# crate-crypto/rust-eth-kzg

Measured on AMD Instinct MI355X. Metric: blobs/sec compute_cells_and_kzg_proofs (4096-pt blob), higher is better.
Workload: dtype u32

## Files before the change

### include/c_eth_kzg_test_hooks.h

```cpp
#ifndef C_ETH_KZG_TEST_HOOKS_H
#define C_ETH_KZG_TEST_HOOKS_H
#include "c_eth_kzg.h"
#ifdef __cplusplus
extern "C" {
#endif

int eth_kzg_amd_test_fr_ntt4096(const DASContext *ctx, const uint8_t *in, uint8_t *out, int inverse_dit);
int eth_kzg_amd_test_g1_fft128(const DASContext *ctx, const uint8_t *in, uint8_t *out, int n_lanes, int inverse);
int eth_kzg_amd_test_fixed_msm(const DASContext *ctx, const uint8_t *scalars, int n_msm, uint8_t *out);
int eth_kzg_amd_test_g1_decompress(const DASContext *ctx, const uint8_t *in, int n, int subgroup_check, int32_t *status,
                                   uint8_t *out);
int eth_kzg_amd_test_field_mul(const DASContext *ctx, const uint8_t *a, const uint8_t *b, uint8_t *out, int n,
                               int is_fp);

int eth_kzg_amd_test_prover_scalars(const DASContext *ctx, int n, const uint8_t *blobs, uint32_t *scalars, uint64_t max_words,
                                    uint64_t *n_words, uint8_t *cells, uint8_t *proofs, int32_t *status, int32_t *fused_launches);

int eth_kzg_amd_test_sha256_many(const DASContext *ctx, uint64_t n, const uint8_t *prefix, uint64_t prefix_len, const uint8_t *d_body,
                                 uint64_t body_stride, uint64_t body_len, const uint8_t *d_tail, uint64_t tail_stride, uint64_t tail_len,
                                 uint8_t *d_out);

int eth_kzg_amd_test_verify_msm(const DASContext *ctx, int form, const uint8_t *points, int n_pts, const uint8_t *sc0, int n0,
                                const uint8_t *sc1, int n1, uint8_t *out96, int32_t *sub_status);

int eth_kzg_amd_test_verify_cells_partial_device(const DASContext *ctx, uint64_t n, const uint8_t *d_commitments,
                                                 const uint64_t *d_cell_indices, const uint8_t *d_cells, const uint8_t *d_proofs, uint64_t lo,
                                                 uint64_t hi, uint8_t *out96);
int eth_kzg_amd_test_verify_blob_batch_inputs(const DASContext *ctx, uint64_t n, int on_device, const void *blobs, const void *commitments,
                                              const void *proofs, uint8_t *out96, int32_t *verified);

int eth_kzg_amd_test_verify_many_sums(const DASContext *ctx, uint64_t n_batches, const uint64_t *commitments_lengths,
                                      const uint8_t *const *const *commitments, const uint64_t *cell_indices_lengths,
                                      const uint64_t *const *cell_indices, const uint64_t *cells_lengths, const uint8_t *const *const *cells,
                                      const uint64_t *proofs_lengths, const uint8_t *const *const *proofs, int32_t *verified, int32_t *status,
                                      int32_t *form4, uint8_t *sums96, uint32_t *rho, uint8_t *fold96, int32_t *probe_ranges,
                                      uint8_t *probe_sums96, uint64_t max_probes, uint64_t *n_probes);

int eth_kzg_amd_test_rs_decode(const DASContext *ctx, int R, const uint64_t *n_cells, const uint64_t *const *cell_indices,
                               const uint8_t *const *const *cells, int flat_source, int32_t *status, int32_t *deg,
                               uint8_t *zp, uint8_t *zeval, uint8_t *zcinv, uint8_t *coeffs);

int eth_kzg_amd_test_op_info(int op, int32_t *in_words, int32_t *out_words, int32_t *device_only, const char **name);
int eth_kzg_amd_test_op(const DASContext *ctx, int op, int n, const int32_t *in, int32_t *out, int on_device);

int eth_kzg_amd_test_table_info(const DASContext *ctx, int kind, int which, int64_t *out8, int32_t *piece_first_block, int max_pieces);
int eth_kzg_amd_test_table_audit(const DASContext *ctx, int kind, int which, uint64_t *visited, uint64_t *n_findings, int32_t *findings,
                                 int max_findings, double *ms);
int eth_kzg_amd_test_table_read(const DASContext *ctx, int kind, int which, int group, int window, int base, int d0, int n, uint32_t *out);
int eth_kzg_amd_test_table_audit_buffer(const DASContext *ctx, int c, int n_groups, int nb, const uint32_t *table, const uint8_t *bases,
                                        int on_device, uint64_t *visited, uint64_t *n_findings, int32_t *findings, int max_findings);

#ifdef __cplusplus
}
#endif
#endif
```

### rust-eth-kzg_amd/__init__.py

```python
import ctypes as C

import numpy as np
import os

_HERE = os.path.dirname(os.path.abspath(__file__))
LIB_PATH = os.path.join(_HERE, "libc_eth_kzg.so")
HOOKS_LIB_PATH = os.path.join(_HERE, "libc_eth_kzg_hooks.so")

BYTES_PER_BLOB = 131072
BYTES_PER_CELL = 2048
BYTES_PER_COMMITMENT = 48
BYTES_PER_PROOF = 48
CELLS_PER_EXT_BLOB = 128
FIELD_ELEMENTS_PER_BLOB = 4096
FIELD_ELEMENTS_PER_CELL = 64


class KzgError(Exception):
    """An operation the reference would report as `Err(..)` (CResult.status == Err)."""


class CResult(C.Structure):
    _fields_ = [("status", C.c_int), ("error_msg", C.c_void_p)]


VERIFY_PARTIAL_BYTES = 96
SETUP_NO_SUBGROUP_CHECK = 1
SETUP_CHECK_POWERS = 2
SETUP_G1_POINTS = 4096
SETUP_G2_POINTS = 65

EXPORTED_SYMBOLS = [
    "eth_kzg_das_context_new", "eth_kzg_das_context_free", "eth_kzg_free_error_message",
    "eth_kzg_blob_to_kzg_commitment", "eth_kzg_compute_cells_and_kzg_proofs", "eth_kzg_compute_cells",
    "eth_kzg_verify_cell_kzg_proof_batch", "eth_kzg_recover_cells_and_proofs",
    "eth_kzg_constant_bytes_per_cell", "eth_kzg_constant_bytes_per_proof", "eth_kzg_constant_cells_per_ext_blob",
    "eth_kzg_compute_kzg_proof", "eth_kzg_compute_blob_kzg_proof", "eth_kzg_verify_kzg_proof",
    "eth_kzg_verify_blob_kzg_proof", "eth_kzg_verify_blob_kzg_proof_batch",
    "eth_kzg_amd_das_context_new_on_device",
    "eth_kzg_amd_das_context_try_new", "eth_kzg_amd_das_context_new_on_devices", "eth_kzg_amd_context_devices",
    "eth_kzg_amd_das_context_new_with_setup", "eth_kzg_amd_das_context_new_with_setup_file", "eth_kzg_amd_setup_digest",
    "eth_kzg_amd_abi_version", "eth_kzg_amd_window_count", "eth_kzg_amd_glv_table",
    "eth_kzg_amd_compute_cells_and_kzg_proofs_batch", "eth_kzg_amd_blob_to_kzg_commitment_batch",
    "eth_kzg_amd_recover_cells_and_proofs_batch", "eth_kzg_amd_recover_cells_and_proofs_device",
    "eth_kzg_amd_verify_cell_kzg_proof_batch_partial", "eth_kzg_amd_verify_cell_kzg_proof_batch_combine",
    "eth_kzg_amd_compute_cells_and_kzg_proofs_device", "eth_kzg_amd_blob_to_kzg_commitment_device",
    "eth_kzg_amd_verify_cell_kzg_proof_batch_device", "eth_kzg_amd_verify_cell_kzg_proof_batch_many",
    "eth_kzg_amd_compute_blob_kzg_proof_batch", "eth_kzg_amd_compute_kzg_proof_batch",
    "eth_kzg_amd_compute_blob_kzg_proof_device", "eth_kzg_amd_compute_kzg_proof_device",
    "eth_kzg_amd_verify_blob_kzg_proof_batch_device",
    "eth_kzg_amd_table_bytes", "eth_kzg_amd_window_bits", "eth_kzg_amd_tables_ready", "eth_kzg_amd_table_groups_ready", "eth_kzg_amd_table_build_info", "eth_kzg_amd_linmap_info",
    "eth_kzg_amd_set_profiling", "eth_kzg_amd_get_stage_times",
    "eth_kzg_amd_comm_probe", "eth_kzg_amd_comm_unique_id", "eth_kzg_amd_comm_init", "eth_kzg_amd_comm_info",
    "eth_kzg_amd_all_gather", "eth_kzg_amd_comm_destroy",
    "eth_kzg_amd_compute_cells_and_kzg_proofs_batch_multi", "eth_kzg_amd_device_count",
]
TEST_HOOK_SYMBOLS = [
    "eth_kzg_amd_test_fr_ntt4096", "eth_kzg_amd_test_g1_fft128", "eth_kzg_amd_test_fixed_msm",
    "eth_kzg_amd_test_g1_decompress", "eth_kzg_amd_test_field_mul", "eth_kzg_amd_test_op_info", "eth_kzg_amd_test_op",
    "eth_kzg_amd_test_table_info", "eth_kzg_amd_test_table_audit", "eth_kzg_amd_test_table_read", "eth_kzg_amd_test_table_audit_buffer",
    "eth_kzg_amd_test_sha256_many", "eth_kzg_amd_test_verify_msm",
    "eth_kzg_amd_test_verify_cells_partial_device", "eth_kzg_amd_test_verify_blob_batch_inputs", "eth_kzg_amd_test_rs_decode",
    "eth_kzg_amd_test_prover_scalars", "eth_kzg_amd_test_verify_many_sums",
]

_lib = None


def load_library():
    global _lib
    if _lib is not None:
        return _lib
    path = os.environ.get("ETH_KZG_AMD_LIB", LIB_PATH)
    if not os.path.exists(path):
        raise RuntimeError(
            f"{LIB_PATH} is missing: build the HIP extension first (python -c 'import __graft_entry__ as g; g.build()' "
            "or make -C rust-eth-kzg_amd/csrc). There is no CPU fallback.")
    lib = C.CDLL(path)
    P, U8P, U64 = C.c_void_p, C.c_char_p, C.c_uint64
    lib.eth_kzg_das_context_new.restype = P
    lib.eth_kzg_das_context_new.argtypes = [C.c_bool]
    lib.eth_kzg_amd_das_context_new_on_device.restype = P
    lib.eth_kzg_amd_das_context_new_on_device.argtypes = [C.c_bool, C.c_int]
    lib.eth_kzg_amd_das_context_try_new.restype = P
    lib.eth_kzg_amd_das_context_try_new.argtypes = [C.c_bool, C.c_int, C.c_double, C.POINTER(CResult)]
    lib.eth_kzg_das_context_free.argtypes = [P]
    lib.eth_kzg_free_error_message.argtypes = [P]
    for name, args in {
        "eth_kzg_blob_to_kzg_commitment": [P, U8P, P],
        "eth_kzg_compute_cells_and_kzg_proofs": [P, U8P, P, P],
        "eth_kzg_compute_cells": [P, U8P, P],
        "eth_kzg_verify_cell_kzg_proof_batch": [P, U64, P, U64, P, U64, P, U64, P, P],
        "eth_kzg_recover_cells_and_proofs": [P, U64, P, U64, P, P, P],
        "eth_kzg_compute_kzg_proof": [P, U8P, U8P, P, P],
        "eth_kzg_compute_blob_kzg_proof": [P, U8P, U8P, P],
        "eth_kzg_verify_kzg_proof": [P, U8P, U8P, U8P, U8P, P],
        "eth_kzg_verify_blob_kzg_proof": [P, U8P, U8P, U8P, P],
        "eth_kzg_verify_blob_kzg_proof_batch": [P, U64, P, U64, P, U64, P, P],
        "eth_kzg_amd_compute_cells_and_kzg_proofs_batch": [P, U64, P, P, P, P],
        "eth_kzg_amd_blob_to_kzg_commitment_batch": [P, U64, P, P, P],
        "eth_kzg_amd_recover_cells_and_proofs_batch": [P, U64, P, P, P, P, P, P, P],
        "eth_kzg_amd_verify_cell_kzg_proof_batch_partial": [P, U64, P, U64, P, U64, P, U64, P, U64, U64, P],
        "eth_kzg_amd_verify_cell_kzg_proof_batch_combine": [P, U64, U8P, P],
        "eth_kzg_amd_recover_cells_and_proofs_device": [P, U64, P, P, P, P, P, P],
        "eth_kzg_amd_compute_cells_and_kzg_proofs_device": [P, U64, P, P, P, P, P],
        "eth_kzg_amd_blob_to_kzg_commitment_device": [P, U64, P, P, P, P],
        "eth_kzg_amd_verify_cell_kzg_proof_batch_device": [P, U64, P, P, P, P, P, P],
        "eth_kzg_amd_verify_cell_kzg_proof_batch_many": [P, U64, P, P, P, P, P, P, P, P, P, P],
        "eth_kzg_amd_compute_blob_kzg_proof_batch": [P, U64, P, P, P, P],
        "eth_kzg_amd_compute_kzg_proof_batch": [P, U64, P, P, P, P, P],
        "eth_kzg_amd_compute_blob_kzg_proof_device": [P, U64, P, P, P, P, P],
        "eth_kzg_amd_compute_kzg_proof_device": [P, U64, P, P, P, P, P, P],
        "eth_kzg_amd_verify_blob_kzg_proof_batch_device": [P, U64, P, P, P, P, P],
        "eth_kzg_amd_comm_unique_id": [P],
        "eth_kzg_amd_comm_probe": [P, P, U64],
        "eth_kzg_amd_comm_info": [P, P, P],
        "eth_kzg_amd_comm_init": [P, U8P, C.c_int, C.c_int],
        "eth_kzg_amd_all_gather": [P, P, P, U64, P],
        "eth_kzg_amd_compute_cells_and_kzg_proofs_batch_multi": [P, U64, U64, P, P, P, P],
    }.items():
        fn = getattr(lib, name)
        fn.restype = CResult
        fn.argtypes = args
    for name in ("eth_kzg_constant_bytes_per_cell", "eth_kzg_constant_bytes_per_proof",
                 "eth_kzg_constant_cells_per_ext_blob"):
        getattr(lib, name).restype = U64
    lib.eth_kzg_amd_comm_destroy.argtypes = [P]
    lib.eth_kzg_amd_comm_destroy.restype = None
    lib.eth_kzg_amd_device_count.restype = C.c_int
    lib.eth_kzg_amd_table_bytes.restype = U64
    lib.eth_kzg_amd_table_bytes.argtypes = [P]
    lib.eth_kzg_amd_window_bits.argtypes = [P]
    lib.eth_kzg_amd_tables_ready.argtypes = [P, C.c_int]
    lib.eth_kzg_amd_tables_ready.restype = C.c_int
    lib.eth_kzg_amd_table_build_info.argtypes = [P, C.POINTER(C.c_double)]
    lib.eth_kzg_amd_table_build_info.restype = None
    lib.eth_kzg_amd_table_groups_ready.argtypes = [P]
    lib.eth_kzg_amd_table_groups_ready.restype = C.c_int
    lib.eth_kzg_amd_linmap_info.argtypes = [P, P]
    lib.eth_kzg_amd_linmap_info.restype = None
    lib.eth_kzg_amd_set_profiling.argtypes = [P, C.c_int]
    lib.eth_kzg_amd_set_profiling.restype = None
    lib.eth_kzg_amd_get_stage_times.argtypes = [P, P, P, C.c_int]
    lib.eth_kzg_amd_das_context_new_on_devices.restype = P
    lib.eth_kzg_amd_das_context_new_on_devices.argtypes = [C.c_bool, P, U64, C.c_double, C.POINTER(CResult)]
    lib.eth_kzg_amd_context_devices.restype = U64
    lib.eth_kzg_amd_context_devices.argtypes = [P, P, U64]
    lib.eth_kzg_amd_abi_version.restype = C.c_int
    if hasattr(lib, "eth_kzg_amd_das_context_new_with_setup"):
        lib.eth_kzg_amd_das_context_new_with_setup.restype = P
        lib.eth_kzg_amd_das_context_new_with_setup.argtypes = [P, U64, P, U64, C.c_uint32, C.c_bool, P, U64, C.c_double, C.POINTER(CResult)]
        lib.eth_kzg_amd_das_context_new_with_setup_file.restype = P
        lib.eth_kzg_amd_das_context_new_with_setup_file.argtypes = [P, U64, C.c_uint32, C.c_bool, P, U64, C.c_double, C.POINTER(CResult)]
        lib.eth_kzg_amd_setup_digest.restype = None
        lib.eth_kzg_amd_setup_digest.argtypes = [P, P]
    lib.eth_kzg_amd_window_count.argtypes = [P]
    lib.eth_kzg_amd_glv_table.argtypes = [P]
    for name, args in {
        "eth_kzg_amd_test_fr_ntt4096": [P, U8P, P, C.c_int],
        "eth_kzg_amd_test_g1_fft128": [P, U8P, P, C.c_int, C.c_int],
        "eth_kzg_amd_test_fixed_msm": [P, U8P, C.c_int, P],
        "eth_kzg_amd_test_g1_decompress": [P, U8P, C.c_int, C.c_int, P, P],
        "eth_kzg_amd_test_field_mul": [P, U8P, U8P, P, C.c_int, C.c_int],
        "eth_kzg_amd_test_op_info": [C.c_int, P, P, P, C.POINTER(C.c_char_p)],
        "eth_kzg_amd_test_op": [P, C.c_int, C.c_int, P, P, C.c_int],
        "eth_kzg_amd_test_table_info": [P, C.c_int, C.c_int, P, P, C.c_int],
        "eth_kzg_amd_test_table_audit": [P, C.c_int, C.c_int, P, P, P, C.c_int, P],
        "eth_kzg_amd_test_table_read": [P, C.c_int, C.c_int, C.c_int, C.c_int, C.c_int, C.c_int, C.c_int, P],
        "eth_kzg_amd_test_table_audit_buffer": [P, C.c_int, C.c_int, C.c_int, P, P, C.c_int, P, P, P, C.c_int],
        "eth_kzg_amd_test_sha256_many": [P, U64, P, U64, P, U64, U64, P, U64, U64, P],
        "eth_kzg_amd_test_verify_msm": [P, C.c_int, U8P, C.c_int, U8P, C.c_int, U8P, C.c_int, P, P],
        "eth_kzg_amd_test_verify_cells_partial_device": [P, U64, P, P, P, P, U64, U64, P],
        "eth_kzg_amd_test_verify_blob_batch_inputs": [P, U64, C.c_int, P, P, P, P, P],
        "eth_kzg_amd_test_rs_decode": [P, C.c_int, P, P, P, C.c_int, P, P, P, P, P, P],
        "eth_kzg_amd_test_prover_scalars": [P, C.c_int, P, P, U64, P, P, P, P, P],
        "eth_kzg_amd_test_verify_many_sums": [P, U64, P, P, P, P, P, P, P, P, P, P, P, P, P, P, P, P, U64, P],
    }.items():
        if hasattr(lib, name):
            getattr(lib, name).argtypes = args
    _lib = lib
    return lib


def present_masks(n, present):
    masks = np.zeros(2 * max(1, n), dtype=np.uint64)
    prev_row, prev_mask = None, 0
    for b in range(n):
        row = present[b]
        if row is prev_row and prev_row is not None:
            m = prev_mask
        else:
            m = 0
            for c in row:
                c = int(c)
                if not 0 <= c < CELLS_PER_EXT_BLOB:
                    raise KzgError("InvalidCellIndex")
                m |= 1 << c
            prev_row, prev_mask = row, m
        masks[2 * b] = m & 0xFFFFFFFFFFFFFFFF
        masks[2 * b + 1] = m >> 64
    return masks


def parse_trusted_setup_json(text):
    import json
    try:
        doc = json.loads(text)
    except ValueError as e:
        raise KzgError(f"InvalidSetup: not JSON ({e})")
    if not isinstance(doc, dict):
        raise KzgError("InvalidSetup: the trusted setup JSON is an object with g1_monomial and g2_monomial")
    out = []
    for key, size in (("g1_monomial", 48), ("g2_monomial", 96)):
        pts = doc.get(key)
        if not isinstance(pts, list):
            raise KzgError(f"InvalidSetup: {key} is missing")
        dec = []
        for i, h in enumerate(pts):
            if not isinstance(h, str) or not h.startswith("0x"):
                raise KzgError(f"InvalidSetup: {key}[{i}] is not a 0x-prefixed hex string")
            try:
                b = bytes.fromhex(h[2:])
            except ValueError:
                raise KzgError(f"InvalidSetup: {key}[{i}] is not hex")
            if len(b) != size:
                raise KzgError(f"InvalidSetup: {key}[{i}] has {len(b)} bytes, not {size}")
            dec.append(b)
        out.append(dec)
    return out[0], out[1]


def _ptr_array(bufs):
    arr = (C.c_void_p * max(1, len(bufs)))()
    keep = []
    for i, b in enumerate(bufs):
        if isinstance(b, (bytes, bytearray)):
            b = C.create_string_buffer(bytes(b), len(b))
        keep.append(b)
        arr[i] = C.addressof(b)
    return arr, keep


def _flat_ptrs(items, size):
    n = len(items)
    flat = np.frombuffer(b"".join(bytes(x) if not isinstance(x, bytes) else x for x in items), dtype=np.uint8) if n else np.zeros(1, np.uint8)
    ptrs = np.uint64(flat.ctypes.data) + np.arange(max(1, n), dtype=np.uint64) * np.uint64(size)
    return ptrs, flat


def _out_ptrs(n_outer, n_inner, size):
    flat = np.zeros(max(1, n_outer * n_inner * size), dtype=np.uint8)
    inner = np.uint64(flat.ctypes.data) + np.arange(max(1, n_outer * n_inner), dtype=np.uint64) * np.uint64(size)
    outer = np.uint64(inner.ctypes.data) + np.arange(max(1, n_outer), dtype=np.uint64) * np.uint64(n_inner * 8)
    return flat, inner, outer


def _split(flat, n_outer, n_inner, size):
    raw = flat.tobytes()
    return [[raw[(b * n_inner + k) * size:(b * n_inner + k + 1) * size] for k in range(n_inner)] for b in range(n_outer)]


def _vp(arr):
    return arr.ctypes.data_as(C.c_void_p)


class DASContext:

    device_index = 0

    def __init__(self, use_precomp=True, device=None, wait_tables=True, table_budget_gb=None, devices=None):
        self.device_index = int(device) if device is not None else int(os.environ.get("ETH_KZG_AMD_DEVICE", "0"))
        self._lib = load_library()
        if devices is not None:
            devs = np.array([int(d) for d in devices], dtype=np.int32)
            self.device_index = int(devs[0]) if len(devs) else 0
            res = CResult()
            self._ctx = C.c_void_p(self._lib.eth_kzg_amd_das_context_new_on_devices(
                bool(use_precomp), _vp(devs) if len(devs) else None, len(devs), float(table_budget_gb or 0.0), C.byref(res)))
            if not self._ctx.value:
                msg = C.cast(res.error_msg, C.c_char_p).value.decode() if res.error_msg else "unknown"
                self._lib.eth_kzg_free_error_message(res.error_msg)
                raise KzgError(msg)
        elif table_budget_gb is not None:
            res = CResult()
            self._ctx = C.c_void_p(self._lib.eth_kzg_amd_das_context_try_new(bool(use_precomp), self.device_index, float(table_budget_gb), C.byref(res)))
            if not self._ctx.value:
                msg = C.cast(res.error_msg, C.c_char_p).value.decode() if res.error_msg else "unknown"
                self._lib.eth_kzg_free_error_message(res.error_msg)
                raise KzgError(msg)
        elif device is None:
            self._ctx = C.c_void_p(self._lib.eth_kzg_das_context_new(bool(use_precomp)))
        else:
            self._ctx = C.c_void_p(self._lib.eth_kzg_amd_das_context_new_on_device(bool(use_precomp), int(device)))
        if not self._ctx.value:
            raise RuntimeError("eth_kzg_das_context_new returned NULL")
        if wait_tables:
            self.tables_ready(-1)

    @classmethod
    def from_trusted_setup(cls, g1_monomial, g2_monomial, *, subgroup_check=True, check_powers=False, use_precomp=True, devices=None,
                           table_budget_gb=None, wait_tables=True):
        def flat(pts, size):
            if isinstance(pts, (bytes, bytearray, memoryview)):
                raw = bytes(pts)
                if len(raw) % size:
                    raise KzgError(f"InvalidSetup: {len(raw)} bytes are not a whole number of {size}-byte points")
                return raw, len(raw) // size
            pts = [bytes(x) for x in pts]
            for i, x in enumerate(pts):
                if len(x) != size:
                    raise KzgError(f"InvalidSetup: point {i} has {len(x)} bytes, not {size}")
            return b"".join(pts), len(pts)
        g1, n1 = flat(g1_monomial, 48)
        g2, n2 = flat(g2_monomial, 96)
        self = cls.__new__(cls)
        self._lib = load_library()
        self._ctx = C.c_void_p(None)
        devs = np.array([int(d) for d in devices], dtype=np.int32) if devices is not None else None
        self.device_index = int(devs[0]) if devs is not None and len(devs) else int(os.environ.get("ETH_KZG_AMD_DEVICE", "0"))
        flags = (0 if subgroup_check else SETUP_NO_SUBGROUP_CHECK) | (SETUP_CHECK_POWERS if check_powers else 0)
        res = CResult()
        b1, b2 = C.create_string_buffer(g1, max(1, len(g1))), C.create_string_buffer(g2, max(1, len(g2)))
        self._ctx = C.c_void_p(self._lib.eth_kzg_amd_das_context_new_with_setup(
            C.addressof(b1), n1, C.addressof(b2), n2, flags, bool(use_precomp), _vp(devs) if devs is not None and len(devs) else None,
            len(devs) if devs is not None else 0, float(table_budget_gb or 0.0), C.byref(res)))
        if not self._ctx.value:
            msg = C.cast(res.error_msg, C.c_char_p).value.decode() if res.error_msg else "unknown"
            self._lib.eth_kzg_free_error_message(res.error_msg)
            raise KzgError(msg)
        if wait_tables:
            self.tables_ready(-1)
        return self

    @classmethod
    def from_trusted_setup_json(cls, text_or_path, *, check_powers=True, **kwargs):
        text = text_or_path
        if not str(text_or_path).lstrip().startswith("{"):
            with open(text_or_path) as f:
                text = f.read()
        g1, g2 = parse_trusted_setup_json(text)
        return cls.from_trusted_setup(g1, g2, check_powers=check_powers, **kwargs)

    @property
    def setup_digest(self):
        out = C.create_string_buffer(32)
        self._lib.eth_kzg_amd_setup_digest(self._ctx, out)
        return out.raw

    def devices(self):
        out = np.zeros(64, dtype=np.int32)
        n = int(self._lib.eth_kzg_amd_context_devices(self._ctx, _vp(out), 64))
        return [int(d) for d in out[:n]]

    def tables_ready(self, wait_ms=0):
        return int(self._lib.eth_kzg_amd_tables_ready(self._ctx, int(wait_ms)))

    def table_build_info(self):
        out = (C.c_double * 4)()
        self._lib.eth_kzg_amd_table_build_info(self._ctx, out)
        return {"hipmalloc_ms": round(out[0], 1), "longest_hipmalloc_ms": round(out[1], 1), "pieces": int(out[2]), "bytes": int(out[3])}

    def table_groups_ready(self):
        return int(self._lib.eth_kzg_amd_table_groups_ready(self._ctx))

    def close(self):
        if getattr(self, "_ctx", None) and self._ctx.value:
            self._lib.eth_kzg_das_context_free(self._ctx)
            self._ctx = C.c_void_p(None)

    def __del__(self):
        try:
            self.close()
        except Exception:
            pass

    @property
    def handle(self):
        return self._ctx

    def _check(self, res):
        if res.status != 0:
            msg = C.string_at(res.error_msg).decode() if res.error_msg else "error"
            self._lib.eth_kzg_free_error_message(res.error_msg)
            raise KzgError(msg)

    def blob_to_kzg_commitment(self, blob):
        if len(blob) != BYTES_PER_BLOB:
            raise KzgError("BlobHasInvalidLength")
        out = C.create_string_buffer(48)
        self._check(self._lib.eth_kzg_blob_to_kzg_commitment(self._ctx, bytes(blob), out))
        return out.raw

    def compute_cells_and_kzg_proofs(self, blob):
        if len(blob) != BYTES_PER_BLOB:
            raise KzgError("BlobHasInvalidLength")
        cells = [C.create_string_buffer(BYTES_PER_CELL) for _ in range(CELLS_PER_EXT_BLOB)]
        proofs = [C.create_string_buffer(48) for _ in range(CELLS_PER_EXT_BLOB)]
        ca, _k1 = _ptr_array(cells)
        pa, _k2 = _ptr_array(proofs)
        self._check(self._lib.eth_kzg_compute_cells_and_kzg_proofs(self._ctx, bytes(blob), ca, pa))
        return [c.raw for c in cells], [p.raw for p in proofs]

    def compute_cells(self, blob):
        if len(blob) != BYTES_PER_BLOB:
            raise KzgError("BlobHasInvalidLength")
        cells = [C.create_string_buffer(BYTES_PER_CELL) for _ in range(CELLS_PER_EXT_BLOB)]
        ca, _k = _ptr_array(cells)
        self._check(self._lib.eth_kzg_compute_cells(self._ctx, bytes(blob), ca))
        return [c.raw for c in cells]

    def verify_cell_kzg_proof_batch(self, commitments, cell_indices, cells, proofs):
        if any(len(c) != 48 for c in commitments) or any(len(p) != 48 for p in proofs) \
                or any(len(c) != BYTES_PER_CELL for c in cells):
            raise KzgError("InvalidLength")
        ca, _k1 = _flat_ptrs(commitments, 48)
        cla, _k2 = _flat_ptrs(cells, BYTES_PER_CELL)
        pa, _k3 = _flat_ptrs(proofs, 48)
        idx = np.array(cell_indices, dtype=np.uint64) if len(cell_indices) else np.zeros(1, np.uint64)
        ok = C.c_bool(False)
        self._check(self._lib.eth_kzg_verify_cell_kzg_proof_batch(
            self._ctx, len(commitments), _vp(ca), len(cell_indices), _vp(idx), len(cells), _vp(cla), len(proofs), _vp(pa),
            C.byref(ok)))
        return bool(ok.value)

    def prepare_verify_cell_kzg_proof_batch(self, commitments, cell_indices, cells, proofs):
        if any(len(c) != 48 for c in commitments) or any(len(p) != 48 for p in proofs) \
                or any(len(c) != BYTES_PER_CELL for c in cells):
            raise KzgError("InvalidLength")
        ca, k1 = _flat_ptrs(commitments, 48)
        cla, k2 = _flat_ptrs(cells, BYTES_PER_CELL)
        pa, k3 = _flat_ptrs(proofs, 48)
        idx = np.array(cell_indices, dtype=np.uint64) if len(cell_indices) else np.zeros(1, np.uint64)
        n = (len(commitments), len(cell_indices), len(cells), len(proofs))

        def run(_keep=(k1, k2, k3)):
            ok = C.c_bool(False)
            self._check(self._lib.eth_kzg_verify_cell_kzg_proof_batch(
                self._ctx, n[0], _vp(ca), n[1], _vp(idx), n[2], _vp(cla), n[3], _vp(pa), C.byref(ok)))
            return bool(ok.value)
        return run

    def prepare_verify_cell_kzg_proof_batch_many(self, problems):
        nb, lens, tabs, keep = self._marshal_many(problems)
        ver = (C.c_bool * max(1, nb))()
        st = (C.c_int32 * max(1, nb))()

        def run(_keep=keep):
            self._check(self._lib.eth_kzg_amd_verify_cell_kzg_proof_batch_many(
                self._ctx, nb, _vp(lens[0]), _vp(tabs[0]), _vp(lens[1]), _vp(tabs[1]), _vp(lens[2]), _vp(tabs[2]), _vp(lens[3]), _vp(tabs[3]),
                ver, st))
            return [bool(v) for v in ver][:nb], list(st)[:nb]
        return run

    @staticmethod
    def _marshal_many(problems):
        nb = len(problems)
        keep, lens = [], np.zeros((4, max(1, nb)), dtype=np.uint64)
        tabs = [np.zeros(max(1, nb), dtype=np.uint64) for _ in range(4)]
        for b, (commitments, cell_indices, cells, proofs) in enumerate(problems):
            if any(len(c) != 48 for c in commitments) or any(len(p) != 48 for p in proofs) \
                    or any(len(c) != BYTES_PER_CELL for c in cells):
                commitments, cell_indices, cells, proofs = [], [0], [], []
            ca, k1 = _flat_ptrs(commitments, 48)
            cla, k2 = _flat_ptrs(cells, BYTES_PER_CELL)
            pa, k3 = _flat_ptrs(proofs, 48)
            idx = np.array(cell_indices, dtype=np.uint64) if len(cell_indices) else np.zeros(1, np.uint64)
            keep += [ca, k1, cla, k2, pa, k3, idx]
            lens[:, b] = (len(commitments), len(cell_indices), len(cells), len(proofs))
            tabs[0][b], tabs[1][b], tabs[2][b], tabs[3][b] = ca.ctypes.data, idx.ctypes.data, cla.ctypes.data, pa.ctypes.data
        return nb, np.ascontiguousarray(lens), tabs, keep

    def verify_cell_kzg_proof_batch_many(self, problems):
        return self.prepare_verify_cell_kzg_proof_batch_many(problems)()

    def verify_cell_kzg_proof_batch_partial(self, commitments, cell_indices, cells, proofs, shard_begin, shard_end):
        if any(len(c) != 48 for c in commitments) or any(len(p) != 48 for p in proofs) \
                or any(len(c) != BYTES_PER_CELL for c in cells):
            raise KzgError("InvalidLength")
        ca, _k1 = _flat_ptrs(commitments, 48)
        cla, _k2 = _flat_ptrs(cells, BYTES_PER_CELL)
        pa, _k3 = _flat_ptrs(proofs, 48)
        idx = np.array(cell_indices, dtype=np.uint64) if len(cell_indices) else np.zeros(1, np.uint64)
        out = C.create_string_buffer(VERIFY_PARTIAL_BYTES)
        self._check(self._lib.eth_kzg_amd_verify_cell_kzg_proof_batch_partial(
            self._ctx, len(commitments), _vp(ca), len(cell_indices), _vp(idx), len(cells), _vp(cla), len(proofs), _vp(pa),
            int(shard_begin), int(shard_end), out))
        return out.raw

    def verify_cell_kzg_proof_batch_combine(self, partials):
        blob = b"".join(partials)
        if len(blob) % VERIFY_PARTIAL_BYTES:
            raise KzgError("InvalidLength")
        ok = C.c_bool(False)
        self._check(self._lib.eth_kzg_amd_verify_cell_kzg_proof_batch_combine(
            self._ctx, len(blob) // VERIFY_PARTIAL_BYTES, blob, C.byref(ok)))
        return bool(ok.value)

    def recover_cells_and_kzg_proofs(self, cell_indices, cells):
        if any(len(c) != BYTES_PER_CELL for c in cells):
            raise KzgError("InvalidLength")
        cla, _k = _ptr_array(cells)
        idx = (C.c_uint64 * max(1, len(cell_indices)))(*cell_indices)
        out_cells = [C.create_string_buffer(BYTES_PER_CELL) for _ in range(CELLS_PER_EXT_BLOB)]
        out_proofs = [C.create_string_buffer(48) for _ in range(CELLS_PER_EXT_BLOB)]
        oca, _k1 = _ptr_array(out_cells)
        opa, _k2 = _ptr_array(out_proofs)
        self._check(self._lib.eth_kzg_recover_cells_and_proofs(
            self._ctx, len(cells), cla, len(cell_indices), idx, oca, opa))
        return [c.raw for c in out_cells], [p.raw for p in out_proofs]

    def compute_kzg_proof(self, blob, z):
        if len(blob) != BYTES_PER_BLOB or len(z) != 32:
            raise KzgError("InvalidLength")
        proof, y = C.create_string_buffer(48), C.create_string_buffer(32)
        self._check(self._lib.eth_kzg_compute_kzg_proof(self._ctx, bytes(blob), bytes(z), proof, y))
        return proof.raw, y.raw

    def compute_blob_kzg_proof(self, blob, commitment):
        if len(blob) != BYTES_PER_BLOB or len(commitment) != 48:
            raise KzgError("InvalidLength")
        proof = C.create_string_buffer(48)
        self._check(self._lib.eth_kzg_compute_blob_kzg_proof(self._ctx, bytes(blob), bytes(commitment), proof))
        return proof.raw

    def verify_kzg_proof(self, commitment, z, y, proof):
        if len(commitment) != 48 or len(proof) != 48 or len(z) != 32 or len(y) != 32:
            raise KzgError("InvalidLength")
        ok = C.c_bool(False)
        self._check(self._lib.eth_kzg_verify_kzg_proof(self._ctx, bytes(commitment), bytes(z), bytes(y), bytes(proof), C.byref(ok)))
        return bool(ok.value)

    def verify_blob_kzg_proof(self, blob, commitment, proof):
        if len(blob) != BYTES_PER_BLOB or len(commitment) != 48 or len(proof) != 48:
            raise KzgError("InvalidLength")
        ok = C.c_bool(False)
        self._check(self._lib.eth_kzg_verify_blob_kzg_proof(self._ctx, bytes(blob), bytes(commitment), bytes(proof), C.byref(ok)))
        return bool(ok.value)

    def verify_blob_kzg_proof_batch(self, blobs, commitments, proofs):
        if any(len(b) != BYTES_PER_BLOB for b in blobs) or any(len(c) != 48 for c in commitments) \
                or any(len(p) != 48 for p in proofs):
            raise KzgError("InvalidLength")
        ba, _k1 = _ptr_array(blobs)
        ca, _k2 = _ptr_array(commitments)
        pa, _k3 = _ptr_array(proofs)
        ok = C.c_bool(False)
        self._check(self._lib.eth_kzg_verify_blob_kzg_proof_batch(self._ctx, len(blobs), ba, len(commitments), ca, len(proofs), pa,
                                                                  C.byref(ok)))
        return bool(ok.value)

    def compute_cells_and_kzg_proofs_batch(self, blobs):
        n = len(blobs)
        if any(len(b) != BYTES_PER_BLOB for b in blobs):
            raise KzgError("InvalidLength")
        ba, _kb = _flat_ptrs(blobs, BYTES_PER_BLOB)
        cells, _ci, cpp = _out_ptrs(n, 128, BYTES_PER_CELL)
        proofs, _pi, ppp = _out_ptrs(n, 128, 48)
        st = (C.c_int32 * max(1, n))()
        self._check(self._lib.eth_kzg_amd_compute_cells_and_kzg_proofs_batch(self._ctx, n, _vp(ba), _vp(cpp), _vp(ppp), st))
        return list(st)[:n], _split(cells, n, 128, BYTES_PER_CELL), _split(proofs, n, 128, 48)

    def host_batch_buffers(self, n):
        cells, ci, cpp = _out_ptrs(n, 128, BYTES_PER_CELL)
        proofs, pi, ppp = _out_ptrs(n, 128, 48)
        return {"cells": cells.reshape(n, 128, BYTES_PER_CELL), "proofs": proofs.reshape(n, 128, 48), "_ci": ci, "_pi": pi,
                "cpp": cpp, "ppp": ppp, "status": (C.c_int32 * max(1, n))()}

    def compute_cells_and_kzg_proofs_batch_np(self, blobs_np, bufs, want_proofs=True):
        n = blobs_np.shape[0]
        assert blobs_np.dtype == np.uint8 and blobs_np.flags["C_CONTIGUOUS"] and blobs_np.size == n * BYTES_PER_BLOB
        ba = np.uint64(blobs_np.ctypes.data) + np.arange(max(1, n), dtype=np.uint64) * np.uint64(BYTES_PER_BLOB)
        self._check(self._lib.eth_kzg_amd_compute_cells_and_kzg_proofs_batch(
            self._ctx, n, _vp(ba), _vp(bufs["cpp"]), _vp(bufs["ppp"]) if want_proofs else None, bufs["status"]))
        return list(bufs["status"])[:n]

    def blob_to_kzg_commitment_batch(self, blobs):
        n = len(blobs)
        if any(len(b) != BYTES_PER_BLOB for b in blobs):
            raise KzgError("InvalidLength")
        ba, _kb = _ptr_array(blobs)
        outs = [C.create_string_buffer(48) for _ in range(n)]
        oa, _ko = _ptr_array(outs)
        st = (C.c_int32 * max(1, n))()
        self._check(self._lib.eth_kzg_amd_blob_to_kzg_commitment_batch(self._ctx, n, ba, oa, st))
        return list(st)[:n], [o.raw for o in outs]

    def recover_cells_and_kzg_proofs_batch(self, batch):
        n = len(batch)
        keep = []
        lens = np.array([len(c) for _, c in batch] or [0], dtype=np.uint64)
        ilens = np.array([len(i) for i, _ in batch] or [0], dtype=np.uint64)
        cpp, ipp = np.zeros(max(1, n), np.uint64), np.zeros(max(1, n), np.uint64)
        for b, (idx, cells) in enumerate(batch):
            if any(len(c) != BYTES_PER_CELL for c in cells):
                raise KzgError("InvalidLength")
            ca, k1 = _flat_ptrs(cells, BYTES_PER_CELL)
            ia = np.array(idx, dtype=np.uint64) if len(idx) else np.zeros(1, np.uint64)
            keep += [ca, k1, ia]
            cpp[b], ipp[b] = ca.ctypes.data, ia.ctypes.data
        out_cells, _ci, ocp = _out_ptrs(n, 128, BYTES_PER_CELL)
        out_proofs, _pi, opp = _out_ptrs(n, 128, 48)
        st = (C.c_int32 * max(1, n))()
        self._check(self._lib.eth_kzg_amd_recover_cells_and_proofs_batch(
            self._ctx, n, _vp(lens), _vp(cpp), _vp(ilens), _vp(ipp), _vp(ocp), _vp(opp), st))
        return list(st)[:n], _split(out_cells, n, 128, BYTES_PER_CELL), _split(out_proofs, n, 128, 48)

    def compute_cells_and_kzg_proofs_device(self, n, d_blobs, d_cells, d_proofs, want_status=True, stream=None):
        st = (C.c_int32 * max(1, n))() if want_status else None
        self._check(self._lib.eth_kzg_amd_compute_cells_and_kzg_proofs_device(
            self._ctx, n, C.c_void_p(d_blobs), C.c_void_p(d_cells) if d_cells else None,
            C.c_void_p(d_proofs) if d_proofs else None, st, C.c_void_p(stream) if stream else None))
        return list(st)[:n] if want_status else None

    def recover_cells_and_kzg_proofs_device(self, n, d_cells, present, d_out_cells, d_out_proofs, stream=None):
        masks = present_masks(n, present)
        st = (C.c_int32 * max(1, n))()
        self._check(self._lib.eth_kzg_amd_recover_cells_and_proofs_device(
            self._ctx, n, C.c_void_p(d_cells), _vp(masks), C.c_void_p(d_out_cells) if d_out_cells else None,
            C.c_void_p(d_out_proofs) if d_out_proofs else None, st, C.c_void_p(stream) if stream else None))
        return list(st)[:n]

    @staticmethod
    def comm_unique_id():
        out = C.create_string_buffer(128)
        res = load_library().eth_kzg_amd_comm_unique_id(out)
        if res.status != 0:
            msg = C.cast(res.error_msg, C.c_char_p).value.decode() if res.error_msg else "error"
            load_library().eth_kzg_free_error_message(res.error_msg)
            raise KzgError(msg)
        return out.raw

    def comm_probe(self):
        buf = C.create_string_buffer(512)
        self._check(self._lib.eth_kzg_amd_comm_probe(self._ctx, buf, 512))
        return buf.value.decode()

    def comm_init(self, unique_id, rank, world):
        self._check(self._lib.eth_kzg_amd_comm_init(self._ctx, unique_id, int(rank), int(world)))

    def comm_info(self):
        r, w = C.c_int(-1), C.c_int(-1)
        self._check(self._lib.eth_kzg_amd_comm_info(self._ctx, C.byref(r), C.byref(w)))
        return r.value, w.value

    def all_gather(self, d_send, d_recv, bytes_per_rank, stream=None):
        self._check(self._lib.eth_kzg_amd_all_gather(self._ctx, C.c_void_p(d_send), C.c_void_p(d_recv), int(bytes_per_rank),
                                                     C.c_void_p(stream) if stream else None))

    def comm_destroy(self):
        self._lib.eth_kzg_amd_comm_destroy(self._ctx)

    @staticmethod
    def compute_cells_and_kzg_proofs_batch_multi(contexts, blobs_np, bufs):
        lib = load_library()
        n = blobs_np.shape[0]
        ba = np.uint64(blobs_np.ctypes.data) + np.arange(max(1, n), dtype=np.uint64) * np.uint64(BYTES_PER_BLOB)
        ctxs = (C.c_void_p * len(contexts))(*[c.handle for c in contexts])
        contexts[0]._check(lib.eth_kzg_amd_compute_cells_and_kzg_proofs_batch_multi(
            ctxs, len(contexts), n, _vp(ba), _vp(bufs["cpp"]), _vp(bufs["ppp"]), bufs["status"]))
        return list(bufs["status"])[:n]

    def verify_cell_kzg_proof_batch_device(self, n, d_commitments, d_cell_indices, d_cells, d_proofs, stream=None):
        ok = C.c_bool(False)
        self._check(self._lib.eth_kzg_amd_verify_cell_kzg_proof_batch_device(
            self._ctx, int(n), C.c_void_p(d_commitments), C.c_void_p(d_cell_indices), C.c_void_p(d_cells), C.c_void_p(d_proofs),
            C.byref(ok), C.c_void_p(stream) if stream else None))
        return bool(ok.value)

    def blob_to_kzg_commitment_device(self, n, d_blobs, d_out, want_status=True, stream=None):
        st = (C.c_int32 * max(1, n))() if want_status else None
        self._check(self._lib.eth_kzg_amd_blob_to_kzg_commitment_device(
            self._ctx, n, C.c_void_p(d_blobs), C.c_void_p(d_out), st, C.c_void_p(stream) if stream else None))
        return list(st)[:n] if want_status else None

    def compute_blob_kzg_proof_batch(self, blobs, commitments):
        n = len(blobs)
        if len(commitments) != n or any(len(b) != BYTES_PER_BLOB for b in blobs) or any(len(c) != 48 for c in commitments):
            raise KzgError("InvalidLength")
        ba, _kb = _flat_ptrs(blobs, BYTES_PER_BLOB)
        ca, _kc = _flat_ptrs(commitments, 48)
        out = np.zeros(max(1, n) * 48, dtype=np.uint8)
        oa = np.uint64(out.ctypes.data) + np.arange(max(1, n), dtype=np.uint64) * np.uint64(48)
        st = (C.c_int32 * max(1, n))()
        self._check(self._lib.eth_kzg_amd_compute_blob_kzg_proof_batch(self._ctx, n, _vp(ba), _vp(ca), _vp(oa), st))
        raw = out.tobytes()
        return list(st)[:n], [raw[48 * b:48 * b + 48] for b in range(n)]

    def compute_kzg_proof_batch(self, blobs, zs):
        n = len(blobs)
        if len(zs) != n or any(len(b) != BYTES_PER_BLOB for b in blobs) or any(len(z) != 32 for z in zs):
            raise KzgError("InvalidLength")
        ba, _kb = _flat_ptrs(blobs, BYTES_PER_BLOB)
        za, _kz = _flat_ptrs(zs, 32)
        proofs, ys = np.zeros(max(1, n) * 48, dtype=np.uint8), np.zeros(max(1, n) * 32, dtype=np.uint8)
        pa = np.uint64(proofs.ctypes.data) + np.arange(max(1, n), dtype=np.uint64) * np.uint64(48)
        ya = np.uint64(ys.ctypes.data) + np.arange(max(1, n), dtype=np.uint64) * np.uint64(32)
        st = (C.c_int32 * max(1, n))()
        self._check(self._lib.eth_kzg_amd_compute_kzg_proof_batch(self._ctx, n, _vp(ba), _vp(za), _vp(pa), _vp(ya), st))
        rp, ry = proofs.tobytes(), ys.tobytes()
        return list(st)[:n], [rp[48 * b:48 * b + 48] for b in range(n)], [ry[32 * b:32 * b + 32] for b in range(n)]

    def compute_blob_kzg_proof_device(self, n, d_blobs, d_commitments, d_out_proofs, want_status=True, stream=None):
        st = (C.c_int32 * max(1, n))() if want_status else None
        self._check(self._lib.eth_kzg_amd_compute_blob_kzg_proof_device(
            self._ctx, n, C.c_void_p(d_blobs), C.c_void_p(d_commitments), C.c_void_p(d_out_proofs), st, C.c_void_p(stream) if stream else None))
        return list(st)[:n] if want_status else None

    def compute_kzg_proof_device(self, n, d_blobs, d_zs, d_out_proofs, d_out_ys, want_status=True, stream=None):
        st = (C.c_int32 * max(1, n))() if want_status else None
        self._check(self._lib.eth_kzg_amd_compute_kzg_proof_device(
            self._ctx, n, C.c_void_p(d_blobs), C.c_void_p(d_zs), C.c_void_p(d_out_proofs), C.c_void_p(d_out_ys), st,
            C.c_void_p(stream) if stream else None))
        return list(st)[:n] if want_status else None

    def verify_blob_kzg_proof_batch_device(self, n, d_blobs, d_commitments, d_proofs, stream=None):
        ok = C.c_bool(False)
        self._check(self._lib.eth_kzg_amd_verify_blob_kzg_proof_batch_device(
            self._ctx, int(n), C.c_void_p(d_blobs), C.c_void_p(d_commitments), C.c_void_p(d_proofs), C.byref(ok),
            C.c_void_p(stream) if stream else None))
        return bool(ok.value)

    STAGES = ["blob_to_coeffs", "coeffs_to_cells", "fk20_scalars", "msm_fixed", "g1_ifft", "g1_fft", "compress", "g1_linmap"]

    def set_profiling(self, on):
        self._lib.eth_kzg_amd_set_profiling(self._ctx, int(bool(on)))

    def get_stage_times(self):
        n = len(self.STAGES)
        ms = (C.c_double * n)()
        ln = (C.c_uint64 * n)()
        self._lib.eth_kzg_amd_get_stage_times(self._ctx, ms, ln, n)
        return {s: (ms[i], int(ln[i])) for i, s in enumerate(self.STAGES)}

    def table_bytes(self):
        return int(self._lib.eth_kzg_amd_table_bytes(self._ctx))

    def window_bits(self):
        return int(self._lib.eth_kzg_amd_window_bits(self._ctx))

    def window_count(self):
        return int(self._lib.eth_kzg_amd_window_count(self._ctx))

    def linmap_info(self):
        out = (C.c_int32 * 4)()
        self._lib.eth_kzg_amd_linmap_info(self._ctx, out)
        return tuple(out)
```

### rust-eth-kzg_amd/csrc/c_api_hooks.cpp

```cpp
#include "../../include/c_eth_kzg_test_hooks.h"
#include "c_ctx.hpp"
#include "launch.hpp"

#include <algorithm>
#include <array>
#include <cstdio>
#include <cstdlib>
#include <cstring>
#include <vector>

namespace {
kzg::Engine* eng(const DASContext* ctx) {
    if (!ctx || !ctx->engine) {
        fprintf(stderr, "c_eth_kzg: context pointer is null\n");
        abort();
    }
    return ctx->engine;
}
}

extern "C" {

int eth_kzg_amd_test_fr_ntt4096(const DASContext* ctx, const uint8_t* in, uint8_t* out, int inverse_dit) {
    return eng(ctx)->test_fr_ntt4096(in, out, inverse_dit);
}
int eth_kzg_amd_test_g1_fft128(const DASContext* ctx, const uint8_t* in, uint8_t* out, int n_lanes, int inverse) {
    return eng(ctx)->test_g1_fft128(in, out, n_lanes, inverse);
}
int eth_kzg_amd_test_fixed_msm(const DASContext* ctx, const uint8_t* scalars, int n_msm, uint8_t* out) {
    return eng(ctx)->test_fixed_msm(scalars, n_msm, out);
}
int eth_kzg_amd_test_prover_scalars(const DASContext* ctx, int n, const uint8_t* blobs, uint32_t* scalars, uint64_t max_words, uint64_t* n_words,
                                    uint8_t* cells, uint8_t* proofs, int32_t* status, int32_t* fused_launches) {
    if (!blobs || !scalars || !n_words || !cells || !proofs || !status || !fused_launches) return kzg::ERR_INPUT;
    return eng(ctx)->test_prover_scalars(n, blobs, scalars, max_words, n_words, cells, proofs, status, fused_launches);
}
int eth_kzg_amd_test_g1_decompress(const DASContext* ctx, const uint8_t* in, int n, int subgroup_check, int32_t* status,
                                   uint8_t* out) {
    return eng(ctx)->test_g1_decompress(in, n, subgroup_check, status, out);
}
int eth_kzg_amd_test_field_mul(const DASContext* ctx, const uint8_t* a, const uint8_t* b, uint8_t* out, int n, int is_fp) {
    return eng(ctx)->test_field_mul(a, b, out, n, is_fp);
}
int eth_kzg_amd_test_sha256_many(const DASContext* ctx, uint64_t n, const uint8_t* prefix, uint64_t prefix_len, const uint8_t* d_body,
                                 uint64_t body_stride, uint64_t body_len, const uint8_t* d_tail, uint64_t tail_stride, uint64_t tail_len,
                                 uint8_t* d_out) {
    if (n > (1u << 24) || (prefix_len | body_len | tail_len) >> 31) return kzg::ERR_INPUT;
    return eng(ctx)->test_sha256_many((int)n, prefix, (uint32_t)prefix_len, d_body, body_stride, (uint32_t)body_len, d_tail, tail_stride,
                                      (uint32_t)tail_len, d_out);
}
int eth_kzg_amd_test_verify_msm(const DASContext* ctx, int form, const uint8_t* points, int n_pts, const uint8_t* sc0, int n0,
                                const uint8_t* sc1, int n1, uint8_t* out96, int32_t* sub_status) {
    if (!points || !sc0 || !sc1 || !out96) return kzg::ERR_INPUT;
    return eng(ctx)->test_verify_msm(form, points, n_pts, sc0, n0, sc1, n1, out96, sub_status);
}
int eth_kzg_amd_test_verify_cells_partial_device(const DASContext* ctx, uint64_t n, const uint8_t* d_commitments, const uint64_t* d_cell_indices,
                                                 const uint8_t* d_cells, const uint8_t* d_proofs, uint64_t lo, uint64_t hi, uint8_t* out96) {
    if (!d_commitments || !d_cell_indices || !d_cells || !d_proofs || !out96) return kzg::ERR_INPUT;
    return eng(ctx)->test_verify_cells_partial_device(n, d_commitments, d_cell_indices, d_cells, d_proofs, lo, hi, out96);
}
int eth_kzg_amd_test_verify_blob_batch_inputs(const DASContext* ctx, uint64_t n, int on_device, const void* blobs, const void* commitments,
                                              const void* proofs, uint8_t* out96, int32_t* verified) {
    if (!blobs || !commitments || !proofs || !out96 || !verified) return kzg::ERR_INPUT;
    int v = 0;
    const int rc = eng(ctx)->test_verify_blob_batch_inputs(n, on_device, blobs, commitments, proofs, out96, &v);
    *verified = v;
    return rc;
}
int eth_kzg_amd_test_verify_many_sums(const DASContext* ctx, uint64_t n_batches, const uint64_t* commitments_lengths,
                                      const uint8_t* const* const* commitments, const uint64_t* cell_indices_lengths,
                                      const uint64_t* const* cell_indices, const uint64_t* cells_lengths, const uint8_t* const* const* cells,
                                      const uint64_t* proofs_lengths, const uint8_t* const* const* proofs, int32_t* verified, int32_t* status,
                                      int32_t* form4, uint8_t* sums96, uint32_t* rho, uint8_t* fold96, int32_t* probe_ranges, uint8_t* probe_sums96,
                                      uint64_t max_probes, uint64_t* n_probes) {
    if (!commitments_lengths || !commitments || !cell_indices_lengths || !cell_indices || !cells_lengths || !cells || !proofs_lengths || !proofs ||
        !verified || !status || !form4 || !sums96 || !rho || !fold96 || !n_probes || (max_probes && (!probe_ranges || !probe_sums96)))
        return kzg::ERR_INPUT;
    return eng(ctx)->test_verify_many_sums(n_batches, commitments_lengths, commitments, cell_indices_lengths, cell_indices, cells_lengths, cells,
                                           proofs_lengths, proofs, verified, status, form4, sums96, rho, fold96, probe_ranges, probe_sums96, max_probes,
                                           n_probes);
}
int eth_kzg_amd_test_rs_decode(const DASContext* ctx, int R, const uint64_t* n_cells, const uint64_t* const* cell_indices,
                               const uint8_t* const* const* cells, int flat_source, int32_t* status, int32_t* deg, uint8_t* zp, uint8_t* zeval,
                               uint8_t* zcinv, uint8_t* coeffs) {
    if (R < 1 || R > 4096 || !n_cells || !cell_indices || !cells || (flat_source != 0 && flat_source != 1)) return kzg::ERR_INPUT;
    for (int r = 0; r < R; r++) {
        if (n_cells[r] < 64 || n_cells[r] > 128 || !cell_indices[r] || !cells[r]) return kzg::ERR_INPUT;
        for (uint64_t k = 0; k < n_cells[r]; k++) {
            if (cell_indices[r][k] >= 128 || (k && cell_indices[r][k - 1] >= cell_indices[r][k])) return kzg::ERR_INPUT;
            if (!cells[r][flat_source ? 0 : k]) return kzg::ERR_INPUT;
        }
    }
    return eng(ctx)->test_rs_decode(R, n_cells, cell_indices, cells, flat_source, status, deg, zp, zeval, zcinv, coeffs);
}
int eth_kzg_amd_test_op_info(int op, int32_t* in_words, int32_t* out_words, int32_t* device_only, const char** name) {
    int i, o, d;
    const char* nm;
    if (kzg::launch::test_op_info(op, &i, &o, &d, &nm) != 0) return -1;
    *in_words = i;
    *out_words = o;
    *device_only = d;
    *name = nm;
    return 0;
}
int eth_kzg_amd_test_op(const DASContext* ctx, int op, int n, const int32_t* in, int32_t* out, int on_device) {
    if (on_device) return eng(ctx)->test_op(op, n, in, out);
    int i, o, d;
    const char* nm;
    if (kzg::launch::test_op_info(op, &i, &o, &d, &nm) != 0 || d || n <= 0) return kzg::ERR_INPUT;
    return kzg::launch::test_op_host(op, n, in, out) == 0 ? 0 : kzg::ERR_INPUT;
}

static bool glv_shape_ok(int c, int n_groups, int nb) {
    return kzg::launch::glv_width_supported(c) && n_groups >= 1 && n_groups <= 128 && nb >= 1 && nb <= 64;
}
int eth_kzg_amd_test_table_info(const DASContext* ctx, int kind, int which, int64_t* out8, int32_t* piece_first_block, int max_pieces) {
    return eng(ctx)->test_table_info(kind, which, out8, piece_first_block, max_pieces);
}
int eth_kzg_amd_test_table_audit(const DASContext* ctx, int kind, int which, uint64_t* visited, uint64_t* n_findings, int32_t* findings,
                                 int max_findings, double* ms) {
    return eng(ctx)->test_table_audit(kind, which, visited, n_findings, findings, max_findings, ms);
}
int eth_kzg_amd_test_table_read(const DASContext* ctx, int kind, int which, int group, int window, int base, int d0, int n, uint32_t* out) {
    return eng(ctx)->test_table_read(kind, which, group, window, base, d0, n, out);
}
int eth_kzg_amd_test_table_audit_buffer(const DASContext* ctx, int c, int n_groups, int nb, const uint32_t* table, const uint8_t* bases,
                                        int on_device, uint64_t* visited, uint64_t* n_findings, int32_t* findings, int max_findings) {
    if (!glv_shape_ok(c, n_groups, nb) || max_findings < 0) return kzg::ERR_INPUT;
    if (on_device) return eng(ctx)->test_table_audit_buffer(c, n_groups, nb, table, bases, visited, n_findings, findings, max_findings);
    const int WL = kzg::launch::glv_lower_windows(c), W = kzg::launch::glv_windows(c);
    const size_t lower = kzg::launch::glv_entries_per_base(c, 0, WL) * (size_t)nb, upper = kzg::launch::glv_entries_per_base(c, WL, W) * (size_t)nb;
    std::vector<const void*> blocks((size_t)2 * n_groups);
    const char* t = (const char*)table;
    for (int g = 0; g < n_groups; g++) {
        blocks[2 * g] = t + (size_t)g * (lower + upper) * kzg::launch::SIZEOF_TABP;
        blocks[2 * g + 1] = t + ((size_t)g * (lower + upper) + lower) * kzg::launch::SIZEOF_TABP;
    }
    unsigned long long v = 0, nf = 0;
    kzg::launch::table_audit_host(blocks.data(), bases, c, n_groups, nb, &v, &nf, findings, max_findings);
    std::vector<std::array<int32_t, 5>> f(std::min<unsigned long long>(nf, (unsigned long long)max_findings));
    if (!f.empty()) {
        memcpy(f.data(), findings, f.size() * sizeof(f[0]));
        std::sort(f.begin(), f.end());
        memcpy(findings, f.data(), f.size() * sizeof(f[0]));
    }
    *visited = v;
    *n_findings = nf;
    return 0;
}

}
```

### rust-eth-kzg_amd/csrc/engine.hip

```cpp
#include "engine_internal.hpp"

namespace kzg {

static Fr fr_from_u64(uint64_t v) {
    Fr a = zero<FrParams>();
    a.v[0] = (uint32_t)v;
    a.v[1] = (uint32_t)(v >> 32);
    return to_mont(a);
}
static Fr fr_pow_limbs(const Fr& base, const uint32_t* e, int nl) {
    Fr acc = one<FrParams>();
    for (int i = 32 * nl - 1; i >= 0; i--) {
        acc = sqr(acc);
        if ((e[i >> 5] >> (i & 31)) & 1) acc = mul(acc, base);
    }
    return acc;
}
static Fr fr_root_of_unity(int log_n) {
    uint32_t e[8];
    for (int i = 0; i < 8; i++) e[i] = FrParams::MOD[i];
    e[0] -= 1;
    for (int s = 0; s < log_n; s++) {
        for (int i = 0; i < 8; i++) e[i] = (e[i] >> 1) | (i < 7 ? (e[i + 1] << 31) : 0);
    }
    return fr_pow_limbs(fr_from_u64(7), e, 8);
}
typedef unsigned __int128 u128;
static const u128 GLV_LAMBDA = ((u128)0xac45a4010001a402ULL << 64) | 0x00000000ffffffffULL;
static void glv_split(const Fr& canon, u128& k1, u128& k2) {
    u128 rem = 0, q = 0;
    for (int i = 255; i >= 0; i--) {
        bool top = (rem >> 127) & 1;
        rem = (rem << 1) | ((canon.v[i >> 5] >> (i & 31)) & 1);
        q <<= 1;
        if (top || rem >= GLV_LAMBDA) { rem -= GLV_LAMBDA; q |= 1; }
    }
    k1 = rem;
    k2 = q;
}
static void recode_glv_wnaf(const Fr& k_mont, const Fr& lambda_mont, uint32_t* out) {
    constexpr int TWW = launch::TWIDDLE_WORDS, W = launch::TWIDDLE_WNAF_W;
    u128 r, q;
    glv_split(from_mont(k_mont), r, q);
    struct Half { u128 mag; bool neg; };
    auto signed_sub = [](u128 a, u128 b) { return a >= b ? Half{a - b, false} : Half{b - a, true}; };
    const Half cand[4][2] = {
        {Half{r, false}, Half{q, false}},
        {signed_sub(r, GLV_LAMBDA), Half{q + 1, false}},
        {signed_sub(r, 1), signed_sub(q, GLV_LAMBDA + 1)},
        {signed_sub(r, GLV_LAMBDA + 1), signed_sub(q, GLV_LAMBDA)},
    };
    auto fr_of = [](const Half& h) {
        Fr a = zero<FrParams>();
        for (int i = 0; i < 4; i++) a.v[i] = (uint32_t)(h.mag >> (32 * i));
        a = to_mont(a);
        return h.neg ? neg(a) : a;
    };
    auto naf = [&](const Half& h, int8_t* dg, int& len, int& weight) {
        u128 v = h.mag;
        len = weight = 0;
        for (int t = 0; v != 0; t++, v >>= 1) {
            if (t >= 4 * TWW) throw std::runtime_error("constant recoding too long");
            if (!(v & 1)) continue;
            int d = (int)(v & ((1u << W) - 1));
            if (d >= (1 << (W - 1))) d -= 1 << W;
            if (d < 0) v += (u128)(-d); else v -= (u128)d;
            dg[t] = (int8_t)(h.neg ? -d : d);
            len = t + 1;
            weight++;
        }
    };
    double best_cost = 0;
    int best = -1;
    std::vector<uint32_t> best_words;
    for (int c = 0; c < 4; c++) {
        if (!eq(add(fr_of(cand[c][0]), mul(fr_of(cand[c][1]), lambda_mont)), k_mont)) throw std::runtime_error("GLV split failed");
        std::vector<uint32_t> words(2 * TWW, 0u);
        int len[2], wt[2];
        for (int h = 0; h < 2; h++) naf(cand[c][h], reinterpret_cast<int8_t*>(&words[(size_t)h * TWW]), len[h], wt[h]);
        const double cost = linmap::COST_DBL * std::max(len[0], len[1]) + 5.0e3 * (wt[0] + wt[1]);
        if (best < 0 || cost < best_cost) { best = c; best_cost = cost; best_words = words; }
    }
    for (int i = 0; i < 2 * TWW; i++) out[i] = best_words[i];
    for (int h = 0; h < 2; h++) {
        const int8_t* dg = reinterpret_cast<const int8_t*>(out + (size_t)h * TWW);
        Fr back = zero<FrParams>(), pw = one<FrParams>();
        for (int t = 0; t < 4 * TWW; t++, pw = add(pw, pw)) {
            const int d = dg[t];
            if (!d) continue;
            Fr term = pw;
            for (int m = 1; m < (d < 0 ? -d : d); m++) term = add(term, pw);
            back = d < 0 ? sub(back, term) : add(back, term);
        }
        if (!eq(back, fr_of(cand[best][h]))) throw std::runtime_error("constant recoding failed");
    }
}
double trace_clock_ms() {
    static const auto t0 = std::chrono::steady_clock::now();
    return std::chrono::duration<double, std::milli>(std::chrono::steady_clock::now() - t0).count();
}
static thread_local std::string t_last_error;
const std::string& Engine::last_error() const { return t_last_error; }
void Engine::set_error(const std::exception& e) { t_last_error = e.what(); }

BufferPool::~BufferPool() {
    for (auto& f : free_) {
        if (host_) (void)hipHostFree(f.second);
        else (void)hipFree(f.second);
    }
}
void* BufferPool::get(size_t bytes, size_t* cls) {
    size_t c = 256;
    while (c < bytes) c <<= 1;
    *cls = c;
    for (size_t i = 0; i < free_.size(); i++)
        if (free_[i].first == c) {
            void* p = free_[i].second;
            free_[i] = free_.back();
            free_.pop_back();
            pooled_ -= c;
            return p;
        }
    void* p = nullptr;
    hipError_t e = host_ ? hipHostMalloc(&p, c, hipHostMallocDefault) : hipMalloc(&p, c);
    if (e != hipSuccess) {
        (void)hipGetLastError();
        for (auto& f : free_) { if (host_) (void)hipHostFree(f.second); else (void)hipFree(f.second); }
        free_.clear();
        pooled_ = 0;
        e = host_ ? hipHostMalloc(&p, c, hipHostMallocDefault) : hipMalloc(&p, c);
        if (e != hipSuccess) throw std::runtime_error(host_ ? "hipHostMalloc failed" : "hipMalloc failed");
    }
    return p;
}
void BufferPool::put(void* p, size_t cls) {
    constexpr size_t KEEP = 6ull << 30;
    if (pooled_ + cls > KEEP) {
        if (host_) (void)hipHostFree(p); else (void)hipFree(p);
        return;
    }
    free_.emplace_back(cls, p);
    pooled_ += cls;
}
PoolBuf::PoolBuf(Engine& e, size_t bytes, bool pinned_host) : e_(e), host_(pinned_host) {
    p = (host_ ? e_.pin_pool_ : e_.dev_pool_).get(bytes ? bytes : 1, &cls_);
}
PoolBuf::~PoolBuf() {
    (void)hipStreamSynchronize(e_.stream_);
    (host_ ? e_.pin_pool_ : e_.dev_pool_).put(p, cls_);
}

std::atomic<bool> g_exiting{false};
std::mutex g_engines_mu;
std::vector<Engine*> g_engines;
void Engine::stop_builder() {
    cancel_build_.store(true);
    if (builder_.joinable()) builder_.join();
}
void stop_all_builders_at_exit() {
    g_exiting.store(true);
    std::vector<Engine*> live;
    {
        std::lock_guard<std::mutex> lk(g_engines_mu);
        live = g_engines;
    }
    for (Engine* e : live) e->stop_builder();
}

Engine::SerialLease Engine::lease_serial() {
    return lanes_.lease(this, max_lanes_, auxiliary_, [this] {
        try {
            return std::unique_ptr<Engine>(new Engine(use_precomp_, dev_, this));
        } catch (...) {
            (void)hipGetLastError();
            throw;
        }
    });
}

Engine::Engine(bool use_precomp, int device, const Engine* primary, double table_budget_gb, std::shared_ptr<const TrustedSetup> setup)
    : dev_(device), use_precomp_(use_precomp), primary_(primary), auxiliary_(primary != nullptr) {
    setup_ = primary ? primary->setup_ : setup ? std::move(setup) : TrustedSetup::mainnet();
    knobs_ = primary ? primary->knobs_ : Knobs::from_env();
    if (knobs_.serial_lanes) max_lanes_ = knobs_.serial_lanes;
    if (knobs_.device_batch_max) device_batch_max_ = ((knobs_.device_batch_max + 63) / 64) * 64;
    if (use_precomp) {
        if (launch::glv_width_supported(knobs_.glv_window)) want_glv_c_ = knobs_.glv_window;
        if (table_budget_gb != 0) table_budget_gb_ = table_budget_gb;
        else if (knobs_.table_budget_gb != 0) table_budget_gb_ = knobs_.table_budget_gb;
    }
    vm_search_ = knobs_.vm_search;
    msm_split_ = knobs_.msm_split;
    fused_scalars_ = knobs_.fused_scalars;
    if (knobs_.pip_shift_min >= 1) pip_shift_min_ = knobs_.pip_shift_min;
#ifdef KZG_CIRC_MAX
    circ_max_ = KZG_CIRC_MAX;
#else
    circ_max_ = 2;
#endif
    try {
        construct();
    } catch (...) {
        teardown();
        throw;
    }
}

void Engine::construct() {
    TraceLap lap{knobs_.trace, "context"};
    HIPCK(hipSetDevice(dev_));
    {
        int cus = 0;
        HIPCK(hipDeviceGetAttribute(&cus, hipDeviceAttributeMultiprocessorCount, dev_));
        wave_slots_ = cus * 4 * 2;
        if (knobs_.msm_chunks >= 0) msm_chunks_ = knobs_.msm_chunks;
    }
    HIPCK(hipStreamCreateWithFlags(&stream_, hipStreamNonBlocking));
    if (!primary_) {
        int prio_low = 0, prio_high = 0;
        HIPCK(hipDeviceGetStreamPriorityRange(&prio_low, &prio_high));
        HIPCK(hipStreamCreateWithPriority(&build_stream_, hipStreamNonBlocking, prio_low));
    }
    if (v_two_streams_) HIPCK(hipStreamCreateWithFlags(&v_side_, hipStreamNonBlocking));
    HIPCK(hipEventCreateWithFlags(&v_decoded_, hipEventDisableTiming));
    HIPCK(hipEventCreateWithFlags(&v_checked_, hipEventDisableTiming));
    for (Work& w : work_) {
        HIPCK(hipEventCreateWithFlags(&w.done, hipEventDisableTiming));
        HIPCK(hipEventCreateWithFlags(&w.ev_in, hipEventDisableTiming));
        HIPCK(hipEventCreateWithFlags(&w.ev_cells, hipEventDisableTiming));
        HIPCK(hipEventCreateWithFlags(&w.ev_cells_host, hipEventDisableTiming));
        HIPCK(hipEventCreateWithFlags(&w.ev_done, hipEventDisableTiming));
        HIPCK(hipEventCreateWithFlags(&w.ev_coeffs, hipEventDisableTiming));
        HIPCK(hipEventCreateWithFlags(&w.ev_side, hipEventDisableTiming));
        if (&w == &work_[0]) continue;
        if (primary_) continue;
        int prio_low = 0, prio_high = 0;
        HIPCK(hipDeviceGetStreamPriorityRange(&prio_low, &prio_high));
        HIPCK(hipStreamCreateWithFlags(&w.stream, hipStreamNonBlocking));
        HIPCK(hipStreamCreateWithPriority(&w.copy, hipStreamNonBlocking, prio_high));
    }
    launch::init_attributes();
    if (!primary_) settle_streams();
    lap("HIP runtime + stream");
    init_constants();
    lap("twiddles, recodings");
    init_srs();
    lap("SRS decompress");
    init_fk20();
    lap("FK20 bases + start tables");
    init_verifier();
    HIPCK(hipStreamSynchronize(stream_));
    lap("verifier (G2 lines, cosets)");
    if (setup_->check_powers && !primary_) {
        check_setup_powers();
        lap("setup: powers of one tau");
    }
    if (knobs_.fault == "constructor" && !primary_) throw std::runtime_error("injected fault (ETH_KZG_AMD_FAULT=constructor)");
    start_builder();
}

bool Engine::streams_overlap(hipStream_t a, hipStream_t b) {
    int khz = 0;
    if (hipDeviceGetAttribute(&khz, hipDeviceAttributeWallClockRate, dev_) != hipSuccess || khz <= 0) khz = 100000;
    const double spin_us = 300.0;
    const uint64_t ticks = (uint64_t)(spin_us * 1e-3 * khz);
    for (int t = 0; t < 3; t++) {
        HIPCK(hipStreamSynchronize(a));
        HIPCK(hipStreamSynchronize(b));
        const auto t0 = std::chrono::steady_clock::now();
        launch::spin(ticks, a);
        launch::spin(ticks, b);
        HIPCK(hipStreamSynchronize(a));
        HIPCK(hipStreamSynchronize(b));
        const double us = std::chrono::duration<double, std::micro>(std::chrono::steady_clock::now() - t0).count();
        if (us < 1.6 * spin_us) return true;
    }
    return false;
}
void Engine::settle_streams() {
    const bool trace = knobs_.trace;
    launch::spin(1, stream_);
    std::vector<hipStream_t> chosen{stream_}, rejected;
    bool gave_up = false;
    for (int i = 1; i < NW; i++) {
        Work& w = work_[i];
        if (!w.stream || gave_up) continue;
        for (int attempt = 0;; attempt++) {
            launch::spin(1, w.stream);
            bool ok = true;
            for (hipStream_t c : chosen) ok = ok && streams_overlap(c, w.stream);
            if (ok || attempt == 5) {
                if (trace) fprintf(stderr, "[eth_kzg_amd] work set %d: stream %s after %d replacement(s)\n", i, ok ? "runs beside the others" : "still shares a queue", attempt);
                if (!ok) gave_up = true;
                break;
            }
            rejected.push_back(w.stream);
            HIPCK(hipStreamCreateWithFlags(&w.stream, hipStreamNonBlocking));
        }
        chosen.push_back(w.stream);
    }
    for (hipStream_t r : rejected) hipStreamDestroy(r);
}

Engine::~Engine() { teardown(); }

void Engine::teardown() noexcept {
    (void)hipSetDevice(dev_);
    lanes_.clear();
    stop_builder();
    {
        std::lock_guard<std::mutex> lk(g_engines_mu);
        g_engines.erase(std::remove(g_engines.begin(), g_engines.end(), this), g_engines.end());
    }
    if (build_stream_) hipStreamDestroy(build_stream_);
    host_pool_.reset();
    vm_pool_.reset();
    stage_pool_.reset();
    void* ptrs[] = {d_w8192_, d_w29_, d_tapk_, d_naf_, d_srs_, d_fk_bases_, d_in_, d_cells_, d_proofs_, d_coset_, d_coset_inv_, d_circ_terms_, d_4844_};
    for (void* p : ptrs)
        if (p) hipFree(p);
    for (SlpProgram& P : slp_prog_) {
        if (P.d_words) hipFree(P.d_words);
        if (P.d_naf && P.owns_naf) hipFree(P.d_naf);
    }
    for (Work& w : work_) {
        void* dev[] = {w.coeffs, w.canon, w.scalars, w.X, w.status, w.circ_table, w.slp_arena, w.d_in, w.d_cells, w.d_proofs};
        for (void* p : dev)
            if (p) hipFree(p);
        void* pin[] = {w.h_in, w.h_cells, w.h_proofs, w.h_status};
        for (void* p : pin)
            if (p) hipHostFree(p);
        hipEvent_t evs[] = {w.done, w.ev_in, w.ev_cells, w.ev_cells_host, w.ev_done, w.ev_coeffs, w.ev_side};
        for (hipEvent_t e : evs)
            if (e) hipEventDestroy(e);
        for (hipEvent_t e : w.sub_events) hipEventDestroy(e);
        if (w.stream) hipStreamDestroy(w.stream);
        if (w.copy) hipStreamDestroy(w.copy);
    }
    if (v_dev_) hipFree(v_dev_);
    if (v_pin_) hipHostFree(v_pin_);
    for (VmSlot& v : vm_slot_) {
        if (v.dev) hipFree(v.dev);
        if (v.pin) hipHostFree(v.pin);
        if (v.vs.dev) hipFree(v.vs.dev);
        if (v.vs.pin) hipHostFree(v.vs.pin);
    }
    if (vd_pin_) hipHostFree(vd_pin_);
    for (hipEvent_t e : vd_events_)
        if (e) hipEventDestroy(e);
    if (v_side_) hipStreamDestroy(v_side_);
    if (v_decoded_) hipEventDestroy(v_decoded_);
    if (v_checked_) hipEventDestroy(v_checked_);
    if (stream_) hipStreamDestroy(stream_);
}

void Engine::init_constants() {
    std::vector<Fr> w(N_EXT);
    Fr g = fr_root_of_unity(13);
    w[0] = one<FrParams>();
    for (int i = 1; i < N_EXT; i++) w[i] = mul(w[i - 1], g);
    if (!eq(mul(w[N_EXT - 1], g), one<FrParams>())) throw std::runtime_error("omega_8192 has wrong order");
    HIPCK(hipMalloc(&d_w8192_, N_EXT * sizeof(Fr)));
    HIPCK(hipMemcpy(d_w8192_, w.data(), N_EXT * sizeof(Fr), hipMemcpyHostToDevice));
    {
        std::vector<uint32_t> w29((size_t)N_EXT * 9);
        launch::ntt_twiddles29(w.data(), w29.data());
        HIPCK(hipMalloc(&d_w29_, w29.size() * 4));
        HIPCK(hipMemcpy(d_w29_, w29.data(), w29.size() * 4, hipMemcpyHostToDevice));
    }
    {
        Fr lam = zero<FrParams>();
        for (int i = 0; i < 4; i++) lam.v[i] = (uint32_t)(GLV_LAMBDA >> (32 * i));
        Fr lm = to_mont(lam);
        if (!is_zero(add(add(sqr(lm), lm), one<FrParams>()))) throw std::runtime_error("GLV lambda is not a cube root of unity");
        constexpr int TWW = launch::TWIDDLE_WORDS;
        std::vector<uint32_t> tw((size_t)128 * 2 * TWW, 0u);
        for (int k = 0; k < 128; k++) recode_glv_wnaf(w[64 * k], lm, &tw[(size_t)k * 2 * TWW]);
        HIPCK(hipMalloc(&d_naf_, tw.size() * 4));
        HIPCK(hipMemcpy(d_naf_, tw.data(), tw.size() * 4, hipMemcpyHostToDevice));
        std::vector<uint32_t> plus, minus;
        int max_t = 0;
        for (int d = 0; d < 128; d++) {
            Fr c = zero<FrParams>();
            for (int t = 0; t < 64; t++) c = add(c, w[(64 * d * t) & (N_EXT - 1)]);
            if (d != 0 && (d & 1) == 0) {
                if (!is_zero(c)) throw std::runtime_error("circulant symbol: even entry is not zero");
                continue;
            }
            u128 kk[2];
            glv_split(from_mont(c), kk[0], kk[1]);
            Fr back = zero<FrParams>();
            for (int half = 0; half < 2; half++) {
                u128 k = kk[half];
                Fr pw = half ? lm : one<FrParams>();
                for (int t = 0; k != 0; t++, k >>= 1, pw = add(pw, pw)) {
                    if (!(k & 1)) continue;
                    const int dg = 2 - (int)(k & 3);
                    if (dg < 0) k += 1;
                    const uint32_t word = (uint32_t)d | ((uint32_t)t << 7) | ((uint32_t)half << 15) | ((dg < 0 ? 1u : 0u) << 16) | (1u << 17);
                    (dg < 0 ? minus : plus).push_back(word);
                    back = dg < 0 ? sub(back, pw) : add(back, pw);
                    if (t > max_t) max_t = t;
                }
            }
            if (!eq(back, c)) throw std::runtime_error("circulant term list does not reproduce its symbol");
        }
        if ((int)plus.size() < launch::CIRC_LANES || max_t >= 255) throw std::runtime_error("circulant term list is malformed");
        std::vector<uint32_t> all(plus);
        all.insert(all.end(), minus.begin(), minus.end());
        circ_T_ = max_t + 1;
        circ_per_lane_ = ((int)all.size() + launch::CIRC_LANES - 1) / launch::CIRC_LANES;
        all.resize((size_t)circ_per_lane_ * launch::CIRC_LANES, 0u);
        HIPCK(hipMalloc(&d_circ_terms_, all.size() * 4));
        HIPCK(hipMemcpy(d_circ_terms_, all.data(), all.size() * 4, hipMemcpyHostToDevice));
    }
    init_linmap(reinterpret_cast<const Fr8*>(w.data()));
    for (int sgi = 0; sgi < 3; sgi++) {
        Fr v = zero<FrParams>();
        v.v[sgi + 1] = 1;
        v = to_mont(v);
        memcpy(&seg_shift_[sgi], &v, 32);
    }
    Fr i4096 = inv(fr_from_u64(N_BLOB)), i128 = inv(fr_from_u64(128));
    memcpy(&n_inv4096_, &i4096, 32);
    memcpy(&inv128_, &i128, 32);
    HIPCK(hipMalloc(&d_tapk_, (size_t)2 * N_EXT * launch::SIZEOF_FR29));
    launch::fk20_tap_consts(d_w29_, half_, d_tapk_, stream_);
    launch::fk20_tap_consts(d_w29_, inv128_, (char*)d_tapk_ + (size_t)N_EXT * launch::SIZEOF_FR29, stream_);
    HIPCK(hipGetLastError());
}

static linmap::Strategy slp_strategy(int id) {
    linmap::Strategy s;
    s.allow_toom8 = true;
    {
        Fr lam = zero<FrParams>();
        for (int i = 0; i < 4; i++) lam.v[i] = (uint32_t)(GLV_LAMBDA >> (32 * i));
        s.lambda = to_mont(lam);
    }
    auto fixed = [&](int k4, int k8, int k16, int k32) {
        s.tuned = false;
        s.balanced_lincomb = true;
        s.phi = false;
        s.hankel_split = {{2, 2}, {4, k4}, {8, k8}, {16, k16}, {32, k32}};
    };
    switch (id) {
        case 2: fixed(2, 2, 2, 2); break;
        case 3: fixed(4, 2, 4, 2); break;
        case 4: fixed(2, 2, 2, 4); break;
        case 5: fixed(4, 2, 4, 8); break;
        default: break;
    }
    return s;
}
void Engine::build_slp_program(int id) {
    const Fr* w128p = reinterpret_cast<const Fr*>(w128_.data());
    const std::vector<Fr> w128(w128p, w128p + 128);
    const bool verbose = knobs_.trace;
    linmap::Plan plan = linmap::build_fk20_proofs_plan(w128, slp_strategy(id), verbose);
    {
        std::vector<linmap::Ref> perm(128);
        for (int p = 0; p < 128; p++) {
            int k = 0;
            for (int b = 0; b < 7; b++) k |= ((p >> b) & 1) << (6 - b);
            perm[p] = plan.outputs[k];
        }
        plan.outputs = perm;
    }
    const linmap::Schedule sched = linmap::make_schedule(plan, id == SLP_TUNED_FUSED);
    uint64_t st = 0x853c49e6748fea9bull + (uint64_t)id;
    for (int it = 0; it < 2; it++) {
        std::vector<Fr> in(128);
        for (auto& v : in) {
            for (int i = 0; i < 8; i++) { st ^= st << 13; st ^= st >> 7; st ^= st << 17; v.v[i] = (uint32_t)(st >> 16); }
            v.v[7] &= 0x3fffffffu;
        }
        const auto want = linmap::fk20_proofs_map_by_definition(w128, in);
        const auto got1 = linmap::run_over_fr(plan, in);
        const auto got2 = linmap::run_schedule_over_fr(sched, plan.consts, 128, 128, in);
        for (int p = 0; p < 128; p++) {
            int k = 0;
            for (int b = 0; b < 7; b++) k |= ((p >> b) & 1) << (6 - b);
            if (!eq(want[k], got1[p]) || !eq(want[k], got2[p])) throw std::runtime_error("FK20 proofs map: compiled program differs from its definition");
        }
    }
    SlpProgram& P = slp_prog_[id];
    if (id == SLP_TUNED && slp_prog_[SLP_TUNED_FUSED].ready) {
        P.d_naf = slp_prog_[SLP_TUNED_FUSED].d_naf;
    } else {
        Fr lam = zero<FrParams>();
        for (int i = 0; i < 4; i++) lam.v[i] = (uint32_t)(GLV_LAMBDA >> (32 * i));
        const Fr lm = to_mont(lam);
        constexpr int TWW = launch::TWIDDLE_WORDS;
        std::vector<uint32_t> naf(plan.consts.size() * 2 * TWW);
        for (size_t c = 0; c < plan.consts.size(); c++) recode_glv_wnaf(plan.consts[c], lm, &naf[c * 2 * TWW]);
        HIPCK(hipMalloc(&P.d_naf, naf.size() * 4));
        P.owns_naf = true;
        HIPCK(hipMemcpy(P.d_naf, naf.data(), naf.size() * 4, hipMemcpyHostToDevice));
    }
    HIPCK(hipMalloc(&P.d_words, sched.words.size() * 4));
    HIPCK(hipMemcpy(P.d_words, sched.words.data(), sched.words.size() * 4, hipMemcpyHostToDevice));
    P.launches.clear();
    for (auto& L : sched.launches) P.launches.push_back(SlpLaunch{(int)L.kind, L.first, L.count});
    P.n_slots = sched.n_slots;
    P.info[0] = (int)plan.count(linmap::OP_MULC);
    P.info[1] = (int)(plan.count(linmap::OP_ADD) + plan.count(linmap::OP_SUB));
    P.info[2] = (int)plan.doublings();
    P.info[3] = (int)sched.launches.size();
    if (verbose) fprintf(stderr, "[linmap] program %d: %d multiplications, %d additions, %d doublings, %d launches, %d slots\n", id, P.info[0], P.info[1], P.info[2], P.info[3], P.n_slots);
    P.ready = true;
}
const Engine::SlpProgram& Engine::slp_program(int id) {
    std::lock_guard<std::mutex> lk(slp_build_mu_);
    if (!slp_prog_[id].ready) build_slp_program(id);
    return slp_prog_[id];
}
int Engine::pick_slp_program(int lanes) const {
    if (slp_force_ >= 0) return slp_force_;
    const int groups = lanes / 64, simds = wave_slots_ / 2;
    if (712 * groups <= simds) return SLP_KARATSUBA;
    if (456 * groups <= simds) return SLP_DEPTH_456;
    if (606 * groups <= wave_slots_) return SLP_DEPTH_606;
    if (456 * groups <= wave_slots_) return SLP_DEPTH_456;
    if (372 * groups <= wave_slots_) return SLP_DEPTH_372;
    if (456 * groups <= wave_slots_ * 3 / 2) return SLP_DEPTH_456;
    if (groups <= 12) return SLP_DEPTH_372;
    return lanes >= slp_fuse_min_ ? SLP_TUNED_FUSED : SLP_TUNED;
}
void Engine::init_linmap(const Fr8* w8192_mont) {
    static_assert(sizeof(Fr8) == sizeof(Fr), "layout");
    if (knobs_.slp_program >= 0 && knobs_.slp_program < SLP_COUNT) slp_force_ = knobs_.slp_program;
    w128_.resize(128);
    for (int e = 0; e < 128; e++) w128_[e] = w8192_mont[64 * e];
    build_slp_program(SLP_TUNED_FUSED);
    build_slp_program(SLP_TUNED);
    const SlpProgram& fused = slp_prog_[SLP_TUNED_FUSED];
    {
        if (fused.info[0] != slp_prog_[SLP_TUNED].info[0]) throw std::runtime_error("FK20 proofs map: the two schedules differ");
    }
    for (int i = 0; i < 3; i++) slp_info_[i] = fused.info[i];
    slp_info_[3] = fused.info[3];
    const Fr h = inv(fr_from_u64(2));
    memcpy(&half_, &h, 32);
}

void Engine::init_srs() {
    const TrustedSetup& ts = *setup_;
    if (ts.g1.size() != (size_t)N_BLOB * 48) throw std::runtime_error("trusted setup: wrong number of G1 points");
    const bool checked = ts.subgroup_check && !ts.embedded && !primary_;
    uint8_t* d_bytes = nullptr;
    int* d_st = nullptr;
    std::vector<int> st(N_BLOB);
    struct Scratch {
        uint8_t*& b;
        int*& s;
        ~Scratch() { if (b) (void)hipFree(b); if (s) (void)hipFree(s); }
    } scratch{d_bytes, d_st};
    HIPCK(hipMalloc(&d_bytes, (size_t)N_BLOB * 48));
    HIPCK(hipMalloc(&d_st, N_BLOB * sizeof(int)));
    HIPCK(hipMalloc(&d_srs_, N_BLOB * sizeof(G1Affine)));
    HIPCK(hipMemcpy(d_bytes, ts.g1.data(), (size_t)N_BLOB * 48, hipMemcpyHostToDevice));
    {
        Fp12w nobeta{};
        launch::g1_decompress(d_bytes, d_srs_, d_st, N_BLOB, 0, nobeta, stream_);
    }
    HIPCK(hipMemcpyAsync(st.data(), d_st, N_BLOB * sizeof(int), hipMemcpyDeviceToHost, stream_));
    HIPCK(hipStreamSynchronize(stream_));
    for (int i = 0; i < N_BLOB; i++) {
        if (st[i]) throw std::runtime_error("g1_monomial[" + std::to_string(i) + "] is not the encoding of a curve point");
        if ((ts.g1[(size_t)i * 48] >> 6) & 1) throw std::runtime_error("g1_monomial[" + std::to_string(i) + "] is the point at infinity");
    }
    {
        G1Affine P;
        HIPCK(hipMemcpy(&P, (const G1Affine*)d_srs_ + 1, sizeof(G1Affine), hipMemcpyDeviceToHost));
        uint32_t lam[4];
        for (int i = 0; i < 4; i++) lam[i] = (uint32_t)(GLV_LAMBDA >> (32 * i));
        G1Affine Q = to_affine(scalar_mul<4>(to_jac(P), lam));
        Fp bx = mul(Q.x, inv(P.x));
        Fp b3 = mul(sqr(bx), bx);
        if (!eq(b3, one<FpParams>()) || eq(bx, one<FpParams>()) || !eq(Q.y, P.y)) {
            if (!ts.embedded) throw std::runtime_error("g1_monomial[1] is not in the prime-order subgroup (the endomorphism check failed on it)");
            throw std::runtime_error("GLV endomorphism check failed");
        }
        memcpy(&beta_, &bx, 48);
    }
    if (checked) {
        launch::g1_decompress(d_bytes, d_srs_, d_st, N_BLOB, 1, beta_, stream_);
        HIPCK(hipMemcpyAsync(st.data(), d_st, N_BLOB * sizeof(int), hipMemcpyDeviceToHost, stream_));
        HIPCK(hipStreamSynchronize(stream_));
        for (int i = 0; i < N_BLOB; i++) {
            if (st[i] == 2) throw std::runtime_error("g1_monomial[" + std::to_string(i) + "] is not in the prime-order subgroup");
            if (st[i]) throw std::runtime_error("g1_monomial[" + std::to_string(i) + "] is not the encoding of a curve point");
        }
    }
}

}
```

### rust-eth-kzg_amd/csrc/engine.hpp

```cpp
#pragma once
#include "knobs.hpp"
#include "host_sync.hpp"
#include "trusted_setup.hpp"
#include <hip/hip_runtime.h>
#include <cstddef>
#include <cstdint>
#include <atomic>
#include <condition_variable>
#include <deque>
#include <functional>
#include <mutex>
#include <thread>
#include <string>
#include <utility>
#include <vector>
#include <memory>

namespace kzg {

namespace pairing { struct G2Prepared; }
struct Comm;
struct G1Affine;
struct Fr8 { uint32_t v[8]; };
struct Fp12w { uint32_t v[12]; };

constexpr uint64_t MAX_CELLS_PER_VERIFICATION = (1u << 24) - 1;
constexpr int VM_SPLIT_MIN_PROBLEMS = 192, VM_SPLIT_MIN_CELLS = 24576, VM_CHUNK_CELLS = 131072;
struct VerifyManyTap {
    int passes = 0;
    int small = 0, folded = 0, searched = 0;
    int fold_verdict = -1;
    std::vector<uint8_t> sums;
    std::vector<uint32_t> rho;
    std::vector<uint8_t> fold;
    std::vector<int> probes;
    std::vector<uint8_t> probe_sums;
};

enum Status : int {
    OK = 0,
    ERR_SCALAR = 1,
    ERR_G1 = 2,
    ERR_INPUT = 3,
    ERR_RECOVERY = 4,
    ERR_DEVICE = 5,
};

class BufferPool {
public:
    explicit BufferPool(bool pinned_host) : host_(pinned_host) {}
    ~BufferPool();
    void* get(size_t bytes, size_t* cls);
    void put(void* p, size_t cls);
private:
    bool host_;
    std::vector<std::pair<size_t, void*>> free_;
    size_t pooled_ = 0;
};
class Engine;
struct PoolBuf {
    void* p = nullptr;
    PoolBuf(Engine& e, size_t bytes, bool pinned_host = false);
    ~PoolBuf();
    PoolBuf(const PoolBuf&) = delete;
    PoolBuf& operator=(const PoolBuf&) = delete;
private:
    Engine& e_;
    size_t cls_ = 0;
    bool host_;
};

struct Work {
    std::mutex mu;
    int cap = 0;
    void *coeffs = nullptr, *canon = nullptr, *scalars = nullptr, *X = nullptr;
    int* status = nullptr;
    void *circ_table = nullptr, *slp_arena = nullptr;
    size_t slp_arena_bytes = 0;
    hipEvent_t done = nullptr;
    int stage_cap = 0;
    uint8_t *d_in = nullptr, *d_cells = nullptr, *d_proofs = nullptr;
    uint8_t *h_in = nullptr, *h_cells = nullptr, *h_proofs = nullptr;
    int* h_status = nullptr;
    hipStream_t stream = nullptr, copy = nullptr;
    hipEvent_t ev_in = nullptr, ev_cells = nullptr, ev_cells_host = nullptr, ev_done = nullptr;
    hipEvent_t ev_coeffs = nullptr, ev_side = nullptr;
    std::vector<hipEvent_t> sub_events;
};
class Engine {
public:
    friend struct PoolBuf;
    struct SharedTable;
    Engine(bool use_precomp, int device, const Engine* primary = nullptr, double table_budget_gb = 0,
           std::shared_ptr<const TrustedSetup> setup = nullptr);
    static constexpr double DEFAULT_TABLE_BUDGET_GB = 108.0;
    ~Engine();
    Engine(const Engine&) = delete;

    using SerialLease = LanePool<Engine>::Lease;
    friend class LanePool<Engine>;

    SerialLease lease_serial();

    int device() const { return dev_; }
    const TrustedSetup& setup() const { return *setup_; }
    Comm* comm() const { return comm_; }
    void set_comm(Comm* c) { comm_ = c; }
    hipStream_t stream() const { return stream_; }
    const std::string& last_error() const;

    int compute_cells_and_kzg_proofs_device(int n, const uint8_t* d_blobs, uint8_t* d_cells, uint8_t* d_proofs,
                                            int* h_status, hipStream_t stream, bool sync);
    int blob_to_kzg_commitment_device(int n, const uint8_t* d_blobs, uint8_t* d_commitments, int* h_status,
                                      hipStream_t stream, bool sync);

    int compute_cells_and_kzg_proofs_host(int n, const uint8_t* const* blobs, uint8_t* const* const* cells,
                                          uint8_t* const* const* proofs, int* h_status);
    int blob_to_kzg_commitment_host(int n, const uint8_t* const* blobs, uint8_t* const* out, int* h_status);

    int verify_cell_kzg_proof_batch_host(uint64_t n_commitments, const uint8_t* const* commitments, uint64_t n_indices,
                                         const uint64_t* cell_indices, uint64_t n_cells, const uint8_t* const* cells,
                                         uint64_t n_proofs, const uint8_t* const* proofs, int* verified);
    int verify_cell_kzg_proof_batch_device(uint64_t n, const uint8_t* d_commitments, const uint64_t* d_cell_indices,
                                           const uint8_t* d_cells, const uint8_t* d_proofs, int* verified, hipStream_t stream);
    int verify_cell_kzg_proof_batch_many_host(uint64_t n_batches, const uint64_t* n_commitments, const uint8_t* const* const* commitments,
                                              const uint64_t* n_indices, const uint64_t* const* cell_indices, const uint64_t* n_cells,
                                              const uint8_t* const* const* cells, const uint64_t* n_proofs,
                                              const uint8_t* const* const* proofs, int* verified, int* status, VerifyManyTap* tap = nullptr);
    int verify_cell_kzg_proof_batch_combined(uint64_t n_commitments, const uint8_t* const* commitments, uint64_t n_indices,
                                             const uint64_t* cell_indices, uint64_t n_cells, const uint8_t* const* cells,
                                             uint64_t n_proofs, const uint8_t* const* proofs, int* verified);
    int verify_cell_kzg_proof_batch_partial_host(uint64_t n_commitments, const uint8_t* const* commitments, uint64_t n_indices,
                                                 const uint64_t* cell_indices, uint64_t n_cells, const uint8_t* const* cells,
                                                 uint64_t n_proofs, const uint8_t* const* proofs, uint64_t lo, uint64_t hi,
                                                 uint8_t* out96);
    int verify_cell_kzg_proof_batch_combine_host(uint64_t n_partials, const uint8_t* partials96, int* verified);
    int recover_cells_and_kzg_proofs_host(uint64_t n_cells, const uint8_t* const* cells, uint64_t n_indices,
                                          const uint64_t* cell_indices, uint8_t* const* out_cells,
                                          uint8_t* const* out_proofs);

    int compute_kzg_proof_host(const uint8_t* blob, const uint8_t* z, uint8_t* out_proof, uint8_t* out_y);
    int compute_blob_kzg_proof_host(const uint8_t* blob, const uint8_t* commitment, uint8_t* out_proof);
    int verify_kzg_proof_host(const uint8_t* commitment, const uint8_t* z, const uint8_t* y, const uint8_t* proof, int* verified);
    int verify_blob_kzg_proof_host(const uint8_t* blob, const uint8_t* commitment, const uint8_t* proof, int* verified);
    int verify_blob_kzg_proof_batch_host(uint64_t n_blobs, const uint8_t* const* blobs, uint64_t n_commitments,
                                         const uint8_t* const* commitments, uint64_t n_proofs, const uint8_t* const* proofs,
                                         int* verified, G1Affine* sums2 = nullptr);
    int compute_blob_kzg_proof_device(int n, const uint8_t* d_blobs, const uint8_t* d_commitments, uint8_t* d_out_proofs, int* h_status,
                                      hipStream_t stream, bool sync);
    int compute_kzg_proof_device(int n, const uint8_t* d_blobs, const uint8_t* d_z, uint8_t* d_out_proofs, uint8_t* d_out_y, int* h_status,
                                 hipStream_t stream, bool sync);
    int compute_blob_kzg_proof_batch_host(int n, const uint8_t* const* blobs, const uint8_t* const* commitments, uint8_t* const* out_proofs,
                                          int* h_status);
    int compute_kzg_proof_batch_host(int n, const uint8_t* const* blobs, const uint8_t* const* zs, uint8_t* const* out_proofs,
                                     uint8_t* const* out_ys, int* h_status);
    int verify_blob_kzg_proof_batch_device(uint64_t n, const uint8_t* d_blobs, const uint8_t* d_commitments, const uint8_t* d_proofs,
                                           int* verified, hipStream_t stream, G1Affine* sums2 = nullptr);

    int recover_cells_and_kzg_proofs_device(int R, const uint8_t* d_cells, const uint64_t* present_masks, uint8_t* d_out_cells,
                                            uint8_t* d_out_proofs, int* status, hipStream_t stream);
    int recover_cells_and_kzg_proofs_batch_host(int R, const uint64_t* n_cells, const uint8_t* const* const* cells,
                                                const uint64_t* n_indices, const uint64_t* const* cell_indices,
                                                uint8_t* const* const* out_cells, uint8_t* const* const* out_proofs,
                                                int* status);

    int test_fr_ntt4096(const uint8_t* in_be, uint8_t* out_be, int inverse_dit);
    int test_g1_fft128(const uint8_t* in_compressed, uint8_t* out_compressed, int n_lanes, int inverse);
    int test_fixed_msm(const uint8_t* scalars_be, int n_msm, uint8_t* out_compressed);
    int test_prover_scalars(int n, const uint8_t* blobs, uint32_t* scalars, uint64_t max_words, uint64_t* n_words, uint8_t* cells, uint8_t* proofs,
                            int32_t* status, int32_t* fused_launches);
    int test_g1_decompress(const uint8_t* in, int n, int subgroup_check, int* h_status, uint8_t* out_recompressed);
    int test_field_mul(const uint8_t* a, const uint8_t* b, uint8_t* out, int n, int is_fp);
    int test_op(int op, int n, const int32_t* in, int32_t* out);
    int test_sha256_many(int n, const uint8_t* prefix, uint32_t prefix_len, const uint8_t* d_body, size_t body_stride, uint32_t body_len,
                         const uint8_t* d_tail, size_t tail_stride, uint32_t tail_len, uint8_t* d_out);
    int test_verify_msm(int form, const uint8_t* points, int n_pts, const uint8_t* sc0_be, int n0, const uint8_t* sc1_be, int n1,
                        uint8_t* out96, int32_t* h_status);
    int test_verify_cells_partial_device(uint64_t n, const uint8_t* d_commitments, const uint64_t* d_cell_indices, const uint8_t* d_cells,
                                         const uint8_t* d_proofs, uint64_t lo, uint64_t hi, uint8_t* out96);
    int test_verify_blob_batch_inputs(uint64_t n, int on_device, const void* blobs, const void* commitments, const void* proofs, uint8_t* out96,
                                      int* verified);
    int test_verify_many_sums(uint64_t n_batches, const uint64_t* n_commitments, const uint8_t* const* const* commitments, const uint64_t* n_indices,
                              const uint64_t* const* cell_indices, const uint64_t* n_cells, const uint8_t* const* const* cells, const uint64_t* n_proofs,
                              const uint8_t* const* const* proofs, int32_t* verified, int32_t* status, int32_t* form4, uint8_t* sums96, uint32_t* rho,
                              uint8_t* fold96, int32_t* probe_ranges, uint8_t* probe_sums96, uint64_t max_probes, uint64_t* n_probes);
    int test_rs_decode(int R, const uint64_t* n_cells, const uint64_t* const* cell_indices, const uint8_t* const* const* cells, int flat_source,
                       int32_t* status, int32_t* deg, uint8_t* zp, uint8_t* zeval, uint8_t* zcinv, uint8_t* coeffs);
    std::shared_ptr<SharedTable> test_table(int kind, int which) const;
    int test_table_info(int kind, int which, int64_t* out8, int32_t* piece_first_block, int max_pieces);
    int test_table_audit(int kind, int which, uint64_t* visited, uint64_t* n_findings, int32_t* findings, int max_findings, double* ms);
    int test_table_read(int kind, int which, int group, int window, int base, int d0, int n, uint32_t* out);
    int test_table_audit_buffer(int c, int n_groups, int nb, const uint32_t* table, const uint8_t* bases, uint64_t* visited, uint64_t* n_findings,
                                int32_t* findings, int max_findings);

    enum Stage { ST_BLOB_TO_COEFFS = 0, ST_COEFFS_TO_CELLS, ST_FK20_SCALARS, ST_MSM_FIXED, ST_G1_IFFT, ST_G1_FFT,
                 ST_COMPRESS, ST_G1_LINMAP, ST_COUNT };
    void set_profiling(bool on);
    void get_stage_times(double* ms, uint64_t* launches);

    struct TableView {
        std::shared_ptr<SharedTable> main, next;
        int c = 0;
        size_t bytes = 0;
    };
    enum TableSel { TAB_FK = 0, TAB_SRS = 1 };
    TableView table_view(TableSel which) const;
    int tables_ready(int wait_ms);
    int table_groups_ready(TableSel which) const;
    void table_build_info(double* out4) const;
    void stop_builder();
    size_t table_bytes() const { return table_view(TAB_FK).bytes + table_view(TAB_SRS).bytes; }
    int window_bits() const { return table_view(TAB_FK).c; }
    int window_count() const { const int c = window_bits(); return c > 0 ? (128 + c - 1) / c : 0; }
    const int* linmap_info() const { return slp_info_; }

private:
    void construct();
    void teardown() noexcept;
    void start_builder();
    void init_constants();
    void init_linmap(const Fr8* w8192_mont);
    void init_srs();
    void check_setup_powers();
    void settle_streams();
    bool streams_overlap(hipStream_t a, hipStream_t b);
    void init_fk20();
    void init_verifier();
    int open_blobs_at(int n, const uint8_t* const* blobs, const Fr8* z_mont, bool want_proofs, uint8_t* h_proofs, Fr8* h_y_canon,
                      int* h_status);
    void open_blobs_core(int n, const uint8_t* d_blobs, const void* d_z_mont, void* d_y, uint8_t* d_proofs, hipStream_t st);
    struct Scratch4844 {
        uint8_t *dig = nullptr, *proofs = nullptr;
        void *z = nullptr, *y = nullptr, *aff = nullptr;
        int *blob_bad = nullptr, *z_bad = nullptr, *g1_bad = nullptr, *status = nullptr;
    };
    Scratch4844 scratch_4844(int n);
    void fs_challenges_device(int n, const uint8_t* d_blobs, const uint8_t* d_commitments, const Scratch4844& s, hipStream_t st);
    int finish_verify_blob_batch(int n, const Fr8* z_mont, const Fr8* y_canon, const uint8_t* const* commitments, const uint8_t* const* proofs,
                                 const void* d_points, G1Affine* sums2 = nullptr);
    int proofs_batch_host(int n, const uint8_t* const* blobs, const uint8_t* const* commitments, const uint8_t* const* zs,
                          uint8_t* const* out_proofs, uint8_t* const* out_ys, int* h_status);
    void open_staged_blobs(int nb, const uint8_t* h_blobs_pinned, const Fr8* z_mont, const uint8_t* h_commitments, uint8_t* h_proofs, Fr8* h_y,
                           int* h_blob_status, int* h_g1_status);
    HostPool* ensure_host_pool();
    void* d_4844_ = nullptr;
    int cap_4844_ = 0;
    int pairing_check_4844(const void* d_points, const std::vector<Fr8>& sc0, const std::vector<Fr8>& sc1, G1Affine* sums2 = nullptr);
    struct VerifyScratch {
        hipStream_t stream = nullptr;
        void* dev = nullptr;
        size_t dev_cap = 0;
        uint8_t* pin = nullptr;
        size_t pin_cap = 0;
    };
    struct VerifyDeviceSource {
        const uint8_t *d_cells, *d_proofs;
        hipEvent_t* chunk_events;
        int chunk_cells, n_chunks;
    };
    int verify_cells_partial(uint64_t n_commitments, const uint8_t* const* commitments, uint64_t n_indices,
                             const uint64_t* cell_indices, uint64_t n_cells, const uint8_t* const* cells, uint64_t n_proofs,
                             const uint8_t* const* proofs, uint64_t lo, uint64_t hi, G1Affine* out2, bool* empty,
                             const VerifyDeviceSource* dsrc = nullptr, VerifyScratch* vs = nullptr);
    int verify_cells_partial_device(uint64_t n, const uint8_t* d_commitments, const uint64_t* d_cell_indices, const uint8_t* d_cells,
                                    const uint8_t* d_proofs, uint64_t lo, uint64_t hi, G1Affine* out2, bool* empty, hipStream_t user_stream);
    bool verify_cells_pairing(const G1Affine* pts2) const;
    bool verify_cells_pairing_split(const G1Affine* pts2);
    struct RsDecodeTap { int* deg = nullptr; Fr8 *zp = nullptr, *zeval = nullptr, *zcinv = nullptr; };
    int rs_decode(int R, const uint8_t* d_cells, bool flat_source, const std::vector<int>& slot, const std::vector<int>& stof,
                  const std::vector<uint32_t>& present, int* st_out, const RsDecodeTap* tap = nullptr);
    int recover_batch_to_coeffs(int R, const uint64_t* n_cells, const uint8_t* const* const* cells,
                                const uint64_t* const* cell_indices, int* st_out);
    void ensure_workspace(int n);
    void ensure_workspace(Work& w, int n, bool release = false);
    void ensure_staging(Work& w, int n);
    void run_proofs_from_coeffs(int n, uint8_t* d_proofs, hipStream_t st) { run_proofs_from_coeffs(work_[0], n, d_proofs, st); }
    enum ProofsPhase { PROOFS_ALL = 0, PROOFS_HEAD = 1, PROOFS_TAIL = 2 };
    void run_proofs_from_coeffs(Work& w, int n, uint8_t* d_proofs, hipStream_t st, const TableView* tv_pre = nullptr, ProofsPhase phase = PROOFS_ALL,
                                int msm_cut = 0);
    void enqueue_compute(Work& w, int n, const uint8_t* d_blobs, uint8_t* d_cells, uint8_t* d_proofs, hipStream_t st,
                         hipEvent_t after_cells);
    int fk20_segs(int n) const;
    Work& lease_work(int first, int last);
    void release_work(Work& w);
    std::mutex lease_mu_;
    std::condition_variable lease_cv_;
    void set_error(const std::exception& e);
    void launch_msm(const void* scalars, TableSel table, void* out, int n_groups, int n_slices, int out_stride,
                    int brp_bits, hipStream_t st, int out_fmt );
    void launch_msm(const void* scalars, const TableView& tv, bool scalars_split, void* out, int n_groups, int n_slices, int out_stride,
                    int brp_bits, hipStream_t st, int out_fmt );
    void launch_msm_range(const void* scalars, const SharedTable& t, int g0, int gcnt, void* out, int n_groups, int n_slices, int out_stride,
                          int brp_bits, hipStream_t st, int out_fmt);
    long msm_waves(long msms, int c) const;
    void build_final_tables();
    void publish(TableSel which, const std::shared_ptr<SharedTable>& main, const std::shared_ptr<SharedTable>& next);
    void g1_fft128_full(void* X, int stride, int inverse, hipStream_t st);

    struct StageMark { int stage; int launches; hipEvent_t a, b; };
    int mark_begin(int stage, hipStream_t st);
    void mark_end(int mark, int launches, hipStream_t st);
    bool profiling_ = false;
    std::vector<StageMark> marks_;
    unsigned marks_gen_ = 0;
    std::mutex marks_mu_;

    int dev_ = 0;
    std::shared_ptr<const TrustedSetup> setup_;
    Comm* comm_ = nullptr;
    bool use_precomp_ = true;
    Knobs knobs_;
    int want_glv_c_ = 0;
    double table_budget_gb_ = DEFAULT_TABLE_BUDGET_GB;
    mutable std::mutex tab_mu_;
    std::condition_variable tab_cv_;
    std::weak_ptr<SharedTable> start_tab_[2];
    Published<SharedTable> pub_[2];
    int tables_state_ = 0;
    std::string tables_error_;
    std::thread builder_;
    std::atomic<bool> cancel_build_{false};
    bool progressive_build_ = false;
    hipStream_t build_stream_ = nullptr;
    int wave_slots_ = 2048;
    int device_batch_max_ = 4096;
    int msm_chunks_ = -1;
    int fused_scalars_ = -1;
    std::atomic<uint64_t> fused_launches_{0};
    bool msm_split_ = true;
    hipStream_t stream_ = nullptr;
    std::recursive_mutex mu_;
    static constexpr int NW = 4;
    Work work_[NW];
    std::unique_ptr<HostPool> host_pool_;
    std::once_flag host_pool_once_;

    void* d_w8192_ = nullptr;
    void* d_w29_ = nullptr;
    void* d_naf_ = nullptr;
    Fp12w beta_;
    void* d_srs_ = nullptr;
    void* d_fk_bases_ = nullptr;
    BufferPool dev_pool_{false}, pin_pool_{true};
    void* d_tapk_ = nullptr;
    Fr8 n_inv4096_, inv128_;

    void* d_coset_ = nullptr;
    void* d_coset_inv_ = nullptr;
    Fr8 inv64_, n_inv8192_;
    std::shared_ptr<pairing::G2Prepared> g2_tau_, g2_neg_gen_;
    std::shared_ptr<pairing::G2Prepared> g2_tau1_;

    void* v_dev_ = nullptr;
    size_t v_dev_cap_ = 0;
    uint8_t* v_pin_ = nullptr;
    size_t v_pin_cap_ = 0;
    hipStream_t v_side_ = nullptr;
    bool v_two_streams_ = false;
    hipEvent_t v_decoded_ = nullptr, v_checked_ = nullptr;

    const Engine* primary_ = nullptr;
    bool auxiliary_ = false;
    std::mutex lane_busy_;
    LanePool<Engine> lanes_;
    int max_lanes_ = 4;

    struct VerifyRequest;
    Combiner<VerifyRequest> combiner_{VM_SLOTS};
    std::atomic<int> verify_inflight_{0};
    int verify_lanes_ = 1;
    int comb_max_cells_ = 1024;

    static constexpr int VM_SLOTS = 3;
    struct VmSlot {
        VerifyScratch vs;
        void* dev = nullptr;
        size_t dev_cap = 0;
        uint8_t* pin = nullptr;
        size_t pin_cap = 0;
    };
    VmSlot vm_slot_[VM_SLOTS];
    SlotSet<VM_SLOTS> vm_slots_;
    std::unique_ptr<HostPool> stage_pool_;
    std::once_flag stage_pool_once_;
    std::unique_ptr<HostPool> vm_pool_;
    std::once_flag vm_pool_once_;
    bool vm_search_ = true;
    int vm_small_max_ = -1;
    uint8_t* vd_pin_ = nullptr;
    size_t vd_pin_cap_ = 0;
    static constexpr int VD_CHUNKS = 8;
    hipEvent_t vd_events_[VD_CHUNKS] = {};

    void *d_circ_terms_ = nullptr;
    int pip_shift_min_ = 1;
    int circ_T_ = 0, circ_per_lane_ = 0, circ_max_ = 2;
    Fr8 seg_shift_[3];
    struct SlpLaunch { int kind, first, count; };
    enum SlpProgramId { SLP_TUNED_FUSED = 0, SLP_TUNED = 1, SLP_KARATSUBA = 2, SLP_DEPTH_456 = 3, SLP_DEPTH_606 = 4, SLP_DEPTH_372 = 5, SLP_COUNT = 6 };
    struct SlpProgram {
        std::vector<SlpLaunch> launches;
        void *d_words = nullptr, *d_naf = nullptr;
        bool owns_naf = false, ready = false;
        int n_slots = 0;
        int info[4] = {0, 0, 0, 0};
    };
    SlpProgram slp_prog_[SLP_COUNT];
    std::mutex slp_build_mu_;
    std::vector<Fr8> w128_;
    const SlpProgram& slp_program(int id);
    void build_slp_program(int id);
    int pick_slp_program(int lanes) const;
    int slp_force_ = -1;
    int slp_fuse_min_ = 1024;
    int slp_info_[4] = {0, 0, 0, 0};
    Fr8 half_;

    int& cap_ = work_[0].cap;
    void *&d_coeffs_ = work_[0].coeffs, *&d_canon_ = work_[0].canon, *&d_scalars_ = work_[0].scalars, *&d_X_ = work_[0].X;
    int*& d_status_ = work_[0].status;
    uint8_t *d_in_ = nullptr, *d_cells_ = nullptr, *d_proofs_ = nullptr;
    int stage_cap_ = 0;
};

}
```

### rust-eth-kzg_amd/csrc/engine_prover.hip

```cpp
#include "engine_internal.hpp"

namespace kzg {

void Engine::set_profiling(bool on) { std::lock_guard<std::mutex> lk(marks_mu_); profiling_ = on; }
int Engine::mark_begin(int stage, hipStream_t st) {
    if (!profiling_) return -1;
    std::lock_guard<std::mutex> lk(marks_mu_);
    StageMark m{stage, 0, nullptr, nullptr};
    HIPCK(hipEventCreate(&m.a));
    HIPCK(hipEventCreate(&m.b));
    HIPCK(hipEventRecord(m.a, st));
    marks_.push_back(m);
    return (int)((marks_gen_ & 0x7ff) << 20) | ((int)marks_.size() - 1);
}
void Engine::mark_end(int mark, int launches, hipStream_t st) {
    if (mark < 0) return;
    std::lock_guard<std::mutex> lk(marks_mu_);
    const int idx = mark & 0xfffff;
    if (((mark >> 20) & 0x7ff) != (int)(marks_gen_ & 0x7ff) || idx >= (int)marks_.size()) return;
    marks_[idx].launches = launches;
    HIPCK(hipEventRecord(marks_[idx].b, st));
}
void Engine::get_stage_times(double* ms, uint64_t* launches) {
    std::lock_guard<std::mutex> lk(marks_mu_);
    for (int i = 0; i < ST_COUNT; i++) { ms[i] = 0; launches[i] = 0; }
    hipSetDevice(dev_);
    hipDeviceSynchronize();
    for (auto& m : marks_) {
        float t = 0;
        if (hipEventElapsedTime(&t, m.a, m.b) == hipSuccess) { ms[m.stage] += t; launches[m.stage] += m.launches; }
        hipEventDestroy(m.a);
        hipEventDestroy(m.b);
    }
    marks_.clear();
    marks_gen_++;
}

void Engine::ensure_workspace(int n) {
    ensure_workspace(work_[0], n);
    HIPCK(hipStreamWaitEvent(stream_, work_[0].done, 0));
}
void Engine::ensure_workspace(Work& w, int n, bool release) {
    if (n <= w.cap && !release) return;
    int cap = ((n + 63) / 64) * 64;
    void** ptrs[] = {&w.coeffs, &w.canon, &w.scalars, &w.X, (void**)&w.status};
    for (void** p : ptrs)
        if (*p) { HIPCK(hipFree(*p)); *p = nullptr; }
    w.cap = 0;
    if (release) {
        if (w.slp_arena) { HIPCK(hipFree(w.slp_arena)); w.slp_arena = nullptr; w.slp_arena_bytes = 0; }
        return;
    }
    HIPCK(hipMalloc(&w.coeffs, (size_t)cap * N_BLOB * sizeof(Fr)));
    if (&w == &work_[0]) HIPCK(hipMalloc(&w.canon, (size_t)cap * N_BLOB * sizeof(Fr)));
    HIPCK(hipMalloc(&w.scalars, (size_t)cap * 128 * 64 * sizeof(Fr)));
    HIPCK(hipMalloc(&w.X, (size_t)cap * 128 * launch::SIZEOF_JACS));
    HIPCK(hipMalloc(&w.status, (size_t)cap * sizeof(int)));
    w.cap = cap;
}
void Engine::ensure_staging(Work& w, int n) {
    if (n <= w.stage_cap) return;
    void* dev[] = {w.d_in, w.d_cells, w.d_proofs};
    for (void* p : dev)
        if (p) HIPCK(hipFree(p));
    void* pin[] = {w.h_in, w.h_cells, w.h_proofs, w.h_status};
    for (void* p : pin)
        if (p) HIPCK(hipHostFree(p));
    w.d_in = w.d_cells = w.d_proofs = w.h_in = w.h_cells = w.h_proofs = nullptr;
    w.h_status = nullptr;
    w.stage_cap = 0;
    HIPCK(hipMalloc(&w.d_in, (size_t)n * BYTES_PER_BLOB));
    HIPCK(hipMalloc(&w.d_cells, (size_t)n * N_CELLS * BYTES_PER_CELL));
    HIPCK(hipMalloc(&w.d_proofs, (size_t)n * N_CELLS * 48));
    HIPCK(hipHostMalloc(&w.h_in, (size_t)n * BYTES_PER_BLOB, hipHostMallocDefault));
    HIPCK(hipHostMalloc(&w.h_cells, (size_t)n * N_CELLS * BYTES_PER_CELL, hipHostMallocDefault));
    HIPCK(hipHostMalloc(&w.h_proofs, (size_t)n * N_CELLS * 48, hipHostMallocDefault));
    HIPCK(hipHostMalloc(&w.h_status, (size_t)n * sizeof(int), hipHostMallocDefault));
    w.stage_cap = n;
}
Work& Engine::lease_work(int first, int last) {
    std::unique_lock<std::mutex> lk(lease_mu_);
    for (;;) {
        for (int i = first; i <= last; i++)
            if (work_[i].mu.try_lock()) return work_[i];
        lease_cv_.wait_for(lk, std::chrono::milliseconds(2));
    }
}
void Engine::release_work(Work& w) {
    w.mu.unlock();
    lease_cv_.notify_one();
}

void Engine::launch_msm(const void* scalars, TableSel which, void* out, int n_groups, int n_slices, int out_stride,
                        int brp_bits, hipStream_t st, int out_fmt) {
    launch_msm(scalars, table_view(which), false, out, n_groups, n_slices, out_stride, brp_bits, st, out_fmt);
}
void Engine::launch_msm(const void* scalars, const TableView& tv, bool scalars_split, void* out, int n_groups, int n_slices,
                        int out_stride, int brp_bits, hipStream_t st, int out_fmt) {
    const SharedTable* main = tv.main.get();
    const SharedTable* next = tv.next.get();
    int ready = 0;
    if (next) ready = std::min(n_groups, next->ready_groups.load(std::memory_order_acquire));
    if (!scalars_split) launch::glv_split(const_cast<void*>(scalars), (size_t)n_groups * n_slices * 64, st);
    if (ready > 0) launch_msm_range(scalars, *next, 0, ready, out, n_groups, n_slices, out_stride, brp_bits, st, out_fmt);
    if (ready < n_groups) launch_msm_range(scalars, *main, ready, n_groups - ready, out, n_groups, n_slices, out_stride, brp_bits, st, out_fmt);
}
long Engine::msm_waves(long msms, int c) const {
    const long W = launch::glv_windows(c);
    if (msm_chunks_ > 0 || (msm_chunks_ < 0 && (msms * 4 + 63) / 64 >= (long)wave_slots_)) return msms * 4;
    if (msm_chunks_ < 0 && msm_split_ && (msms * 4 * W + 63) / 64 <= (long)wave_slots_ / 2) return (msms * 4 * W + 63) / 64;
    return (msms * 2 * W + 63) / 64;
}
void Engine::launch_msm_range(const void* scalars, const SharedTable& t, int g0, int gcnt, void* out, int n_groups, int n_slices,
                              int out_stride, int brp_bits, hipStream_t st, int out_fmt) {
    const launch::TabBlocks tb{(const void* const*)t.d_blocks, g0, gcnt};
    const int c = t.c;
    const long msms = (long)gcnt * n_slices;
    int mode = 1;
    if (n_slices <= FLAT_MSM_MAX_SLICES && circ_max_ > 0) mode = 0;
    else if (msm_chunks_ >= 0) mode = msm_chunks_ == 0 ? 1 : 2;
    else if (msm_split_ && (msms * 4 * launch::glv_windows(c) + 63) / 64 <= (long)wave_slots_ / 2) mode = 3;
    else if ((msms * 4 + 63) / 64 >= (long)wave_slots_) {
        mode = 2;
    }
    if (mode == 1 && msm_chunks_ < 0 && msm_split_) {
        const long per_slice = (long)gcnt * 2 * launch::glv_windows(c), slots = (long)wave_slots_ * 64, lanes = per_slice * n_slices;
        const int n_a = (int)(slots / per_slice);
        if (lanes > slots && lanes * 4 <= slots * 5 && n_a >= 1 && n_a < n_slices) {
            const size_t pt = out_fmt == launch::FMT_JACS ? launch::SIZEOF_JACS : launch::SIZEOF_JACQ;
            launch::msm_glv(c, 1, scalars, tb, out, n_groups, n_a, 64, out_stride, brp_bits, beta_, st, out_fmt);
            const int n_b = n_slices - n_a;
            launch::msm_glv(c, (n_b <= FLAT_MSM_MAX_SLICES && circ_max_ > 0) ? 0 : 3, (const char*)scalars + (size_t)n_a * n_groups * 64 * sizeof(Fr), tb,
                            (char*)out + (size_t)n_a * pt, n_groups, n_b, 64, out_stride, brp_bits, beta_, st, out_fmt);
            return;
        }
    }
    launch::msm_glv(c, mode, scalars, tb, out, n_groups, n_slices, 64, out_stride, brp_bits, beta_, st, out_fmt);
}

void Engine::g1_fft128_full(void* X, int stride, int inverse, hipStream_t st) {
    if (!inverse) {
        for (int half = 64; half >= 1; half >>= 1)
            launch::g1_fft_layer(X, stride, half, 128 / (2 * half), 0, 1, d_naf_, beta_, st);
    } else {
        for (int half = 1; half <= 64; half <<= 1)
            launch::g1_fft_layer(X, stride, half, 128 / (2 * half), 1, 0, d_naf_, beta_, st);
    }
}

int Engine::fk20_segs(int n) const { return (n > circ_max_ || circ_T_ > 129) ? 1 : n <= 2 ? 4 : n <= 4 ? 2 : 1; }
void Engine::run_proofs_from_coeffs(Work& w, int n, uint8_t* d_proofs, hipStream_t st, const TableView* tv_pre, ProofsPhase phase, int msm_cut) {
    const int bp = ((n + 63) / 64) * 64;
    const int segs = fk20_segs(n);
    const Fr8 two_segments[3] = {seg_shift_[1], seg_shift_[1], seg_shift_[1]};
    const bool linmap_mode = n > circ_max_;
    void* X = w.X;
    const SlpProgram* prog = nullptr;
    int mulc_coop_lanes = 0;
    if (linmap_mode) {
        int which = pick_slp_program(bp);
        if (slp_force_ < 0 && bp == 64 && n > 32 && launch::coop_points_max() > 0) which = SLP_DEPTH_456;
        mulc_coop_lanes = n <= 32 ? n : (bp == 64 && which == SLP_DEPTH_456) ? n : 0;
        prog = &slp_program(which);
        const size_t need = (size_t)prog->n_slots * bp * launch::SIZEOF_JACS;
        if (need > w.slp_arena_bytes) {
            if (w.slp_arena) { HIPCK(hipStreamSynchronize(st)); HIPCK(hipFree(w.slp_arena)); w.slp_arena = nullptr; w.slp_arena_bytes = 0; }
            HIPCK(hipMalloc(&w.slp_arena, need));
            w.slp_arena_bytes = need;
        }
        X = w.slp_arena;
    }
    constexpr int fmt = launch::FMT_JACS;
    constexpr size_t pt = launch::SIZEOF_JACS;
    const TableView tv = tv_pre ? *tv_pre : table_view(TAB_FK);
    if (!tv_pre) {
        const int mk1 = mark_begin(ST_FK20_SCALARS, st);
        launch::fk20_scalars(n, w.coeffs, w.scalars, d_w29_, linmap_mode ? half_ : inv128_, segs, segs == 2 ? two_segments : seg_shift_, st);
        mark_end(mk1, 1, st);
    }
    if (phase != PROOFS_ALL) {
        if (!tv_pre || !linmap_mode || segs != 1 || msm_cut <= 0 || msm_cut >= n || msm_cut % 64) throw std::logic_error("run_proofs_from_coeffs: bad MSM cut");
        if (phase == PROOFS_HEAD) {
            launch::g1_set_inf(X, (size_t)128 * bp, st, fmt);
            launch_msm(w.scalars, tv, true, X, 128, msm_cut, bp, 0, st, fmt);
            return;
        }
        launch_msm((char*)w.scalars + (size_t)msm_cut * 128 * 64 * sizeof(Fr), tv, true, (char*)X + (size_t)msm_cut * pt, 128, n - msm_cut, bp, 0, st, fmt);
    }
    if (phase == PROOFS_ALL) launch::g1_set_inf(X, (size_t)128 * bp, st, fmt);
    const int mk2 = mark_begin(ST_MSM_FIXED, st);
    if (phase == PROOFS_ALL) launch_msm(w.scalars, tv, true, X, 128, segs * n, bp, 0, st, fmt);
    mark_end(mk2, 1, st);
    if (linmap_mode) {
        const int mk3 = mark_begin(ST_G1_LINMAP, st);
        int n_launches = 0;
        for (auto& L : prog->launches)
            launch::g1_slp_launch(L.kind, w.slp_arena, bp, (const uint32_t*)prog->d_words + (size_t)L.first * 4, L.count, prog->d_naf, beta_, st, 0,
                                  mulc_coop_lanes, n);
        n_launches = (int)prog->launches.size();
        mark_end(mk3, n_launches, st);
        const int mk4 = mark_begin(ST_COMPRESS, st);
        launch::g1_compress((const char*)w.slp_arena + (size_t)128 * bp * pt, d_proofs, 128, bp, n, st, fmt);
        mark_end(mk4, 1, st);
        return;
    }
    if (n <= circ_max_) {
        if (!w.circ_table) HIPCK(hipMalloc(&w.circ_table, launch::g1_circ_table_bytes(circ_max_, circ_T_)));
        const int mk5 = mark_begin(ST_G1_IFFT, st);
        launch::g1_circ128(w.X, bp, n, segs, w.circ_table, circ_T_, d_circ_terms_, circ_per_lane_, beta_, st);
        mark_end(mk5, 2, st);
    } else throw std::logic_error("run_proofs_from_coeffs: a batch above the circulant form needs the compiled linear map");
    const int mk10 = mark_begin(ST_COMPRESS, st);
    launch::g1_compress(w.X, d_proofs, 128, bp, n, st, fmt);
    mark_end(mk10, 1, st);
}

void Engine::enqueue_compute(Work& w, int n, const uint8_t* d_blobs, uint8_t* d_cells, uint8_t* d_proofs, hipStream_t st,
                             hipEvent_t after_cells) {
    ensure_workspace(w, n);
    HIPCK(hipStreamWaitEvent(st, w.done, 0));
    HIPCK(hipMemsetAsync(w.status, 0, n * sizeof(int), st));
    const int mk11 = mark_begin(ST_BLOB_TO_COEFFS, st);
    launch::blob_to_coeffs(n, d_blobs, w.coeffs, nullptr, w.status, d_w29_, n_inv4096_, st);
    mark_end(mk11, 1, st);
    bool side = d_cells && d_proofs && n <= SIDE_CELLS_MAX && w.copy && !profiling_;
    if (side && n > FLAT_MSM_MAX_SLICES) {
        const long simds = wave_slots_ / 2, waves = msm_waves(128L * n, table_view(TAB_FK).c);
        if (waves > simds * 4 / 5 && waves <= simds) side = false;
    }
    const int segs = fk20_segs(n);
    const bool fused = d_cells && d_proofs && fused_scalars_ != 0 && (fused_scalars_ == 1 || (!side && segs == 1));
    if (fused) {
        const bool linmap_mode = n > circ_max_;
        const Fr8 two_segments[3] = {seg_shift_[1], seg_shift_[1], seg_shift_[1]};
        const TableView tv = table_view(TAB_FK);
        const int mk = mark_begin(ST_COEFFS_TO_CELLS, st);
        launch::coeffs_to_cells_scalars(n, w.coeffs, d_cells, w.scalars, d_blobs, w.status, d_w29_,
                                        (const char*)d_tapk_ + (linmap_mode ? 0 : (size_t)N_EXT * launch::SIZEOF_FR29), segs,
                                        segs == 2 ? two_segments : seg_shift_, st);
        mark_end(mk, 1, st);
        fused_launches_.fetch_add(1, std::memory_order_relaxed);
        if (after_cells) HIPCK(hipEventRecord(after_cells, st));
        run_proofs_from_coeffs(w, n, d_proofs, st, &tv);
        return;
    }
    if (side) {
        HIPCK(hipEventRecord(w.ev_coeffs, st));
        HIPCK(hipStreamWaitEvent(w.copy, w.ev_coeffs, 0));
        launch::coeffs_to_cells(n, w.coeffs, d_cells, d_w29_, w.copy);
        if (after_cells) HIPCK(hipEventRecord(after_cells, w.copy));
        HIPCK(hipEventRecord(w.ev_side, w.copy));
        run_proofs_from_coeffs(w, n, d_proofs, st);
        HIPCK(hipStreamWaitEvent(st, w.ev_side, 0));
        return;
    }
    if (d_cells) {
        const int mk12 = mark_begin(ST_COEFFS_TO_CELLS, st);
        launch::coeffs_to_cells(n, w.coeffs, d_cells, d_w29_, st);
        mark_end(mk12, 1, st);
    }
    if (after_cells) HIPCK(hipEventRecord(after_cells, st));
    if (d_proofs) run_proofs_from_coeffs(w, n, d_proofs, st);
}

int Engine::compute_cells_and_kzg_proofs_device(int n, const uint8_t* d_blobs, uint8_t* d_cells, uint8_t* d_proofs,
                                                int* h_status, hipStream_t st, bool sync) {
    if (n <= 0) return OK;
    Work* held = nullptr;
    try {
        HIPCK(hipSetDevice(dev_));
        Work& w = lease_work(1, NW - 1);
        held = &w;
        if (!st) {
            st = w.stream;
            HIPCK(hipEventRecord(w.ev_in, nullptr));
            HIPCK(hipStreamWaitEvent(st, w.ev_in, 0));
        }
        int sub = std::min(n, device_batch_max_);
        for (int b0 = 0; b0 < n;) {
            const int nb = std::min(sub, n - b0);
            try {
                enqueue_compute(w, nb, d_blobs + (size_t)b0 * BYTES_PER_BLOB, d_cells ? d_cells + (size_t)b0 * N_CELLS * BYTES_PER_CELL : nullptr,
                                d_proofs ? d_proofs + (size_t)b0 * N_CELLS * 48 : nullptr, st, nullptr);
            } catch (const HipError& e) {
                if (!e.out_of_memory() || sub <= 64) throw;
                (void)hipGetLastError();
                HIPCK(hipStreamSynchronize(st));
                ensure_workspace(w, 0, true);
                sub = std::max(64, ((sub / 2 + 63) / 64) * 64);
                continue;
            }
            if (h_status) HIPCK(hipMemcpyAsync(h_status + b0, w.status, nb * sizeof(int), hipMemcpyDeviceToHost, st));
            b0 += nb;
        }
        HIPCK(hipEventRecord(w.done, st));
        HIPCK(hipGetLastError());
        release_work(w);
        held = nullptr;
        if (sync || h_status) HIPCK(hipStreamSynchronize(st));
    } catch (const std::exception& e) {
        if (held) release_work(*held);
        set_error(e);
        return ERR_DEVICE;
    }
    return OK;
}

int Engine::blob_to_kzg_commitment_device(int n, const uint8_t* d_blobs, uint8_t* d_commitments, int* h_status,
                                          hipStream_t st, bool sync) {
    if (n <= 0) return OK;
    std::lock_guard<std::recursive_mutex> lk(mu_);
    if (n > device_batch_max_) {
        for (int b0 = 0; b0 < n; b0 += device_batch_max_) {
            const int nb = std::min(device_batch_max_, n - b0);
            const int rc = blob_to_kzg_commitment_device(nb, d_blobs + (size_t)b0 * BYTES_PER_BLOB, d_commitments + (size_t)b0 * 48,
                                                         h_status ? h_status + b0 : nullptr, st, sync);
            if (rc) return rc;
        }
        return OK;
    }
    try {
        HIPCK(hipSetDevice(dev_));
        if (!st) {
            st = stream_;
            HIPCK(hipEventRecord(work_[0].ev_in, nullptr));
            HIPCK(hipStreamWaitEvent(st, work_[0].ev_in, 0));
        }
        ensure_workspace(n);
        HIPCK(hipStreamWaitEvent(st, work_[0].done, 0));
        const int bp = ((n + 63) / 64) * 64;
        HIPCK(hipMemsetAsync(d_status_, 0, n * sizeof(int), st));
        launch::blob_to_coeffs(n, d_blobs, d_coeffs_, d_canon_, d_status_, d_w29_, n_inv4096_, st);
        launch::g1_set_inf(d_X_, (size_t)64 * bp, st, launch::FMT_JACS);
        launch_msm(d_canon_, TAB_SRS, d_X_, 64, n, bp, 0, st, launch::FMT_JACS);
        launch::g1_sum_positions(d_X_, 64, bp, n, st);
        launch::g1_compress(d_X_, d_commitments, 1, bp, n, st, launch::FMT_JACS);
        if (h_status) HIPCK(hipMemcpyAsync(h_status, d_status_, n * sizeof(int), hipMemcpyDeviceToHost, st));
        HIPCK(hipEventRecord(work_[0].done, st));
        HIPCK(hipGetLastError());
        if (sync || h_status) HIPCK(hipStreamSynchronize(st));
    } catch (const std::exception& e) {
        set_error(e);
        return ERR_DEVICE;
    }
    return OK;
}

HostPool* Engine::ensure_host_pool() {
    std::call_once(host_pool_once_, [this] {
        int t = 8;
        const unsigned hw = std::thread::hardware_concurrency();
        if (hw && (int)hw < 2 * t) t = (int)hw / 2 > 1 ? (int)hw / 2 : 1;
        if (knobs_.host_threads) t = knobs_.host_threads;
        host_pool_.reset(new HostPool(t, [d = dev_] { (void)hipSetDevice(d); }));
    });
    return host_pool_.get();
}

int Engine::compute_cells_and_kzg_proofs_host(int n, const uint8_t* const* blobs, uint8_t* const* const* cells,
                                              uint8_t* const* const* proofs, int* h_status) {
    if (n <= 0) return OK;
    constexpr int SUPER = 4096, SUB = 256, PART = 32;
    const bool threaded = n >= 32;
    const bool trace = knobs_.trace;
    const auto t_begin = std::chrono::steady_clock::now();
    auto now_ms = [&]() { return std::chrono::duration<double, std::milli>(std::chrono::steady_clock::now() - t_begin).count(); };
    const double slow_ms = knobs_.trace ? 50.0 : 0.0;
    double step_at[8] = {0};
    int n_steps = 0;
    auto step = [&]() { if (slow_ms > 0 && n_steps < 8) step_at[n_steps++] = now_ms(); };
    struct SlowReport {
        const double& limit; double* at; int& n; std::function<double()> now;
        ~SlowReport() {
            if (limit <= 0 || now() < limit) return;
            fprintf(stderr, "[host-batch] @%.0f ms: slow call, %.1f ms; steps (lease, enqueue sub-batches, enqueue proofs, events recorded, cells back, all back):", trace_clock_ms(), now());
            for (int i = 0; i < n; i++) fprintf(stderr, " %.1f", at[i]);
            fprintf(stderr, "\n");
        }
    } slow_report{slow_ms, step_at, n_steps, now_ms};
    Work* held = nullptr;
    std::atomic<int> failed{0};
    std::mutex err_mu;
    std::string err_text;
    auto fail = [&](const std::exception& e) {
        std::lock_guard<std::mutex> lk(err_mu);
        if (!failed.exchange(1)) err_text = e.what();
    };
    std::atomic<int> outstanding{0};
    auto nap = [] { std::this_thread::sleep_for(std::chrono::microseconds(30)); };
    auto drain = [&]() { while (outstanding.load(std::memory_order_acquire) > 0) nap(); };
    try {
        HIPCK(hipSetDevice(dev_));
        if (threaded) ensure_host_pool();
        Work& w = lease_work(1, NW - 1);
        held = &w;
        step();
        for (int s0 = 0; s0 < n && !failed.load(); s0 += SUPER) {
            const int ns = std::min(SUPER, n - s0);
            std::vector<int> cut{0};
            if (ns > SUB) cut.push_back(SUB / 4);
            if (ns > SUB) cut.push_back(SUB);
            while (cut.back() < ns) cut.push_back(std::min(ns, cut.back() + SUB));
            const int n_sub = (int)cut.size() - 1;
            ensure_workspace(w, ns);
            ensure_staging(w, ns);
            while ((int)w.sub_events.size() < 3 * n_sub) {
                hipEvent_t e;
                HIPCK(hipEventCreateWithFlags(&e, hipEventDisableTiming));
                w.sub_events.push_back(e);
            }
            HIPCK(hipStreamWaitEvent(w.stream, w.done, 0));
            HIPCK(hipMemsetAsync(w.status, 0, ns * sizeof(int), w.stream));
            std::vector<std::atomic<int>> gathered(n_sub);
            std::function<void(int, int, int)> scatter_cells;
            std::function<void(int, int)> scatter_proofs;
            struct Drain {
                std::function<void()> f;
                ~Drain() { f(); }
            } drain_on_exit{drain};
            for (int i = 0; i < n_sub; i++) {
                const int lo = cut[i], hi = cut[i + 1], parts = (hi - lo + PART - 1) / PART;
                gathered[i].store(threaded ? parts : 0, std::memory_order_relaxed);
                if (!threaded) {
                    for (int b = lo; b < hi; b++) memcpy(w.h_in + (size_t)b * BYTES_PER_BLOB, blobs[s0 + b], BYTES_PER_BLOB);
                    continue;
                }
                for (int p0 = lo; p0 < hi; p0 += PART) {
                    const int p1 = std::min(hi, p0 + PART);
                    outstanding.fetch_add(1, std::memory_order_relaxed);
                    host_pool_->submit([&, i, p0, p1, s0] {
                        for (int b = p0; b < p1; b++) memcpy(w.h_in + (size_t)b * BYTES_PER_BLOB, blobs[s0 + b], BYTES_PER_BLOB);
                        gathered[i].fetch_sub(1, std::memory_order_release);
                        outstanding.fetch_sub(1, std::memory_order_release);
                    });
                }
            }
            scatter_cells = [&](int i, int lo, int hi) {
                const hipError_t q = hipEventQuery(w.sub_events[2 * i + 1]);
                if (q == hipErrorNotReady) {
                    nap();
                    host_pool_->submit([&, i, lo, hi] { scatter_cells(i, lo, hi); });
                    return;
                }
                try {
                    HIPCK(q);
                    for (int b = lo; b < hi; b++) {
                        if (h_status) h_status[s0 + b] = w.h_status[b] ? ERR_SCALAR : OK;
                        if (w.h_status[b] || !cells) continue;
                        const uint8_t* src = w.h_cells + (size_t)b * N_CELLS * BYTES_PER_CELL;
                        for (int k = 0; k < N_CELLS; k++) memcpy(cells[s0 + b][k], src + (size_t)k * BYTES_PER_CELL, BYTES_PER_CELL);
                    }
                } catch (const std::exception& e) { fail(e); }
                outstanding.fetch_sub(1, std::memory_order_release);
            };
            const bool side = cells && proofs && ns <= circ_max_;
            const bool early_scalars = proofs && ns > circ_max_;
            const TableView tv_call = table_view(TAB_FK);
            constexpr int early_msm_blobs = 256;
            int msm_cut = 0;
            if (early_scalars && early_msm_blobs > 0 && ns >= 4 * early_msm_blobs)
                for (int c : cut)
                    if (!msm_cut && c >= early_msm_blobs && c % 64 == 0 && c < ns) msm_cut = c;
            for (int i = 0; i < n_sub; i++) {
                const int lo = cut[i], hi = cut[i + 1], nb = hi - lo;
                while (gathered[i].load(std::memory_order_acquire) > 0) std::this_thread::yield();
                HIPCK(hipMemcpyAsync(w.d_in + (size_t)lo * BYTES_PER_BLOB, w.h_in + (size_t)lo * BYTES_PER_BLOB, (size_t)nb * BYTES_PER_BLOB,
                                     hipMemcpyHostToDevice, w.copy));
                HIPCK(hipEventRecord(w.sub_events[2 * n_sub + i], w.copy));
                HIPCK(hipStreamWaitEvent(w.stream, w.sub_events[2 * n_sub + i], 0));
                launch::blob_to_coeffs(nb, w.d_in + (size_t)lo * BYTES_PER_BLOB, (char*)w.coeffs + (size_t)lo * N_BLOB * sizeof(Fr), nullptr,
                                       w.status + lo, d_w29_, n_inv4096_, w.stream);
                if (cells && !side)
                    launch::coeffs_to_cells(nb, (char*)w.coeffs + (size_t)lo * N_BLOB * sizeof(Fr),
                                            w.d_cells + (size_t)lo * N_CELLS * BYTES_PER_CELL, d_w29_, w.stream);
                HIPCK(hipEventRecord(w.sub_events[2 * i], w.stream));
                if (early_scalars)
                    launch::fk20_scalars(nb, (char*)w.coeffs + (size_t)lo * N_BLOB * sizeof(Fr), (char*)w.scalars + (size_t)lo * 128 * 64 * sizeof(Fr),
                                         d_w29_, half_, 1, seg_shift_, w.stream);
                if (msm_cut && hi == msm_cut) run_proofs_from_coeffs(w, ns, w.d_proofs, w.stream, &tv_call, PROOFS_HEAD, msm_cut);
                if (trace) fprintf(stderr, "[host-batch] sub-batch %d (%d blobs) enqueued at %.2f ms\n", i, nb, now_ms());
            }
            for (int i = 0; i < n_sub; i++) {
                const int lo = cut[i], hi = cut[i + 1], nb = hi - lo;
                HIPCK(hipStreamWaitEvent(w.copy, w.sub_events[2 * i], 0));
                if (side)
                    launch::coeffs_to_cells(nb, (char*)w.coeffs + (size_t)lo * N_BLOB * sizeof(Fr),
                                            w.d_cells + (size_t)lo * N_CELLS * BYTES_PER_CELL, d_w29_, w.copy);
                HIPCK(hipMemcpyAsync(w.h_status + lo, w.status + lo, (size_t)nb * sizeof(int), hipMemcpyDeviceToHost, w.copy));
                if (cells)
                    HIPCK(hipMemcpyAsync(w.h_cells + (size_t)lo * N_CELLS * BYTES_PER_CELL, w.d_cells + (size_t)lo * N_CELLS * BYTES_PER_CELL,
                                         (size_t)nb * N_CELLS * BYTES_PER_CELL, hipMemcpyDeviceToHost, w.copy));
                HIPCK(hipEventRecord(w.sub_events[2 * i + 1], w.copy));
                if (threaded) {
                    for (int p0 = lo; p0 < hi; p0 += PART) {
                        const int p1 = std::min(hi, p0 + PART);
                        outstanding.fetch_add(1, std::memory_order_relaxed);
                        host_pool_->submit([&, i, p0, p1] { scatter_cells(i, p0, p1); });
                    }
                }
            }
            step();
            if (proofs) {
                if (msm_cut) run_proofs_from_coeffs(w, ns, w.d_proofs, w.stream, &tv_call, PROOFS_TAIL, msm_cut);
                else run_proofs_from_coeffs(w, ns, w.d_proofs, w.stream, early_scalars ? &tv_call : nullptr);
                HIPCK(hipMemcpyAsync(w.h_proofs, w.d_proofs, (size_t)ns * N_CELLS * 48, hipMemcpyDeviceToHost, w.stream));
            }
            step();
            HIPCK(hipEventRecord(w.ev_done, w.stream));
            HIPCK(hipEventRecord(w.done, w.stream));
            HIPCK(hipGetLastError());
            step();
            if (!threaded) {
                HIPCK(hipEventSynchronize(w.sub_events[1]));
                for (int b = 0; b < ns; b++) {
                    if (h_status) h_status[s0 + b] = w.h_status[b] ? ERR_SCALAR : OK;
                    if (w.h_status[b] || !cells) continue;
                    const uint8_t* src = w.h_cells + (size_t)b * N_CELLS * BYTES_PER_CELL;
                    for (int k = 0; k < N_CELLS; k++) memcpy(cells[s0 + b][k], src + (size_t)k * BYTES_PER_CELL, BYTES_PER_CELL);
                }
            }
            step();
            HIPCK(hipEventSynchronize(w.ev_done));
            HIPCK(hipStreamSynchronize(w.copy));
            step();
            if (trace) fprintf(stderr, "[host-batch] proofs of %d blobs back at %.2f ms\n", ns, now_ms());
            if (proofs) {
                scatter_proofs = [&, s0](int lo, int hi) {
                    for (int b = lo; b < hi; b++) {
                        if (w.h_status[b]) continue;
                        const uint8_t* src = w.h_proofs + (size_t)b * N_CELLS * 48;
                        for (int k = 0; k < N_CELLS; k++) memcpy(proofs[s0 + b][k], src + (size_t)k * 48, 48);
                    }
                };
                if (threaded && ns >= 256) {
                    const int parts = 8;
                    for (int t = 1; t < parts; t++) {
                        outstanding.fetch_add(1, std::memory_order_relaxed);
                        host_pool_->submit([&, t] { scatter_proofs(t * ns / parts, (t + 1) * ns / parts); outstanding.fetch_sub(1, std::memory_order_release); });
                    }
                    scatter_proofs(0, ns / parts);
                } else scatter_proofs(0, ns);
            }
        }
        release_work(w);
        held = nullptr;
        if (trace) fprintf(stderr, "[host-batch] %d blobs delivered at %.2f ms\n", n, now_ms());
        if (failed.load()) throw std::runtime_error(err_text);
    } catch (const std::exception& e) {
        if (held) {
            (void)hipStreamSynchronize(held->stream);
            (void)hipStreamSynchronize(held->copy);
            drain();
            release_work(*held);
        }
        set_error(e);
        return ERR_DEVICE;
    }
    return OK;
}

int Engine::blob_to_kzg_commitment_host(int n, const uint8_t* const* blobs, uint8_t* const* out, int* h_status) {
    if (n <= 0) return OK;
    std::lock_guard<std::recursive_mutex> whole_call(mu_);
    uint8_t* d_out = nullptr;
    {
        std::lock_guard<std::recursive_mutex> lk(mu_);
        try {
            HIPCK(hipSetDevice(dev_));
            if (n > stage_cap_) {
                if (d_in_) { HIPCK(hipFree(d_in_)); HIPCK(hipFree(d_cells_)); HIPCK(hipFree(d_proofs_)); }
                HIPCK(hipMalloc(&d_in_, (size_t)n * BYTES_PER_BLOB));
                HIPCK(hipMalloc(&d_cells_, (size_t)n * N_CELLS * BYTES_PER_CELL));
                HIPCK(hipMalloc(&d_proofs_, (size_t)n * N_CELLS * 48));
                stage_cap_ = n;
            }
            for (int b = 0; b < n; b++)
                HIPCK(hipMemcpyAsync(d_in_ + (size_t)b * BYTES_PER_BLOB, blobs[b], BYTES_PER_BLOB, hipMemcpyHostToDevice, stream_));
            d_out = d_proofs_;
        } catch (const std::exception& e) {
            set_error(e);
            return ERR_DEVICE;
        }
    }
    std::vector<int> st(n);
    int rc = blob_to_kzg_commitment_device(n, d_in_, d_out, st.data(), stream_, true);
    if (rc) return rc;
    std::lock_guard<std::recursive_mutex> lk(mu_);
    try {
        std::vector<uint8_t> h((size_t)n * 48);
        HIPCK(hipMemcpy(h.data(), d_out, h.size(), hipMemcpyDeviceToHost));
        for (int b = 0; b < n; b++) {
            if (h_status) h_status[b] = st[b] ? ERR_SCALAR : OK;
            if (!st[b]) memcpy(out[b], h.data() + (size_t)b * 48, 48);
        }
    } catch (const std::exception& e) {
        set_error(e);
        return ERR_DEVICE;
    }
    return OK;
}

}
```

### rust-eth-kzg_amd/csrc/fr29_consts.hpp

```cpp
#pragma once
#include <stdint.h>
namespace kzg { namespace r29 {
constexpr uint32_t P[9] = {0x00000001u, 0x1ffffff8u, 0x1f96ffbfu, 0x1b4805ffu, 0x1d80553bu, 0x0c0404d0u, 0x1520cce7u, 0x0a6533afu, 0x0073eda7u};
constexpr uint32_t R2[9] = {0x0a71b3c0u, 0x1d32207eu, 0x1663d999u, 0x1c5abc93u, 0x03b58c44u, 0x0be37438u, 0x0829f771u, 0x1660139eu, 0x0027fd91u};
constexpr uint32_t ONE_PLAIN[9] = {0x00000001u, 0x00000000u, 0x00000000u, 0x00000000u, 0x00000000u, 0x00000000u, 0x00000000u, 0x00000000u, 0x00000000u};
constexpr uint32_t SUBK[6][9] = {
    {0x40000002u, 0x5fffffeeu, 0x5f2dff7du, 0x56900bfdu, 0x5b00aa75u, 0x5808099fu, 0x4a4199ccu, 0x54ca675du, 0x00e7db4cu},
    {0x40000004u, 0x5fffffdeu, 0x5e5bfefdu, 0x4d2017fdu, 0x560154edu, 0x50101341u, 0x5483339bu, 0x4994cebcu, 0x01cfb69bu},
    {0x40000008u, 0x5fffffbeu, 0x5cb7fdfdu, 0x5a402ffdu, 0x4c02a9dcu, 0x40202685u, 0x49066739u, 0x53299d7bu, 0x039f6d38u},
    {0x40000010u, 0x5fffff7eu, 0x596ffbfdu, 0x54805ffdu, 0x580553bbu, 0x40404d0cu, 0x520cce74u, 0x46533af8u, 0x073eda73u},
    {0x40000020u, 0x5ffffefeu, 0x52dff7fdu, 0x4900bffdu, 0x500aa779u, 0x40809a1bu, 0x44199ceau, 0x4ca675f3u, 0x0e7db4e8u},
    {0x40000040u, 0x5ffffdfeu, 0x45bfeffdu, 0x52017ffdu, 0x40154ef4u, 0x41013439u, 0x483339d6u, 0x594cebe8u, 0x1cfb69d2u}};
}}
```

### rust-eth-kzg_amd/csrc/fr29_ntt.hpp

```cpp
#pragma once
#include "fr29.hpp"

namespace kzg {

constexpr int NTT_N = 4096, NTT_W = 8192;

HD Fr29 fr29_twiddled(const Fr29& b, const Fr29* __restrict__ w29, int e) {
    return e ? fr29_mul(b, w29[e]) : fr29_partial_reduce(b);
}
template <class Elems>
HD void ntt4096_dit_inverse_unit(const Elems& m, const Fr29* __restrict__ w29, int h, int u) {
    const int j = u & (h - 1), i0 = ((u - j) << 2) + j;
    const int step_a = NTT_W / (2 * h), step_b = step_a >> 1;
    const int ea = (NTT_W - j * step_a) & (NTT_W - 1), eb0 = (NTT_W - j * step_b) & (NTT_W - 1), eb1 = NTT_W - (j + h) * step_b;
    const Fr29 x0 = m.load(i0), x1 = m.load(i0 + h), x2 = m.load(i0 + 2 * h), x3 = m.load(i0 + 3 * h);
    const Fr29 ta = fr29_twiddled(x1, w29, ea), tc = fr29_twiddled(x3, w29, ea);
    const Fr29 a0 = fr29_add<false>(x0, ta), a1 = fr29_sub2r<false>(x0, ta), a2 = fr29_add<false>(x2, tc), a3 = fr29_sub2r<false>(x2, tc);
    const Fr29 tb0 = fr29_twiddled(a2, w29, eb0), tb1 = fr29_mul(a3, w29[eb1]);
    m.store(i0, fr29_add<true>(a0, tb0));
    m.store(i0 + 2 * h, fr29_sub2r<true>(a0, tb0));
    m.store(i0 + h, fr29_add<true>(a1, tb1));
    m.store(i0 + 3 * h, fr29_sub2r<true>(a1, tb1));
}
template <class Elems>
HD void ntt4096_ct_forward_unit(const Elems& m, const Fr29* __restrict__ w29, int h, int log_m, int u) {
    const int j = u & (h - 1), blk = u / h, i0 = ((u - j) << 2) + j;
    unsigned rb = 0;
    for (int b = 0; b < log_m; b++) rb |= (((unsigned)blk >> b) & 1u) << (log_m - 1 - b);
    const int ea = (int)rb * (2 * h) * (NTT_W / NTT_N);
    const int eb0 = (int)rb * h * (NTT_W / NTT_N), eb1 = (int)(rb + (1u << log_m)) * h * (NTT_W / NTT_N);
    const Fr29 x0 = m.load(i0), x1 = m.load(i0 + h), x2 = m.load(i0 + 2 * h), x3 = m.load(i0 + 3 * h);
    const Fr29 ta = fr29_twiddled(x2, w29, ea), tc = fr29_twiddled(x3, w29, ea);
    const Fr29 a0 = fr29_add<false>(x0, ta), a2 = fr29_sub2r<false>(x0, ta), a1 = fr29_add<false>(x1, tc), a3 = fr29_sub2r<false>(x1, tc);
    const Fr29 tb0 = fr29_twiddled(a1, w29, eb0), tb1 = fr29_mul(a3, w29[eb1]);
    m.store(i0, fr29_add<true>(a0, tb0));
    m.store(i0 + h, fr29_sub2r<true>(a0, tb0));
    m.store(i0 + 2 * h, fr29_add<true>(a2, tb1));
    m.store(i0 + 3 * h, fr29_sub2r<true>(a2, tb1));
}

HD int fk20_tap_row(int e, int h) {
    const int q = e >> 6;
    int rb = 0;
    for (int b = 0; b < 6; b++) rb |= ((q >> b) & 1) << (5 - b);
    return 2 * rb + h;
}
HD int fk20_tap_column(int e) { return 63 - (e & 63); }
HD int fk20_tap_exponent(int e, int h) { return (64 * 65 * fk20_tap_row(e, h) + NTT_W - (e & 63) * h) & (NTT_W - 1); }
HD Fr29 fk20_tap_const(const Fr29* __restrict__ w29, const Fr29& scale_plain, int idx) {
    return fr29_reduce_once(fr29_mul(w29[fk20_tap_exponent(idx & (NTT_N - 1), idx >> 12)], scale_plain));
}
template <class Elems>
HD Fr29 fk20_tap_scalar(const Elems& m, const Fr29* __restrict__ tapk, int e, int h) {
    return fr29_mul(m.load(e), tapk[h * NTT_N + e]);
}

}
```

### rust-eth-kzg_amd/csrc/k_ntt.hip

```cpp
#include "engine.hpp"
#include "kcommon.hpp"
#include "fr29.hpp"
#include "fr29_ntt.hpp"
#include "glv.hpp"
#include "launch.hpp"

namespace kzg {

__device__ __forceinline__ Fr29 lds_load(const uint32_t* s, int idx) {
    Fr29 r;
#pragma unroll
    for (int l = 0; l < RL; l++) r.v[l] = s[l * N_BLOB + idx];
    return r;
}
__device__ __forceinline__ void lds_store(uint32_t* s, int idx, const Fr29& a) {
#pragma unroll
    for (int l = 0; l < RL; l++) s[l * N_BLOB + idx] = a.v[l];
}

struct LdsElems {
    uint32_t* s;
    __device__ __forceinline__ Fr29 load(int i) const { return lds_load(s, i); }
    __device__ __forceinline__ void store(int i, const Fr29& v) const { lds_store(s, i, v); }
};
__device__ __forceinline__ void dit_inverse_pass(uint32_t* s, const Fr29* __restrict__ w29, int h) {
    ntt4096_dit_inverse_unit(LdsElems{s}, w29, h, (int)threadIdx.x);
}
__device__ __forceinline__ void ntt4096_dit_inverse(uint32_t* s, const Fr29* __restrict__ w29) {
    dit_inverse_pass(s, w29, 1);
    __builtin_amdgcn_wave_barrier();
    dit_inverse_pass(s, w29, 4);
    __builtin_amdgcn_wave_barrier();
    dit_inverse_pass(s, w29, 16);
    __builtin_amdgcn_wave_barrier();
    dit_inverse_pass(s, w29, 64);
    __syncthreads();
    dit_inverse_pass(s, w29, 256);
    __syncthreads();
    dit_inverse_pass(s, w29, 1024);
    __builtin_amdgcn_wave_barrier();
}
__device__ __forceinline__ void ct_forward_pass(uint32_t* s, const Fr29* __restrict__ w29, int h, int log_m) {
    ntt4096_ct_forward_unit(LdsElems{s}, w29, h, log_m, (int)threadIdx.x);
}
__device__ __forceinline__ void ntt4096_ct_forward_head(uint32_t* s, const Fr29* __restrict__ w29) {
    __builtin_amdgcn_wave_barrier();
    ct_forward_pass(s, w29, 1024, 0);
    __syncthreads();
    ct_forward_pass(s, w29, 256, 2);
    __syncthreads();
    ct_forward_pass(s, w29, 64, 4);
}
__device__ __forceinline__ void ntt4096_ct_forward_tail(uint32_t* s, const Fr29* __restrict__ w29) {
    __builtin_amdgcn_wave_barrier();
    ct_forward_pass(s, w29, 16, 6);
    __builtin_amdgcn_wave_barrier();
    ct_forward_pass(s, w29, 4, 8);
    __builtin_amdgcn_wave_barrier();
    ct_forward_pass(s, w29, 1, 10);
    __syncthreads();
}
__device__ __forceinline__ void ntt4096_ct_forward(uint32_t* s, const Fr29* __restrict__ w29) {
    ntt4096_ct_forward_head(s, w29);
    ntt4096_ct_forward_tail(s, w29);
}
__device__ __forceinline__ Fr fr_words_of(const Fr29& canonical) {
    Fr r;
    fr29_to_words(r.v, canonical);
    return r;
}
__device__ __forceinline__ void store_split_scalar(Fr* __restrict__ at, const Fr29& x) {
    Fr k = fr_words_of(fr29_reduce_once(x));
    uint32_t h[8];
    glv_split_balanced(k, h);
#pragma unroll
    for (int l = 0; l < 8; l++) k.v[l] = h[l];
    *at = k;
}

struct NttConsts {
    Fr29 ninv_to_sat;
    Fr29 ninv_plain;
    Fr29 one;
};
__global__ __launch_bounds__(1024) void k_blob_to_coeffs(const uint8_t* __restrict__ blobs, Fr* __restrict__ coeffs,
                                                        Fr* __restrict__ canon_out, int* __restrict__ status,
                                                        const Fr29* __restrict__ w29, NttConsts K) {
    extern __shared__ uint32_t s[];
    const int b = blockIdx.x, tid = threadIdx.x;
    const uint8_t* blob = blobs + (size_t)b * BYTES_PER_BLOB;
    bool bad = false;
    for (int e = tid; e < N_BLOB; e += 1024) {
        const Fr x = load_fr_be(blob + 32 * e);
        bad |= geq_mod<FrParams>(x.v);
        lds_store(s, e, fr29_from_plain(x));
    }
    if (bad) atomicOr(&status[b], 1);
    __syncthreads();
    ntt4096_dit_inverse(s, w29);
    for (int e = tid; e < N_BLOB; e += 1024) {
        const Fr29 x = lds_load(s, e);
        coeffs[(size_t)b * N_BLOB + e] = fr_words_of(fr29_reduce_once(fr29_mul(x, K.ninv_to_sat)));
        if (canon_out) canon_out[(size_t)b * N_BLOB + e] = fr_words_of(fr29_reduce_once(fr29_mul(x, K.ninv_plain)));
    }
}

__global__ __launch_bounds__(1024) void k_coeffs_to_cells(const Fr* __restrict__ coeffs, uint8_t* __restrict__ cells,
                                                         const Fr29* __restrict__ w29) {
    extern __shared__ uint32_t s[];
    const int b = blockIdx.x, h = blockIdx.y, tid = threadIdx.x;
    for (int e = tid; e < N_BLOB; e += 1024) {
        Fr29 c = fr29_from_fr_mont(coeffs[(size_t)b * N_BLOB + e]);
        if (h && e) c = fr29_mul(c, w29[e]);
        lds_store(s, e, c);
    }
    __syncthreads();
    ntt4096_ct_forward(s, w29);
    uint8_t* out = cells + ((size_t)b * N_EXT + (size_t)h * N_BLOB) * 32;
    const Fr29 one_plain = fr29_const(r29::ONE_PLAIN);
    for (int e = tid; e < N_BLOB; e += 1024)
        store_fr_be(out + 32 * e, fr_words_of(fr29_reduce_once(fr29_mul(lds_load(s, e), one_plain))));
}

struct SegShifts { Fr29 p[3]; };
__global__ __launch_bounds__(256) void k_fk20_scalars(const Fr* __restrict__ coeffs, Fr* __restrict__ scalars,
                                                      const Fr29* __restrict__ w29, Fr29 scale , int n,
                                                      int segs, SegShifts sh) {
    __shared__ uint32_t s[4][RL][128];
    const int b = blockIdx.x >> 4, wv = threadIdx.x >> 6, lane = threadIdx.x & 63;
    const int i = ((blockIdx.x & 15) << 2) + wv;
    const Fr* a = coeffs + (size_t)b * N_BLOB;
    uint32_t(*sv)[128] = s[wv];
    {
        Fr29 lo, hi;
#pragma unroll
        for (int l = 0; l < RL; l++) lo.v[l] = hi.v[l] = 0;
        if (lane == 0) lo = fr29_mul(fr29_from_plain(a[N_BLOB - 1 - i]), scale);
        else hi = fr29_mul(fr29_from_plain(a[64 * lane - 1 - i]), scale);
#pragma unroll
        for (int l = 0; l < RL; l++) { sv[l][lane] = lo.v[l]; sv[l][64 + lane] = hi.v[l]; }
    }
    __builtin_amdgcn_wave_barrier();
    int log_m = 0;
    for (int half = 64; half >= 1; half >>= 1, log_m++) {
        const int j = lane & (half - 1), blk = lane / half;
        const int i0 = ((lane - j) << 1) + j, i1 = i0 + half;
        const int e = log_m ? (int)(__brev((unsigned)blk) >> (32 - log_m)) * half * (N_EXT / 128) : 0;
        Fr29 x, y;
#pragma unroll
        for (int l = 0; l < RL; l++) { x.v[l] = sv[l][i0]; y.v[l] = sv[l][i1]; }
        const Fr29 t = e ? fr29_mul(y, w29[e]) : fr29_partial_reduce(y);
        Fr29 sum = fr29_add<false>(x, t), d = fr29_sub2r<false>(x, t);
        if ((log_m & 1) || half == 1) { fr29_normalise(sum); fr29_normalise(d); }
#pragma unroll
        for (int l = 0; l < RL; l++) { sv[l][i0] = sum.v[l]; sv[l][i1] = d.v[l]; }
        __builtin_amdgcn_wave_barrier();
    }
    auto emit = [&](size_t at, const Fr29& x) {
        store_split_scalar(&scalars[at], fr29_partial_reduce(x));
    };
    for (int q = lane; q < 128; q += 64) {
        Fr29 x;
#pragma unroll
        for (int l = 0; l < RL; l++) x.v[l] = sv[l][q];
        const int j = __brev((unsigned)q) >> 25;
        emit(((size_t)b * 128 + j) * 64 + i, x);
        for (int sg = 1; sg < segs; sg++)
            emit(((size_t)(sg * n + b) * 128 + j) * 64 + i, fr29_mul(x, sh.p[sg - 1]));
    }
}

__global__ __launch_bounds__(1024) void k_coeffs_to_cells_scalars(const Fr* __restrict__ coeffs, uint8_t* __restrict__ cells,
                                                                 Fr* __restrict__ scalars, const uint8_t* __restrict__ blobs,
                                                                 const int* __restrict__ status, const Fr29* __restrict__ w29,
                                                                 const Fr29* __restrict__ tapk, int n, int segs, SegShifts sh) {
    extern __shared__ uint32_t s[];
    const int b = blockIdx.x, h = blockIdx.y, tid = threadIdx.x;
    for (int e = tid; e < N_BLOB; e += 1024) {
        Fr29 c = fr29_from_fr_mont(coeffs[(size_t)b * N_BLOB + e]);
        if (h && e) c = fr29_mul(c, w29[e]);
        lds_store(s, e, c);
    }
    __syncthreads();
    ntt4096_ct_forward_head(s, w29);
    const int e0 = ((tid >> 6) << 8) + (tid & 63);
#pragma unroll 1
    for (int k = 0; k < 4; k++) {
        const int e = e0 + 64 * k;
        const Fr29 x = fk20_tap_scalar(LdsElems{s}, tapk, e, h);
        const size_t at = (size_t)fk20_tap_row(e, h) * 64 + fk20_tap_column(e);
        store_split_scalar(&scalars[(size_t)b * N_EXT + at], x);
        for (int sg = 1; sg < segs; sg++)
            store_split_scalar(&scalars[(size_t)(sg * n + b) * N_EXT + at], fr29_mul(x, sh.p[sg - 1]));
    }
    uint8_t* out = cells + ((size_t)b * N_EXT + (size_t)h * N_BLOB) * 32;
    if (h == 0 && blobs && status[b] == 0) {
        const uint4* src = reinterpret_cast<const uint4*>(blobs + (size_t)b * BYTES_PER_BLOB);
        uint4* dst = reinterpret_cast<uint4*>(out);
        for (int k = tid; k < BYTES_PER_BLOB / 16; k += 1024) dst[k] = src[k];
        return;
    }
    ntt4096_ct_forward_tail(s, w29);
    const Fr29 one_plain = fr29_const(r29::ONE_PLAIN);
    for (int e = tid; e < N_BLOB; e += 1024)
        store_fr_be(out + 32 * e, fr_words_of(fr29_reduce_once(fr29_mul(lds_load(s, e), one_plain))));
}
__global__ void k_fk20_tap_consts(const Fr29* __restrict__ w29, Fr29 scale_plain, Fr29* __restrict__ out) {
    const int idx = blockIdx.x * blockDim.x + threadIdx.x;
    if (idx < 2 * N_BLOB) out[idx] = fk20_tap_const(w29, scale_plain, idx);
}

#ifdef KZG_TEST_HOOKS
__global__ __launch_bounds__(1024) void k_test_ntt4096(const uint8_t* in, uint8_t* out, const Fr29* w29, NttConsts K, int inverse_dit) {
    extern __shared__ uint32_t s[];
    for (int e = threadIdx.x; e < N_BLOB; e += 1024) lds_store(s, e, fr29_from_plain(load_fr_be(in + 32 * e)));
    __syncthreads();
    if (inverse_dit) ntt4096_dit_inverse(s, w29);
    else ntt4096_ct_forward(s, w29);
    for (int e = threadIdx.x; e < N_BLOB; e += 1024) {
        const Fr29 c = lds_load(s, e);
        store_fr_be(out + 32 * e, fr_words_of(fr29_reduce_once(fr29_mul(c, inverse_dit ? K.ninv_plain : K.one))));
    }
}
__global__ void k_test_scalars_be(const uint8_t* in, Fr* out, size_t n) {
    size_t i = (size_t)blockIdx.x * blockDim.x + threadIdx.x;
    if (i < n) out[i] = load_fr_be(in + 32 * i);
}
template <class F>
__global__ void k_test_field_mul(const uint8_t* a, const uint8_t* b, uint8_t* out, int n) {
    int i = blockIdx.x * blockDim.x + threadIdx.x;
    if (i >= n) return;
    constexpr int NB = F::N * 4;
    F x, y;
    for (int k = 0; k < F::N; k++) {
        const uint8_t* pa = a + (size_t)i * NB + 4 * k;
        const uint8_t* pb = b + (size_t)i * NB + 4 * k;
        x.v[F::N - 1 - k] = ((uint32_t)pa[0] << 24) | ((uint32_t)pa[1] << 16) | ((uint32_t)pa[2] << 8) | pa[3];
        y.v[F::N - 1 - k] = ((uint32_t)pb[0] << 24) | ((uint32_t)pb[1] << 16) | ((uint32_t)pb[2] << 8) | pb[3];
    }
    F z = from_mont(mul(to_mont(x), to_mont(y)));
    for (int k = 0; k < F::N; k++) {
        uint32_t w = z.v[F::N - 1 - k];
        uint8_t* po = out + (size_t)i * NB + 4 * k;
        po[0] = (uint8_t)(w >> 24); po[1] = (uint8_t)(w >> 16); po[2] = (uint8_t)(w >> 8); po[3] = (uint8_t)w;
    }
}

#endif

namespace launch {
void preload_k_ntt() {
    hipFuncAttributes a;
    (void)hipFuncGetAttributes(&a, reinterpret_cast<const void*>(&k_blob_to_coeffs));
}
static Fr as_fr(const Fr8& x) { Fr r; for (int i = 0; i < 8; i++) r.v[i] = x.v[i]; return r; }

constexpr size_t LDS_NTT29 = (size_t)N_BLOB * RL * 4;
void init_attributes() {
    hipFuncSetAttribute(reinterpret_cast<const void*>(k_blob_to_coeffs), hipFuncAttributeMaxDynamicSharedMemorySize, (int)LDS_NTT29);
    hipFuncSetAttribute(reinterpret_cast<const void*>(k_coeffs_to_cells), hipFuncAttributeMaxDynamicSharedMemorySize, (int)LDS_NTT29);
    hipFuncSetAttribute(reinterpret_cast<const void*>(k_coeffs_to_cells_scalars), hipFuncAttributeMaxDynamicSharedMemorySize, (int)LDS_NTT29);
#ifdef KZG_TEST_HOOKS
    hipFuncSetAttribute(reinterpret_cast<const void*>(k_test_ntt4096), hipFuncAttributeMaxDynamicSharedMemorySize, (int)LDS_NTT29);
#endif
}
static Fr29 fr29_mont_of(const Fr& y_mont) {
    Fr c32 = zero<FrParams>();
    c32.v[0] = 32;
    return fr29_from_plain(mul(y_mont, to_mont(c32)));
}
static Fr29 fr29_mont_of(const Fr8& y_mont) { return fr29_mont_of(as_fr(y_mont)); }
static Fr29 fr29_int32x_of(const Fr8& s_mont) {
    Fr c32 = zero<FrParams>();
    c32.v[0] = 32;
    return fr29_from_plain(from_mont(mul(as_fr(s_mont), to_mont(c32))));
}
static NttConsts ntt_consts(const Fr8& n_inv_mont) {
    NttConsts K;
    K.ninv_to_sat = fr29_mont_of(to_mont(as_fr(n_inv_mont)));
    K.ninv_plain = fr29_mont_of(n_inv_mont);
    K.one = fr29_mont_of(one<FrParams>());
    return K;
}
void ntt_twiddles29(const void* w8192_mont_host , void* out_host ) {
    const Fr* w = (const Fr*)w8192_mont_host;
    Fr29* o = (Fr29*)out_host;
    for (int k = 0; k < N_EXT; k++) o[k] = fr29_mont_of(*(const Fr8*)&w[k]);
}
void blob_to_coeffs(int n, const uint8_t* blobs, void* coeffs, void* canon, int* status, const void* w29, const Fr8& n_inv, hipStream_t st) {
    k_blob_to_coeffs<<<n, 1024, LDS_NTT29, st>>>(blobs, (Fr*)coeffs, (Fr*)canon, status, (const Fr29*)w29, ntt_consts(n_inv));
}
void coeffs_to_cells(int n, const void* coeffs, uint8_t* cells, const void* w29, hipStream_t st) {
    k_coeffs_to_cells<<<dim3(n, 2), 1024, LDS_NTT29, st>>>((const Fr*)coeffs, cells, (const Fr29*)w29);
}
void fk20_scalars(int n, const void* coeffs, void* scalars, const void* w29, const Fr8& inv128, int segs, const Fr8* seg_shifts,
                  hipStream_t st) {
    SegShifts sh;
    for (int i = 0; i < 3; i++) sh.p[i] = fr29_mont_of(seg_shifts[i]);
    k_fk20_scalars<<<n * 16, 256, 0, st>>>((const Fr*)coeffs, (Fr*)scalars, (const Fr29*)w29, fr29_int32x_of(inv128), n, segs, sh);
}
void fk20_tap_consts(const void* w29, const Fr8& scale, void* out, hipStream_t st) {
    k_fk20_tap_consts<<<2 * N_BLOB / 256, 256, 0, st>>>((const Fr29*)w29, fr29_from_plain(from_mont(as_fr(scale))), (Fr29*)out);
}
void coeffs_to_cells_scalars(int n, const void* coeffs, uint8_t* cells, void* scalars, const uint8_t* blobs, const int* status, const void* w29,
                             const void* tapk, int segs, const Fr8* seg_shifts, hipStream_t st) {
    const uintptr_t pb = (uintptr_t)blobs, pc = (uintptr_t)cells;
    const bool apart = pb + (size_t)n * BYTES_PER_BLOB <= pc || pc + (size_t)n * N_EXT * 32 <= pb;
    if (!status || ((pb | pc) & 15) || !apart) blobs = nullptr;
    SegShifts sh;
    for (int i = 0; i < 3; i++) sh.p[i] = fr29_mont_of(seg_shifts[i]);
    k_coeffs_to_cells_scalars<<<dim3(n, 2), 1024, LDS_NTT29, st>>>((const Fr*)coeffs, cells, (Fr*)scalars, blobs, status, (const Fr29*)w29,
                                                                   (const Fr29*)tapk, n, segs, sh);
}
#ifdef KZG_TEST_HOOKS
void test_ntt4096(const uint8_t* in, uint8_t* out, const void* w29, const Fr8& n_inv, int inverse_dit, hipStream_t st) {
    k_test_ntt4096<<<1, 1024, LDS_NTT29, st>>>(in, out, (const Fr29*)w29, ntt_consts(n_inv), inverse_dit);
}
void test_scalars_be(const uint8_t* in, void* out, size_t n, hipStream_t st) {
    k_test_scalars_be<<<(unsigned)((n + 255) / 256), 256, 0, st>>>(in, (Fr*)out, n);
}
void test_field_mul(const uint8_t* a, const uint8_t* b, uint8_t* out, int n, int is_fp, hipStream_t st) {
    if (is_fp) k_test_field_mul<Fp><<<(n + 63) / 64, 64, 0, st>>>(a, b, out, n);
    else k_test_field_mul<Fr><<<(n + 63) / 64, 64, 0, st>>>(a, b, out, n);
}
#endif
}
}
```

### rust-eth-kzg_amd/csrc/knobs.hpp

```cpp
#pragma once
#include <cstdlib>
#include <cstring>
#include <string>
#include <vector>

namespace kzg {

struct Knobs {
    int device = 0;
    std::vector<int> devices;
    double table_budget_gb = 0;
    int glv_window = 0;
    bool progressive = true;
    int host_threads = 0;
    int serial_lanes = 0;
    bool trace = false;
    int msm_chunks = -1, slp_program = -1, pip_shift_min = 0, fused_scalars = -1;
    bool vm_search = true, vm_fold = true, verify_combine = true, msm_split = true;
    std::string fault;
    int device_batch_max = 0;

    static Knobs from_env() {
        Knobs k;
        auto num = [](const char* name, int lo, int hi, int& out) {
            if (const char* s = getenv(name)) { const int v = atoi(s); if (v >= lo && v <= hi) out = v; }
        };
        auto flag = [](const char* name, bool& out) {
            if (const char* s = getenv(name)) out = atoi(s) != 0;
        };
        num("ETH_KZG_AMD_DEVICE", 0, 4095, k.device);
        if (const char* s = getenv("ETH_KZG_AMD_DEVICES")) {
            if (!strcmp(s, "all") || !strcmp(s, "ALL")) k.devices.push_back(-1);
            else
                for (const char* p = s; *p;) {
                    char* end = nullptr;
                    const long v = strtol(p, &end, 10);
                    if (end == p) break;
                    if (v >= 0 && v <= 4095 && k.devices.size() < 64) k.devices.push_back((int)v);
                    p = *end == ',' ? end + 1 : end;
                    if (*end && *end != ',') break;
                }
        }
        if (const char* s = getenv("ETH_KZG_AMD_TABLE_GB")) {
            if (!strcmp(s, "max") || !strcmp(s, "MAX")) k.table_budget_gb = -1;
            else if (atof(s) > 0) k.table_budget_gb = atof(s);
        }
        num("ETH_KZG_AMD_GLV_WINDOW", 8, 16, k.glv_window);
        flag("ETH_KZG_AMD_PROGRESSIVE", k.progressive);
        num("ETH_KZG_AMD_HOST_THREADS", 1, 64, k.host_threads);
        num("ETH_KZG_AMD_SERIAL_LANES", 1, 16, k.serial_lanes);
        k.trace = getenv("ETH_KZG_AMD_TRACE") != nullptr;
        num("ETH_KZG_AMD_MSM_CHUNKS", 0, 4, k.msm_chunks);
        num("ETH_KZG_AMD_SLP_PROGRAM", 0, 15, k.slp_program);
        num("ETH_KZG_AMD_PIP_SHIFT_MIN", 1, 1 << 24, k.pip_shift_min);
        flag("ETH_KZG_AMD_VM_SEARCH", k.vm_search);
        flag("ETH_KZG_AMD_VM_FOLD", k.vm_fold);
        flag("ETH_KZG_AMD_VERIFY_COMBINE", k.verify_combine);
        flag("ETH_KZG_AMD_MSM_SPLIT", k.msm_split);
        num("ETH_KZG_AMD_FUSED_SCALARS", 0, 1, k.fused_scalars);
        if (const char* s = getenv("ETH_KZG_AMD_FAULT")) k.fault = s;
        num("ETH_KZG_AMD_DEVICE_BATCH_MAX", 64, 1 << 20, k.device_batch_max);
        return k;
    }
};

}
```

### rust-eth-kzg_amd/csrc/launch.hpp

```cpp
#pragma once
#include <hip/hip_runtime.h>
#include <cstddef>
#include <cstdint>

namespace kzg {
struct Fr8;
struct Fp12w;
namespace launch {

void init_attributes();
void preload_code_objects();

constexpr size_t SIZEOF_FR29 = 36;
void ntt_twiddles29(const void* w8192_mont_host , void* out_host );
void blob_to_coeffs(int n, const uint8_t* blobs, void* coeffs , void* canon , int* status,
                    const void* w29, const Fr8& n_inv, hipStream_t st);
void coeffs_to_cells(int n, const void* coeffs, uint8_t* cells, const void* w29, hipStream_t st);
void fk20_scalars(int n, const void* coeffs, void* scalars, const void* w29, const Fr8& inv128, int segs, const Fr8* seg_shifts,
                  hipStream_t st);
void fk20_tap_consts(const void* w29, const Fr8& scale, void* out , hipStream_t st);
void coeffs_to_cells_scalars(int n, const void* coeffs, uint8_t* cells, void* scalars, const uint8_t* blobs, const int* status, const void* w29,
                             const void* tapk, int segs, const Fr8* seg_shifts, hipStream_t st);
void test_ntt4096(const uint8_t* in, uint8_t* out, const void* w29, const Fr8& n_inv, int inverse_dit, hipStream_t st);
void test_scalars_be(const uint8_t* in, void* out, size_t n, hipStream_t st);
void test_field_mul(const uint8_t* a, const uint8_t* b, uint8_t* out, int n, int is_fp, hipStream_t st);
int test_op_info(int op, int* in_words, int* out_words, int* device_only, const char** name);
int test_op_host(int op, int n, const int32_t* in, int32_t* out);
int test_op_device(int op, int n, const int32_t* d_in, int32_t* d_out, hipStream_t st);
constexpr int TABLE_FINDING_WORDS = 5;
constexpr size_t SIZEOF_AUDIT_OUT = 24;
void table_audit_device(const void* const* blocks, const void* bases, int c, int n_groups, int nb, void* out, hipStream_t st);
void table_audit_host(const void* const* blocks, const void* bases, int c, int n_groups, int nb, unsigned long long* visited,
                      unsigned long long* n_findings, int32_t* findings, int max_findings);

struct TabBlocks {
    const void* const* blocks;
    int g0, gcnt;
};
constexpr int glv_windows(int c) { return (128 + c - 1) / c; }
constexpr int glv_lower_windows(int c) { return (glv_windows(c) + 1) / 2; }
constexpr int glv_base_bits(int c) { return 128 / glv_windows(c); }
constexpr int glv_wide_windows(int c) { return 128 - glv_windows(c) * glv_base_bits(c); }
constexpr int glv_window_bits(int c, int w) { return glv_base_bits(c) + (w < glv_wide_windows(c) ? 1 : 0); }
constexpr int glv_window_lo(int c, int w) { return w * glv_base_bits(c) + (w < glv_wide_windows(c) ? w : glv_wide_windows(c)); }
constexpr size_t glv_entries_per_base(int c, int w0, int w1) {
    size_t n = 0;
    for (int w = w0; w < w1; w++) n += (size_t)1 << (glv_window_bits(c, w) - 1);
    return n;
}
constexpr int GLV_WIDTHS[] = {16, 15, 14, 12, 8};
bool glv_width_supported(int c);
void glv_split(void* scalars, size_t n, hipStream_t st);
constexpr int FMT_JACQ = 0, FMT_JACS = 1;
void msm_glv(int c, int mode, const void* scalars, const TabBlocks& table, void* out , int n_groups, int n_slices, int nb, int out_stride,
             int brp_bits, const Fp12w& beta, hipStream_t st, int out_fmt);
#ifdef TABS_STRIDE_128
constexpr size_t SIZEOF_TABP = 128;
#else
constexpr size_t SIZEOF_TABP = 96;
#endif
size_t table_glv_entries(int c, int n_groups, int nb);
size_t table_glv_side_bytes(int c, int n_groups, int nb);
bool build_table_glv(int c, const void* bases, void* const* blocks, void* scratch, void* side, int n_groups, int nb, int* err, hipStream_t st);

void g1_fft_layer(void* X, int stride, int half, int tw_step, int inverse, int mode, const void* tw, const Fp12w& beta,
                  hipStream_t st);

void g1_slp_launch(int kind, void* arena, int stride, const uint32_t* words, int count, const void* naf, const Fp12w& beta,
                   hipStream_t st, int lanes = 0 ,
                   int coop_lanes = 0 ,
                   int n_active = 0 );

void g1_set_inf(void* X, size_t n, hipStream_t st, int fmt);
int coop_points_max();
void spin(uint64_t wall_clock_ticks, hipStream_t st);
void g1_compress(const void* X, uint8_t* out, int n_pos, int stride, int n_slices, hipStream_t st, int fmt);
void g1_sum_positions(void* X , int n_pos, int stride, int n_slices, hipStream_t st);
void g1_decompress(const uint8_t* in, void* out , int* status, int n, int subgroup_check, const Fp12w& beta,
                   hipStream_t st);
void g1_decompress2(const uint8_t* in0, void* out0, int* status0, int n0, const uint8_t* in1, void* out1, int* status1, int n1,
                    const Fp12w& beta, hipStream_t st);
void g1_decode2(const uint8_t* in0, void* out0, int* status0, int n0, const uint8_t* in1, void* out1, int* status1, int n1,
                const Fp12w& beta, hipStream_t st);
void g1_subgroup2(const void* pts0, int* status0, int n0, const void* pts1, int* status1, int n1, const Fp12w& beta, hipStream_t st);
void fk20_srs_vectors(const void* srs, void* X, hipStream_t st);
void fk20_gather_bases(const void* X, void* bases, hipStream_t st);
void test_load_points(const uint8_t* in, void* X, int n_lanes, int stride, hipStream_t st);
void test_recompress(const void* pts, uint8_t* out, int n, hipStream_t st);

constexpr int TWIDDLE_WNAF_W = 5;
constexpr int TWIDDLE_WORDS = 33;
constexpr int CIRC_LANES = 256;
size_t g1_circ_table_bytes(int n, int T);
void g1_circ128(void* X , int stride, int n, int segs, void* D, int T, const void* terms, int per_lane, const Fp12w& beta, hipStream_t st);
void init_attributes_verify();
void cells_to_fr(const uint8_t* cells, void* evals, const int* slot_of, int* status, const int* status_of, const int* src_of, int n,
                 hipStream_t st);
void rec_vanishing_poly(const uint32_t* present, const void* w8192, void* zp, int* deg, int R, hipStream_t st);
void rec_vanishing(const void* zp, const int* deg, const void* w8192, const Fr8& seven64, void* zeval, void* zcinv, int R,
                   hipStream_t st);
void verify_scalars(const Fr8* pow_table24, int k0, const int* cell_idx, const void* w8192, void* rp_mont, void* s1, void* s2,
                    int n, hipStream_t st);
void verify_weights(const void* rp_mont, const int* row, void* weights, int n, int m, hipStream_t st);
void interp(const void* evals, const int* cell_idx, const void* rp_mont, const void* w8192, const Fr8& inv64, void* partial,
            int nblocks, void* out_neg_canon, int n, hipStream_t st);
void interp_cells(const void* evals, const int* cell_idx, const void* w8192, const Fr8& inv64, void* coef, int n, hipStream_t st);
void interp_sum(const void* coef, const void* rp_mont, void* partial, int nblocks, void* out_neg_canon, int n, hipStream_t st);
size_t pip_shift_workspace_bytes(int n_max);
void pip_shift_prepare(const void* points, int n_pts, int n_max, void* workspace, const Fp12w& beta, hipStream_t st);
void pip_shift_prepare_and_subgroup(const void* points, int n_pts, int n_max, void* workspace, const void* pts0, int* status0, int n0,
                                    const void* pts1, int* status1, int n1, const Fp12w& beta, hipStream_t st);
void msm_pippenger2_shifted(const void* sc0, int n0, const void* sc1, int n1, int n_max, void* workspace, void* out_jacq2,
                            hipStream_t st);
size_t pip_workspace_bytes(int n_max);
void copy_affine(const void* src, void* dst, int n, hipStream_t st);
void msm_pippenger2(const void* points, const void* sc0, int n0, const void* sc1, int n1, void* workspace, void* out_affine2,
                    const Fp12w& beta, hipStream_t st);
void rec_dit_half(int R, const void* V, const void* fac, void* T, const void* w8192, hipStream_t st);
void rec_dit_last(int R, const void* T, const void* shift, const Fr8& n_inv, void* U, void* coeffs, int* status,
                  const void* w8192, int final_pass, hipStream_t st);
void rec_dif_half(int R, const void* U, const void* fac, void* V, const void* w8192, hipStream_t st);

void vm_scalars(const void* pow_tables , const int* batch_of, const int* pos_in_batch, const int* cell_idx, const void* w8192,
                void* rp_mont, void* s1, void* s2, int n, hipStream_t st);
void vm_weights(const void* rp_mont, const int* row, const int* row_batch, const int* cell_start, void* weights, int m, hipStream_t st);
void vm_interp_sum(const void* coef, const void* rp_mont, const int* cell_start, void* out_neg_canon, int n_batches, hipStream_t st);
void vm_mul(const void* pts, const void* s1, const void* s2, const void* wts, void* prod, int n, int m, const Fp12w& beta, hipStream_t st);
void vm_mul_small(const void* pts, const void* s1, const void* s2, const void* wts, const void* isc, const void* srs, void* prod, int n, int m,
                  int n_batches, int* status, const Fp12w& beta, hipStream_t st);
void vm_reduce_small(const void* prod, const int* cell_start, const int* row_start, void* out, int n, int m, int n_batches, hipStream_t st);
void vm_reduce(const void* prod, const void* icommit, const int* cell_start, const int* row_start, void* out , int n,
               int n_batches, hipStream_t st);
void vm_fold(const void* sums, const uint32_t* rho, void* prod, void* out2, int n_batches, const Fp12w& beta, hipStream_t st);
void vm_fold_ranges(const void* prod, const int* ranges , void* out , int n_ranges, hipStream_t st);

void quotient_by_linear(int n, const void* coeffs, const void* z_mont, void* quotient, void* y_out, hipStream_t st);
void fr_from_be32(int n, const uint8_t* in, void* out_mont, int* bad, bool reduce, hipStream_t st);
void fr_to_be32(int n, const void* canon , uint8_t* out, hipStream_t st);
void status_4844(int n, const int* blob_bad, const int* z_bad, const int* g1_bad, int* out, hipStream_t st);

void sha256_many(int n, const uint8_t* prefix, uint32_t prefix_len, const uint8_t* body, size_t body_stride, uint32_t body_len,
                 const uint8_t* tail, size_t tail_stride, uint32_t tail_len, uint8_t* out, hipStream_t st);

constexpr size_t SIZEOF_FR = 32, SIZEOF_G1AFFINE = 96, SIZEOF_G1JAC = 144;
constexpr size_t SIZEOF_JACS = 156;
constexpr size_t SIZEOF_AFFQ = 112, SIZEOF_JACQ = 168;

}
}
```

Measured before the change: 40030.

## Fuse blob-to-coeffs, cells and FK20 scalars into a single one-pass kernel

Adds a kernel that reads blobs once, runs the inverse NTT, emits the even FK20 tap scalars mid-transform, then applies a precomputed coset twist and runs the forward NTT to write extension cells and odd-tap scalars. This replaces the separate blob_to_coeffs launch and its coefficient buffer round trip through global memory. The odd-half scalars come from a precomputed twist table instead of a second block dimension. The trade-offs are one 1024-thread block per blob doing serial work that was previously split across two blocks, extra constant tables, and an aliasing check that falls back to the old path.

```diff
diff --git a/include/c_eth_kzg_test_hooks.h b/include/c_eth_kzg_test_hooks.h
--- a/include/c_eth_kzg_test_hooks.h
+++ b/include/c_eth_kzg_test_hooks.h
@@ -15,6 +15,8 @@
 
 int eth_kzg_amd_test_prover_scalars(const DASContext *ctx, int n, const uint8_t *blobs, uint32_t *scalars, uint64_t max_words,
                                     uint64_t *n_words, uint8_t *cells, uint8_t *proofs, int32_t *status, int32_t *fused_launches);
+
+int eth_kzg_amd_test_one_pass_launches(const DASContext *ctx, uint64_t *launches);
 
 int eth_kzg_amd_test_sha256_many(const DASContext *ctx, uint64_t n, const uint8_t *prefix, uint64_t prefix_len, const uint8_t *d_body,
                                  uint64_t body_stride, uint64_t body_len, const uint8_t *d_tail, uint64_t tail_stride, uint64_t tail_len,
diff --git a/rust-eth-kzg_amd/__init__.py b/rust-eth-kzg_amd/__init__.py
--- a/rust-eth-kzg_amd/__init__.py
+++ b/rust-eth-kzg_amd/__init__.py
@@ -61,7 +61,7 @@
     "eth_kzg_amd_test_table_info", "eth_kzg_amd_test_table_audit", "eth_kzg_amd_test_table_read", "eth_kzg_amd_test_table_audit_buffer",
     "eth_kzg_amd_test_sha256_many", "eth_kzg_amd_test_verify_msm",
     "eth_kzg_amd_test_verify_cells_partial_device", "eth_kzg_amd_test_verify_blob_batch_inputs", "eth_kzg_amd_test_rs_decode",
-    "eth_kzg_amd_test_prover_scalars", "eth_kzg_amd_test_verify_many_sums",
+    "eth_kzg_amd_test_prover_scalars", "eth_kzg_amd_test_verify_many_sums", "eth_kzg_amd_test_one_pass_launches",
 ]
 
 _lib = None
@@ -174,6 +174,7 @@
         "eth_kzg_amd_test_verify_blob_batch_inputs": [P, U64, C.c_int, P, P, P, P, P],
         "eth_kzg_amd_test_rs_decode": [P, C.c_int, P, P, P, C.c_int, P, P, P, P, P, P],
         "eth_kzg_amd_test_prover_scalars": [P, C.c_int, P, P, U64, P, P, P, P, P],
+        "eth_kzg_amd_test_one_pass_launches": [P, P],
         "eth_kzg_amd_test_verify_many_sums": [P, U64, P, P, P, P, P, P, P, P, P, P, P, P, P, P, P, P, U64, P],
     }.items():
         if hasattr(lib, name):
diff --git a/rust-eth-kzg_amd/csrc/c_api_hooks.cpp b/rust-eth-kzg_amd/csrc/c_api_hooks.cpp
--- a/rust-eth-kzg_amd/csrc/c_api_hooks.cpp
+++ b/rust-eth-kzg_amd/csrc/c_api_hooks.cpp
@@ -34,6 +34,11 @@
                                     uint8_t* cells, uint8_t* proofs, int32_t* status, int32_t* fused_launches) {
     if (!blobs || !scalars || !n_words || !cells || !proofs || !status || !fused_launches) return kzg::ERR_INPUT;
     return eng(ctx)->test_prover_scalars(n, blobs, scalars, max_words, n_words, cells, proofs, status, fused_launches);
+}
+int eth_kzg_amd_test_one_pass_launches(const DASContext* ctx, uint64_t* launches) {
+    if (!launches) return kzg::ERR_INPUT;
+    *launches = eng(ctx)->test_one_pass_launches();
+    return 0;
 }
 int eth_kzg_amd_test_g1_decompress(const DASContext* ctx, const uint8_t* in, int n, int subgroup_check, int32_t* status,
                                    uint8_t* out) {
diff --git a/rust-eth-kzg_amd/csrc/engine.hip b/rust-eth-kzg_amd/csrc/engine.hip
--- a/rust-eth-kzg_amd/csrc/engine.hip
+++ b/rust-eth-kzg_amd/csrc/engine.hip
@@ -192,6 +192,7 @@
     vm_search_ = knobs_.vm_search;
     msm_split_ = knobs_.msm_split;
     fused_scalars_ = knobs_.fused_scalars;
+    one_pass_ = knobs_.one_pass;
     if (knobs_.pip_shift_min >= 1) pip_shift_min_ = knobs_.pip_shift_min;
 #ifdef KZG_CIRC_MAX
     circ_max_ = KZG_CIRC_MAX;
@@ -316,7 +317,7 @@
     host_pool_.reset();
     vm_pool_.reset();
     stage_pool_.reset();
-    void* ptrs[] = {d_w8192_, d_w29_, d_tapk_, d_naf_, d_srs_, d_fk_bases_, d_in_, d_cells_, d_proofs_, d_coset_, d_coset_inv_, d_circ_terms_, d_4844_};
+    void* ptrs[] = {d_w8192_, d_w29_, d_tapk_, d_tapk_even_, d_twist_, d_naf_, d_srs_, d_fk_bases_, d_in_, d_cells_, d_proofs_, d_coset_, d_coset_inv_, d_circ_terms_, d_4844_};
     for (void* p : ptrs)
         if (p) hipFree(p);
     for (SlpProgram& P : slp_prog_) {
@@ -427,6 +428,11 @@
     HIPCK(hipMalloc(&d_tapk_, (size_t)2 * N_EXT * launch::SIZEOF_FR29));
     launch::fk20_tap_consts(d_w29_, half_, d_tapk_, stream_);
     launch::fk20_tap_consts(d_w29_, inv128_, (char*)d_tapk_ + (size_t)N_EXT * launch::SIZEOF_FR29, stream_);
+    HIPCK(hipMalloc(&d_tapk_even_, (size_t)2 * N_BLOB * launch::SIZEOF_FR29));
+    launch::fk20_tap_even_consts(d_w29_, half_, d_tapk_even_, stream_);
+    launch::fk20_tap_even_consts(d_w29_, inv128_, (char*)d_tapk_even_ + (size_t)N_BLOB * launch::SIZEOF_FR29, stream_);
+    HIPCK(hipMalloc(&d_twist_, (size_t)N_BLOB * launch::SIZEOF_FR29));
+    launch::fr_twist_consts(d_w29_, d_twist_, stream_);
     HIPCK(hipGetLastError());
 }
 
diff --git a/rust-eth-kzg_amd/csrc/engine.hpp b/rust-eth-kzg_amd/csrc/engine.hpp
--- a/rust-eth-kzg_amd/csrc/engine.hpp
+++ b/rust-eth-kzg_amd/csrc/engine.hpp
@@ -169,6 +169,7 @@
     int test_fixed_msm(const uint8_t* scalars_be, int n_msm, uint8_t* out_compressed);
     int test_prover_scalars(int n, const uint8_t* blobs, uint32_t* scalars, uint64_t max_words, uint64_t* n_words, uint8_t* cells, uint8_t* proofs,
                             int32_t* status, int32_t* fused_launches);
+    uint64_t test_one_pass_launches() const { return one_pass_launches_.load(); }
     int test_g1_decompress(const uint8_t* in, int n, int subgroup_check, int* h_status, uint8_t* out_recompressed);
     int test_field_mul(const uint8_t* a, const uint8_t* b, uint8_t* out, int n, int is_fp);
     int test_op(int op, int n, const int32_t* in, int32_t* out);
@@ -327,6 +328,8 @@
     int msm_chunks_ = -1;
     int fused_scalars_ = -1;
     std::atomic<uint64_t> fused_launches_{0};
+    int one_pass_ = -1;
+    std::atomic<uint64_t> one_pass_launches_{0};
     bool msm_split_ = true;
     hipStream_t stream_ = nullptr;
     std::recursive_mutex mu_;
@@ -342,6 +345,8 @@
     void* d_srs_ = nullptr;
     void* d_fk_bases_ = nullptr;
     BufferPool dev_pool_{false}, pin_pool_{true};
+    void* d_tapk_even_ = nullptr;
+    void* d_twist_ = nullptr;
     void* d_tapk_ = nullptr;
     Fr8 n_inv4096_, inv128_;
 
diff --git a/rust-eth-kzg_amd/csrc/engine_prover.hip b/rust-eth-kzg_amd/csrc/engine_prover.hip
--- a/rust-eth-kzg_amd/csrc/engine_prover.hip
+++ b/rust-eth-kzg_amd/csrc/engine_prover.hip
@@ -220,9 +220,6 @@
     ensure_workspace(w, n);
     HIPCK(hipStreamWaitEvent(st, w.done, 0));
     HIPCK(hipMemsetAsync(w.status, 0, n * sizeof(int), st));
-    const int mk11 = mark_begin(ST_BLOB_TO_COEFFS, st);
-    launch::blob_to_coeffs(n, d_blobs, w.coeffs, nullptr, w.status, d_w29_, n_inv4096_, st);
-    mark_end(mk11, 1, st);
     bool side = d_cells && d_proofs && n <= SIDE_CELLS_MAX && w.copy && !profiling_;
     if (side && n > FLAT_MSM_MAX_SLICES) {
         const long simds = wave_slots_ / 2, waves = msm_waves(128L * n, table_view(TAB_FK).c);
@@ -230,9 +227,30 @@
     }
     const int segs = fk20_segs(n);
     const bool fused = d_cells && d_proofs && fused_scalars_ != 0 && (fused_scalars_ == 1 || (!side && segs == 1));
+    const bool one_pass = d_cells && d_proofs && fused_scalars_ != 0 && one_pass_ != 0 && (one_pass_ == 1 || (!side && segs == 1));
+    const bool linmap_mode = n > circ_max_;
+    const Fr8 two_segments[3] = {seg_shift_[1], seg_shift_[1], seg_shift_[1]};
+    if (one_pass) {
+        const TableView tv = table_view(TAB_FK);
+        const int mk = mark_begin(ST_COEFFS_TO_CELLS, st);
+        const size_t scale_at = linmap_mode ? 0 : 1;
+        const bool launched = launch::blob_to_cells_scalars(n, d_blobs, d_cells, w.scalars, w.status, d_w29_,
+                                                            (const char*)d_tapk_even_ + scale_at * N_BLOB * launch::SIZEOF_FR29,
+                                                            (const char*)d_tapk_ + scale_at * N_EXT * launch::SIZEOF_FR29, d_twist_, segs,
+                                                            segs == 2 ? two_segments : seg_shift_, st);
+        mark_end(mk, launched ? 1 : 0, st);
+        if (launched) {
+            fused_launches_.fetch_add(1, std::memory_order_relaxed);
+            one_pass_launches_.fetch_add(1, std::memory_order_relaxed);
+            if (after_cells) HIPCK(hipEventRecord(after_cells, st));
+            run_proofs_from_coeffs(w, n, d_proofs, st, &tv);
+            return;
+        }
+    }
+    const int mk11 = mark_begin(ST_BLOB_TO_COEFFS, st);
+    launch::blob_to_coeffs(n, d_blobs, w.coeffs, nullptr, w.status, d_w29_, n_inv4096_, st);
+    mark_end(mk11, 1, st);
     if (fused) {
-        const bool linmap_mode = n > circ_max_;
-        const Fr8 two_segments[3] = {seg_shift_[1], seg_shift_[1], seg_shift_[1]};
         const TableView tv = table_view(TAB_FK);
         const int mk = mark_begin(ST_COEFFS_TO_CELLS, st);
         launch::coeffs_to_cells_scalars(n, w.coeffs, d_cells, w.scalars, d_blobs, w.status, d_w29_,
diff --git a/rust-eth-kzg_amd/csrc/fr29_consts.hpp b/rust-eth-kzg_amd/csrc/fr29_consts.hpp
--- a/rust-eth-kzg_amd/csrc/fr29_consts.hpp
+++ b/rust-eth-kzg_amd/csrc/fr29_consts.hpp
@@ -4,6 +4,8 @@
 constexpr uint32_t P[9] = {0x00000001u, 0x1ffffff8u, 0x1f96ffbfu, 0x1b4805ffu, 0x1d80553bu, 0x0c0404d0u, 0x1520cce7u, 0x0a6533afu, 0x0073eda7u};
 constexpr uint32_t R2[9] = {0x0a71b3c0u, 0x1d32207eu, 0x1663d999u, 0x1c5abc93u, 0x03b58c44u, 0x0be37438u, 0x0829f771u, 0x1660139eu, 0x0027fd91u};
 constexpr uint32_t ONE_PLAIN[9] = {0x00000001u, 0x00000000u, 0x00000000u, 0x00000000u, 0x00000000u, 0x00000000u, 0x00000000u, 0x00000000u, 0x00000000u};
+constexpr uint32_t NINV_R2[9] = {0x1cfca71cu, 0x1333d31bu, 0x18d7020cu, 0x12ecea43u, 0x07067c9au, 0x1395d1e7u, 0x16e99f80u, 0x1e98e193u, 0x0058c473u};
+constexpr uint32_t INV64_R2[9] = {0x1f29c6cfu, 0x0cf4c881u, 0x09d98f66u, 0x02716af2u, 0x1c0ed631u, 0x18af8dd0u, 0x0f20a7ddu, 0x08d9804eu, 0x00009ff6u};
 constexpr uint32_t SUBK[6][9] = {
     {0x40000002u, 0x5fffffeeu, 0x5f2dff7du, 0x56900bfdu, 0x5b00aa75u, 0x5808099fu, 0x4a4199ccu, 0x54ca675du, 0x00e7db4cu},
     {0x40000004u, 0x5fffffdeu, 0x5e5bfefdu, 0x4d2017fdu, 0x560154edu, 0x50101341u, 0x5483339bu, 0x4994cebcu, 0x01cfb69bu},
diff --git a/rust-eth-kzg_amd/csrc/fr29_ntt.hpp b/rust-eth-kzg_amd/csrc/fr29_ntt.hpp
--- a/rust-eth-kzg_amd/csrc/fr29_ntt.hpp
+++ b/rust-eth-kzg_amd/csrc/fr29_ntt.hpp
@@ -55,4 +55,20 @@
     return fr29_mul(m.load(e), tapk[h * NTT_N + e]);
 }
 
+HD int fk20_tap_even_row(int e) { return fk20_tap_row(e, 0); }
+HD int fk20_tap_even_exponent(int e) {
+    const int j = fk20_tap_even_row(e);
+    return (64 * 65 * j + NTT_W - (e & 63) * j) & (NTT_W - 1);
 }
+HD Fr29 fk20_tap_even_const(const Fr29* __restrict__ w29, const Fr29& scale_plain, int e) {
+    return fr29_reduce_once(fr29_mul(fr29_mul(w29[fk20_tap_even_exponent(e)], scale_plain), fr29_const(r29::INV64_R2)));
+}
+template <class Elems>
+HD Fr29 fk20_tap_even_scalar(const Elems& m, const Fr29* __restrict__ tapk_even, int e) {
+    return fr29_mul(m.load(e), tapk_even[e]);
+}
+HD Fr29 fr_twist_const(const Fr29* __restrict__ w29, int e) {
+    return fr29_reduce_once(fr29_mul(w29[e], fr29_const(r29::NINV_R2)));
+}
+
+}
diff --git a/rust-eth-kzg_amd/csrc/k_ntt.hip b/rust-eth-kzg_amd/csrc/k_ntt.hip
--- a/rust-eth-kzg_amd/csrc/k_ntt.hip
+++ b/rust-eth-kzg_amd/csrc/k_ntt.hip
@@ -23,41 +23,59 @@
     __device__ __forceinline__ Fr29 load(int i) const { return lds_load(s, i); }
     __device__ __forceinline__ void store(int i, const Fr29& v) const { lds_store(s, i, v); }
 };
+template <bool FRESH>
+__device__ __forceinline__ int pass_unit() {
+    int u = (int)threadIdx.x;
+    if (FRESH) asm volatile("" : "+v"(u));
+    return u;
+}
+template <bool FRESH = false>
 __device__ __forceinline__ void dit_inverse_pass(uint32_t* s, const Fr29* __restrict__ w29, int h) {
-    ntt4096_dit_inverse_unit(LdsElems{s}, w29, h, (int)threadIdx.x);
+    ntt4096_dit_inverse_unit(LdsElems{s}, w29, h, pass_unit<FRESH>());
+}
+template <bool FRESH = false>
+__device__ __forceinline__ void ntt4096_dit_inverse_head(uint32_t* s, const Fr29* __restrict__ w29) {
+    dit_inverse_pass<FRESH>(s, w29, 1);
+    __builtin_amdgcn_wave_barrier();
+    dit_inverse_pass<FRESH>(s, w29, 4);
+    __builtin_amdgcn_wave_barrier();
+    dit_inverse_pass<FRESH>(s, w29, 16);
+}
+template <bool FRESH = false>
+__device__ __forceinline__ void ntt4096_dit_inverse_tail(uint32_t* s, const Fr29* __restrict__ w29) {
+    __builtin_amdgcn_wave_barrier();
+    dit_inverse_pass<FRESH>(s, w29, 64);
+    __syncthreads();
+    dit_inverse_pass<FRESH>(s, w29, 256);
+    __syncthreads();
+    dit_inverse_pass<FRESH>(s, w29, 1024);
+    __builtin_amdgcn_wave_barrier();
 }
 __device__ __forceinline__ void ntt4096_dit_inverse(uint32_t* s, const Fr29* __restrict__ w29) {
-    dit_inverse_pass(s, w29, 1);
-    __builtin_amdgcn_wave_barrier();
-    dit_inverse_pass(s, w29, 4);
-    __builtin_amdgcn_wave_barrier();
-    dit_inverse_pass(s, w29, 16);
-    __builtin_amdgcn_wave_barrier();
-    dit_inverse_pass(s, w29, 64);
-    __syncthreads();
-    dit_inverse_pass(s, w29, 256);
-    __syncthreads();
-    dit_inverse_pass(s, w29, 1024);
-    __builtin_amdgcn_wave_barrier();
-}
+    ntt4096_dit_inverse_head(s, w29);
+    ntt4096_dit_inverse_tail(s, w29);
+}
+template <bool FRESH = false>
 __device__ __forceinline__ void ct_forward_pass(uint32_t* s, const Fr29* __restrict__ w29, int h, int log_m) {
-    ntt4096_ct_forward_unit(LdsElems{s}, w29, h, log_m, (int)threadIdx.x);
-}
+    ntt4096_ct_forward_unit(LdsElems{s}, w29, h, log_m, pass_unit<FRESH>());
+}
+template <bool FRESH = false>
 __device__ __forceinline__ void ntt4096_ct_forward_head(uint32_t* s, const Fr29* __restrict__ w29) {
     __builtin_amdgcn_wave_barrier();
-    ct_forward_pass(s, w29, 1024, 0);
-    __syncthreads();
-    ct_forward_pass(s, w29, 256, 2);
-    __syncthreads();
-    ct_forward_pass(s, w29, 64, 4);
-}
+    ct_forward_pass<FRESH>(s, w29, 1024, 0);
+    __syncthreads();
+    ct_forward_pass<FRESH>(s, w29, 256, 2);
+    __syncthreads();
+    ct_forward_pass<FRESH>(s, w29, 64, 4);
+}
+template <bool FRESH = false>
 __device__ __forceinline__ void ntt4096_ct_forward_tail(uint32_t* s, const Fr29* __restrict__ w29) {
     __builtin_amdgcn_wave_barrier();
-    ct_forward_pass(s, w29, 16, 6);
-    __builtin_amdgcn_wave_barrier();
-    ct_forward_pass(s, w29, 4, 8);
-    __builtin_amdgcn_wave_barrier();
-    ct_forward_pass(s, w29, 1, 10);
+    ct_forward_pass<FRESH>(s, w29, 16, 6);
+    __builtin_amdgcn_wave_barrier();
+    ct_forward_pass<FRESH>(s, w29, 4, 8);
+    __builtin_amdgcn_wave_barrier();
+    ct_forward_pass<FRESH>(s, w29, 1, 10);
     __syncthreads();
 }
 __device__ __forceinline__ void ntt4096_ct_forward(uint32_t* s, const Fr29* __restrict__ w29) {
@@ -205,6 +223,67 @@
     for (int e = tid; e < N_BLOB; e += 1024)
         store_fr_be(out + 32 * e, fr_words_of(fr29_reduce_once(fr29_mul(lds_load(s, e), one_plain))));
 }
+
+__global__ __launch_bounds__(1024) void k_blob_to_cells_scalars(const uint8_t* __restrict__ blobs, uint8_t* __restrict__ cells,
+                                                               Fr* __restrict__ scalars, int* __restrict__ status,
+                                                               const Fr29* __restrict__ w29, const Fr29* __restrict__ tapk_even,
+                                                               const Fr29* __restrict__ tapk, const Fr29* __restrict__ twist, int n,
+                                                               int segs, SegShifts sh) {
+    extern __shared__ uint32_t s[];
+    const int b = blockIdx.x, tid = threadIdx.x;
+    const uint8_t* blob = blobs + (size_t)b * BYTES_PER_BLOB;
+    uint8_t* out = cells + (size_t)b * N_EXT * 32;
+    bool bad = false;
+#pragma unroll 1
+    for (int e = tid; e < N_BLOB; e += 1024) {
+        const Fr x = load_fr_be(blob + 32 * e);
+        bad |= geq_mod<FrParams>(x.v);
+        const Fr29 p = fr29_from_plain(x);
+        lds_store(s, e, p);
+        store_fr_be(out + 32 * e, fr_words_of(fr29_reduce_once(fr29_partial_reduce(p))));
+    }
+    if (bad) atomicOr(&status[b], 1);
+    __syncthreads();
+    ntt4096_dit_inverse_head<true>(s, w29);
+    auto emit = [&](size_t at, const Fr29& x) {
+        store_split_scalar(&scalars[(size_t)b * N_EXT + at], x);
+        for (int sg = 1; sg < segs; sg++)
+            store_split_scalar(&scalars[(size_t)(sg * n + b) * N_EXT + at], fr29_mul(x, sh.p[sg - 1]));
+    };
+    {
+        const int e0 = ((tid >> 4) << 6) + (tid & 15);
+#pragma unroll 1
+        for (int k = 0; k < 4; k++) {
+            const int e = e0 + 16 * k;
+            emit((size_t)fk20_tap_even_row(e) * 64 + fk20_tap_column(e), fk20_tap_even_scalar(LdsElems{s}, tapk_even, e));
+        }
+    }
+    ntt4096_dit_inverse_tail<true>(s, w29);
+#pragma unroll 1
+    for (int e = tid; e < N_BLOB; e += 1024) lds_store(s, e, fr29_mul(lds_load(s, e), twist[e]));
+    ntt4096_ct_forward_head<true>(s, w29);
+    {
+        const int e0 = ((tid >> 6) << 8) + (tid & 63);
+#pragma unroll 1
+        for (int k = 0; k < 4; k++) {
+            const int e = e0 + 64 * k;
+            emit((size_t)fk20_tap_row(e, 1) * 64 + fk20_tap_column(e), fk20_tap_scalar(LdsElems{s}, tapk, e, 1));
+        }
+    }
+    ntt4096_ct_forward_tail<true>(s, w29);
+    const Fr29 one_plain = fr29_const(r29::ONE_PLAIN);
+#pragma unroll 1
+    for (int e = tid; e < N_BLOB; e += 1024)
+        store_fr_be(out + 32 * (N_BLOB + e), fr_words_of(fr29_reduce_once(fr29_mul(lds_load(s, e), one_plain))));
+}
+__global__ void k_fk20_tap_even_consts(const Fr29* __restrict__ w29, Fr29 scale_plain, Fr29* __restrict__ out) {
+    const int e = blockIdx.x * blockDim.x + threadIdx.x;
+    if (e < N_BLOB) out[e] = fk20_tap_even_const(w29, scale_plain, e);
+}
+__global__ void k_fr_twist_consts(const Fr29* __restrict__ w29, Fr29* __restrict__ out) {
+    const int e = blockIdx.x * blockDim.x + threadIdx.x;
+    if (e < N_BLOB) out[e] = fr_twist_const(w29, e);
+}
 __global__ void k_fk20_tap_consts(const Fr29* __restrict__ w29, Fr29 scale_plain, Fr29* __restrict__ out) {
     const int idx = blockIdx.x * blockDim.x + threadIdx.x;
     if (idx < 2 * N_BLOB) out[idx] = fk20_tap_const(w29, scale_plain, idx);
@@ -260,6 +339,7 @@
     hipFuncSetAttribute(reinterpret_cast<const void*>(k_blob_to_coeffs), hipFuncAttributeMaxDynamicSharedMemorySize, (int)LDS_NTT29);
     hipFuncSetAttribute(reinterpret_cast<const void*>(k_coeffs_to_cells), hipFuncAttributeMaxDynamicSharedMemorySize, (int)LDS_NTT29);
     hipFuncSetAttribute(reinterpret_cast<const void*>(k_coeffs_to_cells_scalars), hipFuncAttributeMaxDynamicSharedMemorySize, (int)LDS_NTT29);
+    hipFuncSetAttribute(reinterpret_cast<const void*>(k_blob_to_cells_scalars), hipFuncAttributeMaxDynamicSharedMemorySize, (int)LDS_NTT29);
 #ifdef KZG_TEST_HOOKS
     hipFuncSetAttribute(reinterpret_cast<const void*>(k_test_ntt4096), hipFuncAttributeMaxDynamicSharedMemorySize, (int)LDS_NTT29);
 #endif
@@ -312,6 +392,22 @@
     k_coeffs_to_cells_scalars<<<dim3(n, 2), 1024, LDS_NTT29, st>>>((const Fr*)coeffs, cells, (Fr*)scalars, blobs, status, (const Fr29*)w29,
                                                                    (const Fr29*)tapk, n, segs, sh);
 }
+void fk20_tap_even_consts(const void* w29, const Fr8& scale, void* out, hipStream_t st) {
+    k_fk20_tap_even_consts<<<N_BLOB / 256, 256, 0, st>>>((const Fr29*)w29, fr29_from_plain(from_mont(as_fr(scale))), (Fr29*)out);
+}
+void fr_twist_consts(const void* w29, void* out, hipStream_t st) {
+    k_fr_twist_consts<<<N_BLOB / 256, 256, 0, st>>>((const Fr29*)w29, (Fr29*)out);
+}
+bool blob_to_cells_scalars(int n, const uint8_t* blobs, uint8_t* cells, void* scalars, int* status, const void* w29, const void* tapk_even,
+                           const void* tapk, const void* twist, int segs, const Fr8* seg_shifts, hipStream_t st) {
+    const uintptr_t pb = (uintptr_t)blobs, pc = (uintptr_t)cells;
+    if (!(pb + (size_t)n * BYTES_PER_BLOB <= pc || pc + (size_t)n * N_EXT * 32 <= pb)) return false;
+    SegShifts sh;
+    for (int i = 0; i < 3; i++) sh.p[i] = fr29_mont_of(seg_shifts[i]);
+    k_blob_to_cells_scalars<<<n, 1024, LDS_NTT29, st>>>(blobs, cells, (Fr*)scalars, status, (const Fr29*)w29, (const Fr29*)tapk_even,
+                                                        (const Fr29*)tapk, (const Fr29*)twist, n, segs, sh);
+    return true;
+}
 #ifdef KZG_TEST_HOOKS
 void test_ntt4096(const uint8_t* in, uint8_t* out, const void* w29, const Fr8& n_inv, int inverse_dit, hipStream_t st) {
     k_test_ntt4096<<<1, 1024, LDS_NTT29, st>>>(in, out, (const Fr29*)w29, ntt_consts(n_inv), inverse_dit);
diff --git a/rust-eth-kzg_amd/csrc/knobs.hpp b/rust-eth-kzg_amd/csrc/knobs.hpp
--- a/rust-eth-kzg_amd/csrc/knobs.hpp
+++ b/rust-eth-kzg_amd/csrc/knobs.hpp
@@ -15,7 +15,7 @@
     int host_threads = 0;
     int serial_lanes = 0;
     bool trace = false;
-    int msm_chunks = -1, slp_program = -1, pip_shift_min = 0, fused_scalars = -1;
+    int msm_chunks = -1, slp_program = -1, pip_shift_min = 0, fused_scalars = -1, one_pass = -1;
     bool vm_search = true, vm_fold = true, verify_combine = true, msm_split = true;
     std::string fault;
     int device_batch_max = 0;
@@ -58,6 +58,7 @@
         flag("ETH_KZG_AMD_VERIFY_COMBINE", k.verify_combine);
         flag("ETH_KZG_AMD_MSM_SPLIT", k.msm_split);
         num("ETH_KZG_AMD_FUSED_SCALARS", 0, 1, k.fused_scalars);
+        num("ETH_KZG_AMD_ONE_PASS", 0, 1, k.one_pass);
         if (const char* s = getenv("ETH_KZG_AMD_FAULT")) k.fault = s;
         num("ETH_KZG_AMD_DEVICE_BATCH_MAX", 64, 1 << 20, k.device_batch_max);
         return k;
diff --git a/rust-eth-kzg_amd/csrc/launch.hpp b/rust-eth-kzg_amd/csrc/launch.hpp
--- a/rust-eth-kzg_amd/csrc/launch.hpp
+++ b/rust-eth-kzg_amd/csrc/launch.hpp
@@ -21,6 +21,10 @@
 void fk20_tap_consts(const void* w29, const Fr8& scale, void* out , hipStream_t st);
 void coeffs_to_cells_scalars(int n, const void* coeffs, uint8_t* cells, void* scalars, const uint8_t* blobs, const int* status, const void* w29,
                              const void* tapk, int segs, const Fr8* seg_shifts, hipStream_t st);
+void fk20_tap_even_consts(const void* w29, const Fr8& scale, void* out , hipStream_t st);
+void fr_twist_consts(const void* w29, void* out , hipStream_t st);
+bool blob_to_cells_scalars(int n, const uint8_t* blobs, uint8_t* cells, void* scalars, int* status, const void* w29, const void* tapk_even,
+                           const void* tapk, const void* twist, int segs, const Fr8* seg_shifts, hipStream_t st);
 void test_ntt4096(const uint8_t* in, uint8_t* out, const void* w29, const Fr8& n_inv, int inverse_dit, hipStream_t st);
 void test_scalars_be(const uint8_t* in, void* out, size_t n, hipStream_t st);
 void test_field_mul(const uint8_t* a, const uint8_t* b, uint8_t* out, int n, int is_fp, hipStream_t st);
```

New measurement: 40320, median of 6. No clear change (+0.7%).
